# owl-project/owlExaBrick

Hardware: AMD Instinct MI355X
Metric: frames/sec at 2048^2 DVR, exajet-like, MI355X (higher is better)
Workload: dtype f32; 1 GPU; c4_exajet (seed 0xe7a0003 procedural AMR, scale 1.0): 640512000 cells / 1251000 bricks / 13349488 regions, 2048x2048 DVR, dt 0.5, alpha ramp, gradient shading on, space skipping on, frameID 0; tiling=16x16 tiles interleaved over 1 GPU(s)

## Files before the change

include/exa_hip.h:

```cpp
#ifndef EXA_HIP_H
#define EXA_HIP_H

#include <stddef.h>
#include <stdint.h>

#ifdef __cplusplus
extern "C" {
#endif

#define EXA_NUM_XF_VALUES      128
#define EXA_MAX_CHANNELS       10
#define EXA_MAX_ISO_SURFACES   2
#define EXA_MAX_CONTOUR_PLANES 3


typedef struct ExaBrick {
  int32_t  lower[3];
  int32_t  size[3];
  int32_t  level;
  uint32_t begin;
} ExaBrick;

typedef struct ExaBrickRegion {
  float   domain_lo[3], domain_hi[3];
// ... 44 lines not shown
  int32_t               numFields;
  float                 voxelBounds_lo[3], voxelBounds_hi[3];
  const ExaKdNode      *kdNodes;
  uint64_t              numKdNodes;
  int32_t               kdRoot;
  int32_t               allowEmptyCells;
} ExaHipScene;

#define EXA_EMPTY_CELL_POISON_VALUE (-1e20f)
#define EXA_PREP_ALLOW_EMPTY_CELLS 1

typedef struct ExaHipStats {
  uint64_t segments;
  uint64_t sample_evals;
  uint64_t samples;
  uint64_t brick_visits;
  uint64_t corner_loads;
  uint64_t iso_segments;
  uint64_t iso_evals;
  uint64_t nodes_visited;
  uint64_t node_bytes;
  uint64_t pixels;
  uint64_t diag[9];
  uint64_t phase_cycles[5];
  float    kernel_ms;
  float    rebuild_ms;
  uint64_t walk_restarts;
  uint64_t walk_union_nodes;
  uint64_t walk_probe_overflow;
  uint64_t wave_iters;
  uint64_t tile_iters;
  uint64_t walk_leaf_visits;
} ExaHipStats;

typedef struct ExaHipRenderer ExaHipRenderer;
typedef struct ExaPrep ExaPrep;


int exa_prep_create(const int32_t *bricks7, uint64_t numBricks,
                    const int32_t *cellIDs, uint64_t numCellIDs,
                    const float *const *fields, const uint64_t *fieldLen,
                    int32_t numFields, int32_t numRegionFields, int32_t numThreads,
                    ExaPrep **out);
int exa_prep_create_ex(const int32_t *bricks7, uint64_t numBricks,
                       const int32_t *cellIDs, uint64_t numCellIDs,
                       const float *const *fields, const uint64_t *fieldLen,
                       int32_t numFields, int32_t numRegionFields, int32_t numThreads, int32_t flags,
                       ExaPrep **out);
void exa_prep_destroy(ExaPrep *);
int  exa_prep_scene(const ExaPrep *, ExaHipScene *out);
const char *exa_prep_last_error(void);
int exa_prep_ropes(const ExaPrep *, uint64_t *numLeaves, uint64_t *numNodes, float *leafBoxes, int32_t *leafLinks,
                   int32_t *leafRegion, ExaKdNode *nodes, int32_t *flags);
int exa_prep_set_kd_tree(ExaPrep *, const ExaKdNode *nodes, uint64_t numNodes, int32_t root);


int exa_hip_create(const ExaHipScene *scene, int32_t device, ExaHipRenderer **out);
int exa_hip_create_multi(const ExaHipScene *scene, const int32_t *devices, int32_t numDevices, ExaHipRenderer **out);
int exa_hip_destroy(ExaHipRenderer *);

int exa_hip_resize(ExaHipRenderer *, int32_t width, int32_t height);

int exa_hip_set_frame_state(ExaHipRenderer *, const ExaHipFrameState *);

int exa_hip_set_xf(ExaHipRenderer *, int32_t chan, const float *rgba128);

int exa_hip_set_triangles(ExaHipRenderer *, const float *vertices, uint64_t numVertices,
                          const int32_t *triangles, uint64_t numTris);

typedef struct ExaHipTracer {
  int32_t enabled;
  int32_t channels[3];
  int32_t numTraces, numTimesteps;
  float   steplen;
} ExaHipTracer;
int exa_hip_reset_tracer(ExaHipRenderer *, const ExaHipTracer *, const float *seeds);
int exa_hip_set_tracer_enabled(ExaHipRenderer *, int32_t enabled);
int exa_hip_advance_tracer(ExaHipRenderer *, int32_t *rebuild);
int exa_hip_read_traces(ExaHipRenderer *, float *dst);

int exa_hip_set_params(ExaHipRenderer *, const ExaHipParams *);

int exa_hip_set_shard(ExaHipRenderer *, int32_t rank, int32_t worldSize);
uint64_t exa_hip_output_pixels(const ExaHipRenderer *);
int exa_hip_untile(ExaHipRenderer *, const uint32_t *gathered, uint64_t shardStridePixels,
                   int32_t worldSize, uint32_t *rgba8_out, void *hipStream);

int exa_hip_render(ExaHipRenderer *, uint32_t *rgba8, int32_t dstIsDevice,
                   void *hipStream, int32_t async);

int exa_hip_render_stats(ExaHipRenderer *, uint32_t *rgba8, int32_t dstIsDevice, ExaHipStats *out);
int exa_hip_get_stats(ExaHipRenderer *, ExaHipStats *out);

int exa_hip_read_accum(ExaHipRenderer *, float *dst4);
int exa_hip_write_accum(ExaHipRenderer *, const float *src4);

int exa_hip_read_activity(ExaHipRenderer *, int32_t which , uint8_t *dst);

#define EXA_SAMPLE_WORLD_SPACE          1
#define EXA_SAMPLE_GRADIENT             2
#define EXA_SAMPLE_GRADIENT_NORMALIZED  4
int exa_hip_sample_points(ExaHipRenderer *, const float *points , uint64_t n,
                          const int32_t *channels, int32_t numChannels, int32_t flags, float fill,
                          float *values, float *gradients, int32_t *status,
                          int32_t pointersAreDevice, void *hipStream, int32_t async);
int exa_hip_resample(ExaHipRenderer *, const float lo[3], const float hi[3], const int32_t dims[3],
                     int32_t channel, int32_t flags, float fill,
                     float *out , int32_t dstIsDevice, void *hipStream, int32_t async);

int exa_hip_isosurface(ExaHipRenderer *, const float lo[3], const float hi[3], const int32_t dims[3], int32_t channel,
                       float iso, int32_t flags, uint64_t *numVertices, uint64_t *numTriangles, void *hipStream);
int exa_hip_isosurface_read(ExaHipRenderer *, float *vertices, float *gradients, int32_t *triangles,
                            int32_t pointersAreDevice, void *hipStream);
int exa_hip_isosurface_release(ExaHipRenderer *);
int exa_hip_isosurface_stage_ms(ExaHipRenderer *, float ms[6]);

#define EXA_HIST_MAX_BINS   4096
#define EXA_HIST_MAX_LEVELS 32
typedef struct ExaHipFieldStats {
  uint64_t slots;
  uint64_t empty, nan, under, over, binned;
  uint64_t levelCells[EXA_HIST_MAX_LEVELS];
  float    min, max;
} ExaHipFieldStats;
int exa_hip_histogram(ExaHipRenderer *, int32_t channel, float lo, float hi, int32_t numBins,
                      const int32_t box[6] ,
                      uint64_t *cells , uint64_t *volume ,
                      ExaHipFieldStats *stats , void *hipStream);
int exa_hip_histogram_ms(ExaHipRenderer *, float *ms);

#define EXA_STREAM_FORWARD     1
#define EXA_STREAM_BACKWARD    2
#define EXA_STREAM_NORMALIZE   4
#define EXA_STREAM_VELOCITIES  8
#define EXA_STREAM_MAX_STEPS   1048576
#define EXA_STREAM_END_NONE     0
#define EXA_STREAM_END_MAXSTEPS 1
#define EXA_STREAM_END_LEFT     2
#define EXA_STREAM_END_NOVALUE  3
#define EXA_STREAM_END_STAGNANT 4
int exa_hip_streamlines(ExaHipRenderer *, const float *seeds , uint64_t n,
                        const int32_t channels[3], float step, int32_t maxSteps, int32_t flags,
                        uint64_t *numVertices, void *hipStream);
int exa_hip_streamlines_read(ExaHipRenderer *, float *vertices , float *velocities ,
                             uint64_t *offsets , uint32_t *seedVertex , int32_t *reasons ,
                             int32_t pointersAreDevice, void *hipStream);
int exa_hip_streamlines_release(ExaHipRenderer *);
int exa_hip_streamlines_ms(ExaHipRenderer *, float *ms);

int exa_hip_set_option(ExaHipRenderer *, const char *key, int32_t value);

const char *exa_hip_last_error(const ExaHipRenderer * );

#ifdef __cplusplus
}
#endif
#endif
```

owlexabrick_amd/binding.py:

```python
import ctypes as C
import os

import numpy as np

_HERE = os.path.dirname(os.path.abspath(__file__))
LIB_PATH = os.environ.get("EXA_HIP_LIB") or os.path.join(_HERE, "libexa_hip.so")

NUM_XF_VALUES, MAX_CHANNELS, MAX_ISO, MAX_CONTOUR = 128, 10, 2, 3
DEFAULT_BASIS_FORM = 1


class _Iso(C.Structure):
    _fields_ = [("enabled", C.c_int32), ("value", C.c_float), ("channel", C.c_int32)]


class _Contour(C.Structure):
    _fields_ = [("enabled", C.c_int32), ("normal", C.c_float * 3), ("channel", C.c_int32), ("offset", C.c_float)]


class _Clip(C.Structure):
    _fields_ = [("lo", C.c_float * 3), ("hi", C.c_float * 3), ("enabled", C.c_int32)]


class _AO(C.Structure):
    _fields_ = [("length", C.c_float), ("enabled", C.c_int32)]


class ExaHipFrameState(C.Structure):
    _fields_ = [("cam_pos", C.c_float * 3), ("cam_dir00", C.c_float * 3),
                ("cam_dirDu", C.c_float * 3), ("cam_dirDv", C.c_float * 3),
                ("iso", _Iso * MAX_ISO), ("contour", _Contour * MAX_CONTOUR),
                ("clipBox", _Clip), ("ao", _AO), ("clockScale", C.c_float),
                ("xfm_vx", C.c_float * 3), ("xfm_vy", C.c_float * 3),
                ("xfm_vz", C.c_float * 3), ("xfm_p", C.c_float * 3),
                ("frameID", C.c_int32), ("xfDomain", (C.c_float * 2) * MAX_CHANNELS),
                ("xfOpacityScale", C.c_float)]


class ExaHipParams(C.Structure):
    _fields_ = [("dt", C.c_float), ("numPrimaryChannels", C.c_int32), ("colormapChannel", C.c_int32),
                ("gradientShadingDVR", C.c_int32), ("gradientShadingISO", C.c_int32),
                ("numChannels", C.c_int32), ("spaceSkippingEnabled", C.c_int32)]


class ExaHipTracer(C.Structure):
    _fields_ = [("enabled", C.c_int32), ("channels", C.c_int32 * 3), ("numTraces", C.c_int32),
                ("numTimesteps", C.c_int32), ("steplen", C.c_float)]


class ExaHipScene(C.Structure):
    _fields_ = [("bricks", C.c_void_p), ("numBricks", C.c_uint64),
                ("regions", C.c_void_p), ("numRegions", C.c_uint64),
                ("leafList", C.c_void_p), ("leafListSize", C.c_uint64),
                ("scalars", C.c_void_p), ("channelOffset", C.c_void_p),
                ("totalCells", C.c_uint64), ("numFields", C.c_int32),
                ("voxelBounds_lo", C.c_float * 3), ("voxelBounds_hi", C.c_float * 3),
                ("kdNodes", C.c_void_p), ("numKdNodes", C.c_uint64), ("kdRoot", C.c_int32), ("allowEmptyCells", C.c_int32)]


class ExaHipStats(C.Structure):
    _fields_ = [(n, C.c_uint64) for n in ("segments", "sample_evals", "samples", "brick_visits", "corner_loads",
                                          "iso_segments", "iso_evals", "nodes_visited", "node_bytes", "pixels")] + \
               [("diag", C.c_uint64 * 9), ("phase_cycles", C.c_uint64 * 5), ("kernel_ms", C.c_float), ("rebuild_ms", C.c_float),
                ("walk_restarts", C.c_uint64), ("walk_union_nodes", C.c_uint64), ("walk_probe_overflow", C.c_uint64),
                ("wave_iters", C.c_uint64), ("tile_iters", C.c_uint64), ("walk_leaf_visits", C.c_uint64)]

    def asdict(self):
        d = {}
        for n, t in self._fields_:
            v = getattr(self, n)
            d[n] = int(v) if t is C.c_uint64 else (float(v) if t is C.c_float else [int(x) for x in v])
        return d


HIST_MAX_BINS = 4096
HIST_MAX_LEVELS = 32


class ExaHipFieldStats(C.Structure):
    _fields_ = [("slots", C.c_uint64), ("empty", C.c_uint64), ("nan", C.c_uint64), ("under", C.c_uint64), ("over", C.c_uint64),
                ("binned", C.c_uint64), ("levelCells", C.c_uint64 * HIST_MAX_LEVELS), ("min", C.c_float), ("max", C.c_float)]

    def asdict(self):
        d = {k: int(getattr(self, k)) for k in ("slots", "empty", "nan", "under", "over", "binned")}
        d["levelCells"] = np.array(self.levelCells, dtype=np.uint64)
        d["min"], d["max"] = np.float32(self.min), np.float32(self.max)
        return d


BRICK_DTYPE = np.dtype([("lower", "<i4", 3), ("size", "<i4", 3), ("level", "<i4"), ("begin", "<u4")])
REGION_DTYPE = np.dtype([("dom_lo", "<f4", 3), ("dom_hi", "<f4", 3), ("vr_lo", "<f4"), ("vr_hi", "<f4"),
                         ("leafListBegin", "<i4"), ("leafListSize", "<i4"), ("finestLevelCellWidth", "<f4")])
KDNODE_DTYPE = np.dtype([("split", "<f4"), ("axis", "<i4"), ("left", "<i4"), ("right", "<i4")])
KD_EMPTY = -2 ** 31

ABI_SYMBOLS = ["exa_prep_create", "exa_prep_create_ex", "exa_prep_destroy", "exa_prep_scene", "exa_prep_last_error", "exa_prep_ropes", "exa_prep_set_kd_tree",
               "exa_hip_create", "exa_hip_create_multi", "exa_hip_destroy", "exa_hip_resize", "exa_hip_set_frame_state",
               "exa_hip_set_xf", "exa_hip_set_triangles", "exa_hip_reset_tracer", "exa_hip_set_tracer_enabled",
               "exa_hip_advance_tracer", "exa_hip_read_traces", "exa_hip_set_params", "exa_hip_set_shard", "exa_hip_output_pixels",
               "exa_hip_untile", "exa_hip_render", "exa_hip_render_stats", "exa_hip_get_stats",
               "exa_hip_read_accum", "exa_hip_write_accum", "exa_hip_read_activity",
               "exa_hip_set_option", "exa_hip_last_error", "exa_hip_sample_points", "exa_hip_resample",
               "exa_hip_isosurface", "exa_hip_isosurface_read", "exa_hip_isosurface_release", "exa_hip_isosurface_stage_ms",
               "exa_hip_histogram", "exa_hip_histogram_ms",
               "exa_hip_streamlines", "exa_hip_streamlines_read", "exa_hip_streamlines_release", "exa_hip_streamlines_ms"]

SAMPLE_WORLD_SPACE = 1
SAMPLE_GRADIENT = 2
SAMPLE_GRADIENT_NORMALIZED = 4

STREAM_FORWARD = 1
STREAM_BACKWARD = 2
STREAM_NORMALIZE = 4
STREAM_VELOCITIES = 8
STREAM_MAX_STEPS = 1 << 20
STREAM_END_NONE, STREAM_END_MAXSTEPS, STREAM_END_LEFT, STREAM_END_NOVALUE, STREAM_END_STAGNANT = range(5)

_lib = None


def lib():
    global _lib
    if _lib is None:
        if not os.path.exists(LIB_PATH):
            import subprocess
            try:
                subprocess.check_call(["make", "-C", os.path.join(_HERE, "csrc"), "-s", "-j6"])
            except Exception as e:
                raise RuntimeError(f"{LIB_PATH} not found and building it failed ({e}); run "
                                   "__graft_entry__.build(); there is no CPU fallback") from e
        L = C.CDLL(LIB_PATH)
        vp = C.c_void_p
        L.exa_prep_create.restype = C.c_int
        L.exa_prep_create.argtypes = [vp, C.c_uint64, vp, C.c_uint64, C.POINTER(vp), C.POINTER(C.c_uint64),
                                      C.c_int32, C.c_int32, C.c_int32, C.POINTER(vp)]
        L.exa_prep_create_ex.restype = C.c_int
        L.exa_prep_create_ex.argtypes = [vp, C.c_uint64, vp, C.c_uint64, C.POINTER(vp), C.POINTER(C.c_uint64),
                                         C.c_int32, C.c_int32, C.c_int32, C.c_int32, C.POINTER(vp)]
        L.exa_prep_destroy.argtypes = [vp]
        L.exa_prep_ropes.argtypes = [vp, C.POINTER(C.c_uint64), C.POINTER(C.c_uint64), vp, vp, vp, vp, C.POINTER(C.c_int32)]
        L.exa_prep_scene.argtypes = [vp, C.POINTER(ExaHipScene)]
        L.exa_prep_set_kd_tree.argtypes = [vp, vp, C.c_uint64, C.c_int32]
        L.exa_prep_last_error.restype = C.c_char_p
        L.exa_hip_create.argtypes = [C.POINTER(ExaHipScene), C.c_int32, C.POINTER(vp)]
        L.exa_hip_create_multi.argtypes = [C.POINTER(ExaHipScene), C.POINTER(C.c_int32), C.c_int32, C.POINTER(vp)]
        L.exa_hip_destroy.argtypes = [vp]
        L.exa_hip_resize.argtypes = [vp, C.c_int32, C.c_int32]
        L.exa_hip_set_frame_state.argtypes = [vp, C.POINTER(ExaHipFrameState)]
        L.exa_hip_set_xf.argtypes = [vp, C.c_int32, vp]
        L.exa_hip_set_params.argtypes = [vp, C.POINTER(ExaHipParams)]
        L.exa_hip_set_triangles.argtypes = [vp, vp, C.c_uint64, vp, C.c_uint64]
        L.exa_hip_reset_tracer.argtypes = [vp, C.POINTER(ExaHipTracer), vp]
        L.exa_hip_set_tracer_enabled.argtypes = [vp, C.c_int32]
        L.exa_hip_advance_tracer.argtypes = [vp, C.POINTER(C.c_int32)]
        L.exa_hip_read_traces.argtypes = [vp, vp]
        L.exa_hip_set_shard.argtypes = [vp, C.c_int32, C.c_int32]
        L.exa_hip_output_pixels.restype = C.c_uint64
        L.exa_hip_output_pixels.argtypes = [vp]
        L.exa_hip_untile.argtypes = [vp, vp, C.c_uint64, C.c_int32, vp, vp]
        L.exa_hip_render.argtypes = [vp, vp, C.c_int32, vp, C.c_int32]
        L.exa_hip_render_stats.argtypes = [vp, vp, C.c_int32, C.POINTER(ExaHipStats)]
        L.exa_hip_get_stats.argtypes = [vp, C.POINTER(ExaHipStats)]
        L.exa_hip_read_accum.argtypes = [vp, vp]
        L.exa_hip_write_accum.argtypes = [vp, vp]
        L.exa_hip_read_activity.argtypes = [vp, C.c_int32, vp]
        L.exa_hip_set_option.argtypes = [vp, C.c_char_p, C.c_int32]
        L.exa_hip_last_error.restype = C.c_char_p
        L.exa_hip_last_error.argtypes = [vp]
        L.exa_hip_sample_points.argtypes = [vp, vp, C.c_uint64, vp, C.c_int32, C.c_int32, C.c_float, vp, vp, vp,
                                            C.c_int32, vp, C.c_int32]
        L.exa_hip_resample.argtypes = [vp, vp, vp, vp, C.c_int32, C.c_int32, C.c_float, vp, C.c_int32, vp, C.c_int32]
        L.exa_hip_isosurface.argtypes = [vp, vp, vp, vp, C.c_int32, C.c_float, C.c_int32, C.POINTER(C.c_uint64),
                                         C.POINTER(C.c_uint64), vp]
        L.exa_hip_isosurface_read.argtypes = [vp, vp, vp, vp, C.c_int32, vp]
        L.exa_hip_isosurface_release.argtypes = [vp]
        L.exa_hip_isosurface_stage_ms.argtypes = [vp, vp]
        L.exa_hip_histogram_ms.argtypes = [vp, C.POINTER(C.c_float)]
        L.exa_hip_histogram.argtypes = [vp, C.c_int32, C.c_float, C.c_float, C.c_int32, vp, vp, vp, C.POINTER(ExaHipFieldStats), vp]
        L.exa_hip_streamlines.argtypes = [vp, vp, C.c_uint64, vp, C.c_float, C.c_int32, C.c_int32, C.POINTER(C.c_uint64), vp]
        L.exa_hip_streamlines_read.argtypes = [vp, vp, vp, vp, vp, vp, C.c_int32, vp]
        L.exa_hip_streamlines_release.argtypes = [vp]
        L.exa_hip_streamlines_ms.argtypes = [vp, C.POINTER(C.c_float)]
        _lib = L
    return _lib


class Prep:

    def __init__(self, scene, num_region_fields=None, num_threads=0, allow_empty_cells=False):
        L = lib()
        self.bricks7 = np.ascontiguousarray(scene.bricks7, dtype=np.int32).reshape(-1, 7)
        self.cellIDs = np.ascontiguousarray(scene.cellIDs, dtype=np.int32)
        self.fields = [np.ascontiguousarray(f, dtype=np.float32) for f in scene.fields]
        nf = len(self.fields)
        ptrs = (C.c_void_p * max(nf, 1))(*[f.ctypes.data for f in self.fields])
        lens = (C.c_uint64 * max(nf, 1))(*[f.size for f in self.fields])
        self.h = C.c_void_p()
        rc = L.exa_prep_create_ex(self.bricks7.ctypes.data, self.bricks7.shape[0], self.cellIDs.ctypes.data,
                                  self.cellIDs.size, ptrs, lens, nf,
                                  nf if num_region_fields is None else num_region_fields, num_threads,
                                  1 if allow_empty_cells else 0, C.byref(self.h))
        if rc:
            raise RuntimeError(L.exa_prep_last_error().decode())
        self.scene = ExaHipScene()
        L.exa_prep_scene(self.h, C.byref(self.scene))
        self.num_fields = nf

    def _arr(self, ptr, count, dtype):
        if count == 0:
            return np.zeros(0, dtype=dtype)
        buf = (C.c_char * (count * np.dtype(dtype).itemsize)).from_address(ptr)
        return np.frombuffer(buf, dtype=dtype)

    def bricks(self):
        return self._arr(self.scene.bricks, self.scene.numBricks, BRICK_DTYPE)

    def regions(self):
        return self._arr(self.scene.regions, self.scene.numRegions, REGION_DTYPE)

    def leaflist(self):
        return self._arr(self.scene.leafList, self.scene.leafListSize, np.int32)

    def scalars(self):
        return self._arr(self.scene.scalars, self.scene.numFields * self.scene.totalCells, np.float32)

    def kd_nodes(self):
        return self._arr(self.scene.kdNodes, self.scene.numKdNodes, KDNODE_DTYPE)

    def ropes(self):
        nl, nn, flags = C.c_uint64(0), C.c_uint64(0), C.c_int32(0)
        if lib().exa_prep_ropes(self.h, C.byref(nl), C.byref(nn), None, None, None, None, None):
            raise RuntimeError(lib().exa_prep_last_error().decode())
        boxes = np.zeros((nl.value, 6), dtype=np.float32)
        links = np.zeros((nl.value, 6), dtype=np.int32)
        region = np.zeros(nl.value, dtype=np.int32)
        nodes = np.zeros(max(1, nn.value), dtype=KDNODE_DTYPE)
        if lib().exa_prep_ropes(self.h, C.byref(nl), C.byref(nn), boxes.ctypes.data, links.ctypes.data, region.ctypes.data,
                                nodes.ctypes.data, C.byref(flags)):
            raise RuntimeError(lib().exa_prep_last_error().decode())
        return dict(boxes=boxes, links=links, region=region, nodes=nodes[:nn.value], flags=int(flags.value))

    def set_kd_tree(self, nodes, root):
        nodes = np.ascontiguousarray(nodes, dtype=KDNODE_DTYPE)
        if lib().exa_prep_set_kd_tree(self.h, nodes.ctypes.data if len(nodes) else None, len(nodes), int(root)):
            raise RuntimeError(lib().exa_prep_last_error().decode())
        lib().exa_prep_scene(self.h, C.byref(self.scene))

    def voxel_bounds(self):
        return (np.array(self.scene.voxelBounds_lo, dtype=np.float32),
                np.array(self.scene.voxelBounds_hi, dtype=np.float32))

    def close(self):
        if getattr(self, "h", None):
            lib().exa_prep_destroy(self.h)
            self.h = None

    __del__ = close


class Renderer:

    def __init__(self, prep, device=0, multiFieldDvr=True, devices=None):
        L = lib()
        self.prep = prep
        self.h = C.c_void_p()
        if devices is not None:
            arr = (C.c_int32 * len(devices))(*devices)
            rc = L.exa_hip_create_multi(C.byref(prep.scene), arr, len(devices), C.byref(self.h))
        else:
            rc = L.exa_hip_create(C.byref(prep.scene), device, C.byref(self.h))
        if rc:
            raise RuntimeError(L.exa_hip_last_error(None).decode())
        self.numFields = prep.num_fields
        self.frameState = ExaHipFrameState()
        self.frameState.xfm_vx[0] = self.frameState.xfm_vy[1] = self.frameState.xfm_vz[2] = 1.0
        self.frameState.ao.length, self.frameState.ao.enabled = 1e20, 1
        self.frameState.xfOpacityScale = 1.0
        for i in range(MAX_CONTOUR):
            self.frameState.contour[i].normal[0] = 1.0
            self.frameState.contour[i].offset = 0.5
        nprim = self.numFields if multiFieldDvr else 1
        self.params = ExaHipParams(0.5, nprim, 0 if (multiFieldDvr or self.numFields < 2) else 1, 1, 1, nprim, 1)
        self.doSpaceSkipping = True
        self.fbSize = (0, 0)
        self.voxelSpaceBounds = prep.voxel_bounds()

    def _check(self, rc):
        if rc:
            raise RuntimeError(lib().exa_hip_last_error(self.h).decode())

    def close(self):
        if getattr(self, "h", None):
            lib().exa_hip_destroy(self.h)
            self.h = None

    __del__ = close

    def setVoxelSpaceTransform(self, vx, vy, vz, p):
        for i in range(3):
            self.frameState.xfm_vx[i], self.frameState.xfm_vy[i] = float(vx[i]), float(vy[i])
            self.frameState.xfm_vz[i], self.frameState.xfm_p[i] = float(vz[i]), float(p[i])

    def resizeFrameBuffer(self, fbSize):
        self.fbSize = (int(fbSize[0]), int(fbSize[1]))
        self._check(lib().exa_hip_resize(self.h, *self.fbSize))

    def updateIsoValues(self, isoValues, channels, enabled):
        for i in range(MAX_ISO):
            self.frameState.iso[i].value = float(isoValues[i])
            self.frameState.iso[i].channel = int(channels[i])
            self.frameState.iso[i].enabled = int(enabled[i])

    def resetTracer(self, seeds, channels=(0, 1, 2), numTimesteps=100, steplen=1e-6, enabled=True):
        sd = np.ascontiguousarray(seeds, dtype=np.float32).reshape(-1, 3)
        self._tracer = ExaHipTracer(int(enabled), (C.c_int32 * 3)(*channels), sd.shape[0], int(numTimesteps), float(steplen))
        self._check(lib().exa_hip_reset_tracer(self.h, C.byref(self._tracer), sd.ctypes.data))

    def setTracerEnabled(self, enable):
        self._check(lib().exa_hip_set_tracer_enabled(self.h, int(bool(enable))))

    def advanceTracer(self):
        r = C.c_int32(0)
        self._check(lib().exa_hip_advance_tracer(self.h, C.byref(r)))
        return bool(r.value)

    def readTraces(self):
        out = np.zeros((self._tracer.numTraces, self._tracer.numTimesteps, 3), dtype=np.float32)
        self._check(lib().exa_hip_read_traces(self.h, out.ctypes.data))
        return out

    def setTriangles(self, verts, tris):
        v = np.ascontiguousarray(verts, dtype=np.float32).reshape(-1, 3)
        t = np.ascontiguousarray(tris, dtype=np.int32).reshape(-1, 3)
        self._check(lib().exa_hip_set_triangles(self.h, v.ctypes.data, v.shape[0], t.ctypes.data, t.shape[0]))

    def updateContourPlanes(self, normals, offsets, channels, enabled):
        for i in range(MAX_CONTOUR):
            n = np.asarray(normals[i], dtype=np.float32)
            n = (n * (np.float32(1.0) / np.sqrt(np.dot(n, n), dtype=np.float32))).astype(np.float32)
            for k in range(3):
                self.frameState.contour[i].normal[k] = float(n[k])
            self.frameState.contour[i].offset = float(offsets[i])
            self.frameState.contour[i].channel = int(channels[i])
            self.frameState.contour[i].enabled = int(enabled[i])

    def updateCamera(self, pos, dir00, dirDu, dirDv):
        for i in range(3):
            self.frameState.cam_pos[i], self.frameState.cam_dir00[i] = float(pos[i]), float(dir00[i])
            self.frameState.cam_dirDu[i], self.frameState.cam_dirDv[i] = float(dirDu[i]), float(dirDv[i])

    def updateXF(self, chan, opacities, colorMap, xfDomain, xfOpacityScale=0.1):
        colorMap = np.asarray(colorMap, dtype=np.float32)
        if colorMap.shape[0] != NUM_XF_VALUES:
            raise RuntimeError("mismatching xf size!?")
        lut = np.concatenate([colorMap[:, :3], np.asarray(opacities, dtype=np.float32).reshape(-1, 1)], axis=1)
        lut = np.ascontiguousarray(lut, dtype=np.float32)
        self.frameState.xfDomain[chan][0], self.frameState.xfDomain[chan][1] = float(xfDomain[0]), float(xfDomain[1])
        self.frameState.xfOpacityScale = float(xfOpacityScale)
        self._check(lib().exa_hip_set_xf(self.h, chan, lut.ctypes.data))

    def updateFrameID(self, frameID):
        self.frameState.frameID = int(frameID)

    def updateDt(self, dt):
        self.params.dt = float(dt)

    def setSpaceSkipping(self, enable):
        self.doSpaceSkipping = bool(enable)

    def setGradientShadingDVR(self, enable):
        self.params.gradientShadingDVR = int(bool(enable))

    def setGradientShadingISO(self, enable):
        self.params.gradientShadingISO = int(bool(enable))

    def setShard(self, rank, world):
        self._check(lib().exa_hip_set_shard(self.h, rank, world))

    def setOption(self, key, value):
        self._check(lib().exa_hip_set_option(self.h, key.encode(), int(value)))

    def _push_state(self):
        contour = any(self.frameState.contour[i].enabled for i in range(MAX_CONTOUR))
        self.params.spaceSkippingEnabled = int((not contour) and self.doSpaceSkipping)
        self._check(lib().exa_hip_set_frame_state(self.h, C.byref(self.frameState)))
        self._check(lib().exa_hip_set_params(self.h, C.byref(self.params)))

    def outputPixels(self):
        return int(lib().exa_hip_output_pixels(self.h))

    def render(self, device_ptr=None, stream=None, async_=False):
        self._push_state()
        if device_ptr is not None:
            self._check(lib().exa_hip_render(self.h, C.c_void_p(device_ptr), 1, C.c_void_p(stream or 0), int(async_)))
            return None
        n = self.outputPixels()
        out = np.zeros(n, dtype=np.uint32)
        self._check(lib().exa_hip_render(self.h, out.ctypes.data, 0, None, 0))
        W, H = self.fbSize
        return out.reshape(H, W) if n == W * H else out

    def renderStats(self):
        self._push_state()
        n = self.outputPixels()
        out = np.zeros(n, dtype=np.uint32)
        st = ExaHipStats()
        self._check(lib().exa_hip_render_stats(self.h, out.ctypes.data, 0, C.byref(st)))
        W, H = self.fbSize
        return (out.reshape(H, W) if n == W * H else out), st.asdict()

    def stats(self):
        st = ExaHipStats()
        self._check(lib().exa_hip_get_stats(self.h, C.byref(st)))
        return st.asdict()

    def readAccum(self):
        n = self.outputPixels()
        out = np.zeros((n, 4), dtype=np.float32)
        self._check(lib().exa_hip_read_accum(self.h, out.ctypes.data))
        W, H = self.fbSize
        return out.reshape(H, W, 4) if n == W * H else out

    def writeAccum(self, accum):
        a = np.ascontiguousarray(accum, dtype=np.float32)
        self._check(lib().exa_hip_write_accum(self.h, a.ctypes.data))

    def readActivity(self, which=0):
        self._push_state()
        out = np.zeros(self.prep.scene.numRegions, dtype=np.uint8)
        self._check(lib().exa_hip_read_activity(self.h, which, out.ctypes.data))
        return out

    def untile(self, gathered_ptr, shard_stride, world, out_ptr, stream=None):
        self._check(lib().exa_hip_untile(self.h, C.c_void_p(gathered_ptr), shard_stride, world,
                                         C.c_void_p(out_ptr), C.c_void_p(stream or 0)))

    def _probe_world(self, world):
        if world:
            self._push_state()
        return SAMPLE_WORLD_SPACE if world else 0

    def samplePoints(self, points, channels=(0,), gradient=False, normalized=False, world=False, fill=float("nan"),
                     stream=None, async_=False):
        chans = np.ascontiguousarray(channels, dtype=np.int32).reshape(-1)
        flags = self._probe_world(world) | (SAMPLE_GRADIENT if gradient or normalized else 0)
        flags |= SAMPLE_GRADIENT_NORMALIZED if normalized else 0
        k = chans.size
        if getattr(points, "is_cuda", False):
            import torch
            if points.dtype != torch.float32 or not points.is_contiguous() or points.numel() % 3:
                raise TypeError("points: a contiguous float32 tensor [n, 3]")
            n = points.numel() // 3
            values = torch.empty((n, k), dtype=torch.float32, device=points.device)
            grads = torch.empty((n, k, 3), dtype=torch.float32, device=points.device) if flags & SAMPLE_GRADIENT else None
            status = torch.empty((n, k), dtype=torch.int32, device=points.device)
            self._check(lib().exa_hip_sample_points(self.h, _dev_ptr(points), n, chans.ctypes.data, k, flags, float(fill),
                                                    _dev_ptr(values), _dev_ptr(grads), _dev_ptr(status), 1,
                                                    C.c_void_p(stream or 0), int(async_)))
            return values, grads, status
        pts = np.ascontiguousarray(points, dtype=np.float32).reshape(-1, 3)
        n = pts.shape[0]
        values = np.empty((n, k), dtype=np.float32)
        grads = np.empty((n, k, 3), dtype=np.float32) if flags & SAMPLE_GRADIENT else None
        status = np.empty((n, k), dtype=np.int32)
        self._check(lib().exa_hip_sample_points(self.h, pts.ctypes.data, n, chans.ctypes.data, k, flags, float(fill),
                                                values.ctypes.data, grads.ctypes.data if grads is not None else None,
                                                status.ctypes.data, 0, None, 0))
        return values, grads, status

    def resample(self, lo, hi, dims, channel=0, world=False, fill=float("nan"), out_ptr=None, stream=None, async_=False):
        flags = self._probe_world(world)
        lo3 = (C.c_float * 3)(*[float(v) for v in lo])
        hi3 = (C.c_float * 3)(*[float(v) for v in hi])
        d3 = (C.c_int32 * 3)(*[int(v) for v in dims])
        if out_ptr is not None:
            self._check(lib().exa_hip_resample(self.h, lo3, hi3, d3, int(channel), flags, float(fill), _dev_ptr(out_ptr), 1,
                                               C.c_void_p(stream or 0), int(async_)))
            return None
        out = np.empty(tuple(max(int(d), 0) for d in dims[::-1]), dtype=np.float32)
        self._check(lib().exa_hip_resample(self.h, lo3, hi3, d3, int(channel), flags, float(fill), out.ctypes.data, 0, None, 0))
        return out

    def extractIsoSurface(self, lo, hi, dims, iso, channel=0, world=False, gradients=False, stream=None):
        flags = self._probe_world(world) | (SAMPLE_GRADIENT if gradients else 0)
        lo3 = (C.c_float * 3)(*[float(v) for v in lo])
        hi3 = (C.c_float * 3)(*[float(v) for v in hi])
        d3 = (C.c_int32 * 3)(*[int(v) for v in dims])
        nv, nt = C.c_uint64(0), C.c_uint64(0)
        self._check(lib().exa_hip_isosurface(self.h, lo3, hi3, d3, int(channel), float(iso), flags, C.byref(nv), C.byref(nt),
                                             C.c_void_p(stream or 0)))
        self._iso_counts = (int(nv.value), int(nt.value), bool(gradients))
        return self._iso_counts[:2]

    def readIsoSurface(self):
        nv, nt, grad = getattr(self, "_iso_counts", (0, 0, False))
        verts = np.empty((nv, 3), dtype=np.float32)
        tris = np.empty((nt, 3), dtype=np.int32)
        grads = np.empty((nv, 3), dtype=np.float32) if grad else None
        self._check(lib().exa_hip_isosurface_read(self.h, verts.ctypes.data, grads.ctypes.data if grad else None,
                                                  tris.ctypes.data, 0, None))
        return verts, tris, grads

    def releaseIsoSurface(self):
        self._check(lib().exa_hip_isosurface_release(self.h))
        self._iso_counts = (0, 0, False)

    def isoSurfaceStageMs(self):
        ms = (C.c_float * 6)()
        self._check(lib().exa_hip_isosurface_stage_ms(self.h, ms))
        return [float(v) for v in ms]

    def isosurface(self, lo, hi, dims, iso, channel=0, world=False, gradients=False):
        self.extractIsoSurface(lo, hi, dims, iso, channel=channel, world=world, gradients=gradients)
        try:
            return self.readIsoSurface()
        finally:
            self.releaseIsoSurface()

    def histogram(self, channel, lo, hi, bins, box=None, volume=True, stream=None):
        bins = int(bins)
        n = min(max(bins, 0), HIST_MAX_BINS)
        cells = np.zeros(n, dtype=np.uint64)
        vol = np.zeros(n, dtype=np.uint64) if volume else None
        b6 = (C.c_int32 * 6)(*[int(v) for v in box]) if box is not None else None
        st = ExaHipFieldStats()
        self._check(lib().exa_hip_histogram(self.h, int(channel), float(lo), float(hi), bins, b6, cells.ctypes.data,
                                            vol.ctypes.data if volume else None, C.byref(st), C.c_void_p(stream or 0)))
        return cells, vol, st.asdict()

    def histogramMs(self):
        ms = C.c_float(0)
        self._check(lib().exa_hip_histogram_ms(self.h, C.byref(ms)))
        return float(ms.value)
# ... 56 lines not shown
```

owlexabrick_amd/csrc/exa_create.cpp:

```cpp
#include "exa_renderer.h"
#include "exa_hostbvh.h"

#include <cmath>
#include <cstdlib>
#include <cstring>

thread_local std::string g_createError;

namespace {

struct EventSlot { hipEvent_t ExaHipRenderer::*ev; bool timing; };
const EventSlot kEvents[] = {
  { &ExaHipRenderer::ev0, true },      { &ExaHipRenderer::ev1, true },      { &ExaHipRenderer::ev2, true },
  { &ExaHipRenderer::evFork, false },  { &ExaHipRenderer::evJoin4, false }, { &ExaHipRenderer::evJoin2, false },
  { &ExaHipRenderer::evJoinN, false }, { &ExaHipRenderer::evPre, false },   { &ExaHipRenderer::evPre2, false },
  { &ExaHipRenderer::evAo, false },    { &ExaHipRenderer::evAo2, false },
};
hipStream_t ExaHipRenderer::*const kSideStreams[] = { &ExaHipRenderer::side4, &ExaHipRenderer::side2, &ExaHipRenderer::sideN };

uint64_t volumeOf(const ExaBrick &B) { return uint64_t(B.size[0]) * uint64_t(B.size[1]) * uint64_t(B.size[2]); }

void buildBrickOrders(ExaHipRenderer *h, const ExaHipScene *scene)
{
  const uint64_t nb = scene->numBricks;
  h->beginUploaded.resize(nb);
  std::vector<std::pair<uint64_t, uint32_t>> keyed(nb);
  for (uint64_t b = 0; b < nb; b++) {
    const ExaBrick &B = scene->bricks[b];
    h->beginUploaded[b] = B.begin;
    double c[3];
    for (int k = 0; k < 3; k++) {
      const double cw = double(1u << B.level);
      c[k] = double(B.lower[k]) + 0.5 * cw * double(B.size[k]);
    }
    keyed[b] = { mortonKey(c, scene->voxelBounds_lo, scene->voxelBounds_hi), uint32_t(b) };
  }
  std::sort(keyed.begin(), keyed.end());
  h->beginMorton.resize(nb);
  uint64_t at = 0;
  for (uint64_t i = 0; i < nb; i++) {
    h->beginMorton[keyed[i].second] = uint32_t(at);
    at += volumeOf(scene->bricks[keyed[i].second]);
  }
  bool partition = at == scene->totalCells;
  for (int f = 0; f < scene->numFields && partition; f++) partition = scene->channelOffset[f] == uint64_t(f) * scene->totalCells;
  if (partition) {
    std::vector<std::pair<uint32_t, uint64_t>> spans(nb);
    for (uint64_t b = 0; b < nb; b++) spans[b] = { scene->bricks[b].begin, volumeOf(scene->bricks[b]) };
    std::sort(spans.begin(), spans.end());
    uint64_t run = 0;
    for (uint64_t b = 0; b < nb && partition; b++) { partition = spans[b].first == run; run += spans[b].second; }
  }
  h->brickOrderPossible = partition;
  if (!partition) h->beginMorton = h->beginUploaded;
  if (const char *e = std::getenv("EXA_BRICK_ORDER")) h->brickOrderWanted = std::atoi(e) != 0 && h->brickOrderPossible;
}

std::vector<ExaBrick> buildMarchHeaders(const ExaHipScene *scene)
{
  std::vector<ExaBrick> hdr(scene->leafListSize);
  for (uint64_t i = 0; i < scene->leafListSize; i++) {
    const ExaBrick &B = scene->bricks[scene->leafList[i]];
    const float lowerF[3] = { float(B.lower[0]), float(B.lower[1]), float(B.lower[2]) };
    const float invCw = std::ldexp(1.f, -B.level);
    ExaBrick &o = hdr[i];
    std::memcpy(&o.lower[0], lowerF, sizeof(lowerF));
    std::memcpy(&o.size[0], &invCw, sizeof(float));
    o.size[1] = B.size[0]; o.size[2] = B.size[1]; o.level = B.size[2]; o.begin = B.begin;
  }
  return hdr;
}

void chooseAddressForms(ExaHipRenderer *h, const ExaHipScene *scene)
{
  h->mul24 = 1;
  for (uint64_t b = 0; b < scene->numBricks; b++) {
    const ExaBrick &B = scene->bricks[b];
    if (uint64_t(B.size[0]) * uint64_t(B.size[1]) >= (1ull << 24) || B.size[0] >= (1 << 24) || B.size[1] >= (1 << 24) || B.size[2] >= (1 << 24))
      h->mul24 = 0;
  }
  if (scene->totalCells >= (1ull << 32)) h->mul24 = 0;
  h->addr32 = ((scene->totalCells + 2) * sizeof(float) <= (1ull << 32)
               && scene->leafListSize * 32ull < (1ull << 32)
               && scene->numKdNodes * sizeof(KdNodeDev) < (1ull << 32)) ? 1 : 0;
}

bool kdTreeWellFormed(const ExaHipScene *scene)
{
  const uint64_t nk = scene->numKdNodes;
  auto refOk = [&](int32_t ref) {
    if (ref == EXA_KD_EMPTY) return true;
    return ref >= 0 ? uint64_t(ref) < nk : uint64_t(~ref) < scene->numRegions;
  };
  bool ok = refOk(scene->kdRoot) && scene->kdRoot != EXA_KD_EMPTY && nk < 0x7fffffffull;
  for (uint64_t i = 0; ok && i < nk; i++) {
    const ExaKdNode &n = scene->kdNodes[i];
    ok = n.axis >= 0 && n.axis <= 2 && refOk(n.left) && refOk(n.right)
         && (n.left < 0 || uint64_t(n.left) > i) && (n.right < 0 || uint64_t(n.right) > i);
  }
  return ok;
}

void buildKdLevelOrder(const ExaHipScene *scene, std::vector<int32_t> &ids, std::vector<int> &levelBegin)
{
  const uint64_t nk = scene->numKdNodes;
  std::vector<int32_t> kh(nk, 1);
  for (uint64_t ii = nk; ii-- > 0;) {
    const ExaKdNode &n = scene->kdNodes[ii];
    int hh = 0;
    if (n.left >= 0) hh = std::max(hh, kh[n.left]);
    if (n.right >= 0) hh = std::max(hh, kh[n.right]);
    kh[ii] = hh + 1;
  }
  orderByHeight(kh, ids, levelBegin);
}

bool buildMarchTree(const ExaHipScene *scene, const std::vector<KdNodeDev> &kd, std::vector<KdNodeDev> &mk, int32_t &root,
                    uint32_t &bb, uint32_t &sb)
{
  auto bitsFor = [](uint64_t maxValue) { uint32_t b = 0; while (b < 63 && (1ull << b) <= maxValue) b++; return b; };
  uint64_t maxSize = 1; int maxLevel = 0; bool pow2 = true;
  for (uint64_t r = 0; r < scene->numRegions; r++) {
    const ExaBrickRegion &R = scene->regions[r];
    maxSize = std::max<uint64_t>(maxSize, (uint64_t)R.leafListSize);
    const int lv = levelOfWidth(R.finestLevelCellWidth);
    if (float(1 << lv) != R.finestLevelCellWidth) pow2 = false;
    maxLevel = std::max(maxLevel, lv);
  }
  bb = std::max(1u, bitsFor(scene->leafListSize ? scene->leafListSize - 1 : 0));
  sb = bitsFor(maxSize - 1);
  const uint32_t lb = bitsFor((uint64_t)maxLevel);
  if (!pow2 || bb + sb + lb > 31) return false;
  auto pack = [&](int32_t ref) -> int32_t {
    if (ref >= 0 || ref == EXA_KD_EMPTY) return ref;
    const ExaBrickRegion &R = scene->regions[~ref];
    return ~int32_t(packLeafRec(R.leafListBegin, R.leafListSize, R.finestLevelCellWidth, bb, sb));
  };
  mk = kd;
  bool clash = false;
  for (auto &n : mk) {
    n.left = pack(n.left); n.right = pack(n.right);
    clash = clash || (n.left < 0 && n.left != EXA_KD_EMPTY && n.left <= INT32_MIN + 1) || (n.right < 0 && n.right != EXA_KD_EMPTY && n.right <= INT32_MIN + 1);
  }
  root = pack(scene->kdRoot);
  clash = clash || (root < 0 && root <= INT32_MIN + 1);
  if (clash) return false;
  if (mk.empty()) mk.resize(1);
  return true;
}

}

extern "C" {

int exa_hip_create(const ExaHipScene *scene, int32_t device, ExaHipRenderer **out)
{
  if (!out || !scene) { g_createError = "exa_hip_create: null argument"; return 1; }
  *out = nullptr;
  if (scene->allowEmptyCells != 0 && scene->allowEmptyCells != 1) {
    g_createError = "exa_hip_create: ExaHipScene.allowEmptyCells is 0 or 1 (was the struct zero-initialised before it was filled?)";
    return 1;
  }
  int ndev = 0;
  hipError_t e = hipGetDeviceCount(&ndev);
  if (e != hipSuccess || ndev <= 0) {
    g_createError = std::string("exa_hip_create: no HIP device available (") + hipGetErrorString(e)
                  + "); this module has no CPU fallback";
    return 2;
  }
  if (device < 0 || device >= ndev) { g_createError = "exa_hip_create: bad device index"; return 1; }
  if (scene->numFields < 1 || scene->numFields > EXA_MAX_CHANNELS) { g_createError = "exa_hip_create: 1..10 scalar fields required"; return 1; }
  if (scene->numRegions == 0 || scene->numBricks == 0) { g_createError = "exa_hip_create: empty scene"; return 1; }
  if (scene->numRegions > 0x7fffffffull) { g_createError = "exa_hip_create: too many regions"; return 1; }
  ExaHipRenderer *h = new ExaHipRenderer;
  h->device = device;
  auto bail = [&]() { g_createError = h->err; delete h; return 1; };
#define CREATE_TRY(call) do { hipError_t e_ = (call); if (e_ != hipSuccess) { h->fail(std::string(#call) + ": " + hipGetErrorString(e_)); return bail(); } } while (0)
  DeviceGuard guard_(device);
  CREATE_TRY(guard_.err);

  for (uint64_t i = 0; i < scene->leafListSize; i++)
    if (scene->leafList[i] < 0 || uint64_t(scene->leafList[i]) >= scene->numBricks) { h->fail("exa_hip_create: leaf list entry out of range"); return bail(); }
  for (uint64_t b = 0; b < scene->numBricks; b++) {
    const ExaBrick &B = scene->bricks[b];
    if (B.size[0] <= 0 || B.size[1] <= 0 || B.size[2] <= 0 || B.level < 0 || B.level > 30
        || uint64_t(B.begin) + volumeOf(B) > scene->totalCells) { h->fail("exa_hip_create: brick record out of range"); return bail(); }
  }
  for (int f = 0; f < scene->numFields; f++)
    if (scene->channelOffset[f] + scene->totalCells > uint64_t(scene->numFields) * scene->totalCells) { h->fail("exa_hip_create: channel offset out of range"); return bail(); }

  h->numFields = scene->numFields;
  h->emptyCells = scene->allowEmptyCells != 0;
  if (h->emptyCells) h->basisForm = 0;
  h->totalCells = scene->totalCells;
  h->numBricks = scene->numBricks; h->leafListSize = scene->leafListSize;
  buildBrickOrders(h, scene);
  if (const char *e = std::getenv("EXA_BASIS_FORM")) h->basisForm = std::atoi(e) != 0 && !h->emptyCells;
  for (int k = 0; k < 3; k++) { h->voxLo[k] = scene->voxelBounds_lo[k]; h->voxHi[k] = scene->voxelBounds_hi[k]; }
  static_assert(sizeof(ExaBrick) == 2 * sizeof(int4), "brick = two int4");
  CREATE_TRY(h->bricks.upload(reinterpret_cast<const int4 *>(scene->bricks), scene->numBricks * 2));
  CREATE_TRY(h->leafList.upload(scene->leafList, scene->leafListSize));
  {
    const std::vector<ExaBrick> hdr = buildMarchHeaders(scene);
    CREATE_TRY(h->leafHdr.upload(reinterpret_cast<const int4 *>(hdr.data()), hdr.size() * 2));
  }
  chooseAddressForms(h, scene);
  CREATE_TRY(h->scalars.upload(scene->scalars, size_t(scene->numFields) * scene->totalCells));
  std::vector<RegionInfo> ri(scene->numRegions);
  std::vector<float2> vr(scene->numRegions);
  std::vector<float> dom(scene->numRegions * 6);
  for (uint64_t r = 0; r < scene->numRegions; r++) {
    const ExaBrickRegion &R = scene->regions[r];
    if (R.leafListSize < 1 || R.leafListBegin < 0 || uint64_t(R.leafListBegin) + uint64_t(R.leafListSize) > scene->leafListSize) {
      h->fail("exa_hip_create: region leaf list out of range"); return bail();
    }
    {
      int ex = 0;
      const float mant = std::frexp(R.finestLevelCellWidth, &ex);
      if (!(R.finestLevelCellWidth >= 1.f && R.finestLevelCellWidth <= 1073741824.f) || mant != 0.5f) {
        h->fail("exa_hip_create: region finestLevelCellWidth is not a power of two >= 1"); return bail();
      }
    }
    ri[r].listBegin = R.leafListBegin;
    ri[r].listSize = R.leafListSize;
    ri[r].finestLevelCellWidth = R.finestLevelCellWidth;
    ri[r].firstBrick = scene->leafList[R.leafListBegin];
    vr[r] = make_float2(R.valueRange_lo, R.valueRange_hi);
    for (int k = 0; k < 3; k++) { dom[6 * r + k] = R.domain_lo[k]; dom[6 * r + 3 + k] = R.domain_hi[k]; }
  }
  CREATE_TRY(h->regionInfo.upload(ri.data(), ri.size()));
  CREATE_TRY(h->valueRange.upload(vr.data(), vr.size()));
  CREATE_TRY(h->domain.upload(dom.data(), dom.size()));

  for (int k = 0; k < 3; k++) { h->kdLo[k] = INFINITY; h->kdHi[k] = -INFINITY; }
  for (uint64_t r = 0; r < scene->numRegions; r++)
    for (int k = 0; k < 3; k++) {
      h->kdLo[k] = std::fmin(h->kdLo[k], scene->regions[r].domain_lo[k]);
      h->kdHi[k] = std::fmax(h->kdHi[k], scene->regions[r].domain_hi[k]);
    }
  if (scene->kdNodes != nullptr || (scene->numKdNodes == 0 && scene->numRegions == 1 && scene->kdRoot == ~int32_t(0))) {
    const uint64_t nk = scene->numKdNodes;
    if (!kdTreeWellFormed(scene)) { h->fail("exa_hip_create: malformed kd-tree"); return bail(); }
    std::vector<int32_t> kids;
    buildKdLevelOrder(scene, kids, h->kdLevelBegin);
    std::vector<KdNodeDev> kd(nk);
    for (uint64_t i = 0; i < nk; i++) {
      kd[i].split = scene->kdNodes[i].split;
      kd[i].word = (uint32_t)scene->kdNodes[i].axis;
      kd[i].left = scene->kdNodes[i].left;
      kd[i].right = scene->kdNodes[i].right;
    }
    std::vector<RegionRec> rec(scene->numRegions);
    for (uint64_t r = 0; r < scene->numRegions; r++) {
      const ExaBrickRegion &R = scene->regions[r];
      RegionRec &q = rec[r];
      q.lo[0] = R.domain_lo[0]; q.lo[1] = R.domain_lo[1]; q.lo[2] = R.domain_lo[2];
      q.hi0 = R.domain_hi[0]; q.hi1 = R.domain_hi[1]; q.hi2 = R.domain_hi[2];
      q.finestLevelCellWidth = R.finestLevelCellWidth;
      q.firstBrick = scene->leafList[R.leafListBegin];
      q.listBegin = R.leafListBegin; q.listSize = R.leafListSize; q.pad0 = q.pad1 = 0;
    }
    CREATE_TRY(h->kdNodes.upload(kd.data(), kd.size()));
    {
      std::vector<KdNodeDev> mk;
      int32_t root = 0;
      uint32_t bb = 0, sb = 0;
      if (buildMarchTree(scene, kd, mk, root, bb, sb)) {
        CREATE_TRY(h->kdMarchNodes.upload(mk.data(), mk.size()));
        h->kdMarchRoot = root;
        h->leafBeginBits = bb; h->leafSizeBits = sb;
      }
    }
    CREATE_TRY(h->kdLevelIds.upload(kids.data(), kids.size()));
    CREATE_TRY(h->regionRec.upload(rec.data(), rec.size()));
    h->kdRoot = scene->kdRoot;
    h->haveKd = true;
  }
  CREATE_TRY(h->volActive.alloc(scene->numRegions));
  CREATE_TRY(h->isoActive.alloc(scene->numRegions));
  CREATE_TRY(h->xf.alloc(size_t(EXA_MAX_CHANNELS) * EXA_NUM_XF_VALUES));
  std::memset(h->xfHost, 0, sizeof(h->xfHost));
  CREATE_TRY(h->statsBuf.alloc(ST_COUNT));
  CREATE_TRY(h->errorFlag.alloc(1));
  CREATE_TRY(hipMemset(h->errorFlag.p, 0, sizeof(int32_t)));
  for (const EventSlot &slot : kEvents)
    CREATE_TRY(hipEventCreateWithFlags(&(h->*slot.ev), slot.timing ? hipEventDefault : hipEventDisableTiming));
  for (auto stream : kSideStreams) CREATE_TRY(hipStreamCreateWithFlags(&(h->*stream), hipStreamNonBlocking));
  {
    hipDeviceProp_t prop;
    if (hipGetDeviceProperties(&prop, device) == hipSuccess && prop.multiProcessorCount > 0)
      h->numSimdWaves = prop.multiProcessorCount * 4 * 6;
  }

  h->sc.bricks = h->bricks.p;
  h->sc.leafList = h->leafList.p;
  h->sc.leafHdr = h->leafHdr.p;
  h->sc.scalars = h->scalars.p;
  h->sc.regionInfo = h->regionInfo.p;
  h->sc.valueRange = h->valueRange.p;
  h->sc.domain = h->domain.p;
  for (int f = 0; f < EXA_MAX_CHANNELS; f++) h->sc.channelOffset[f] = f < scene->numFields ? scene->channelOffset[f] : 0;
  h->sc.numRegions = (uint32_t)scene->numRegions;
  h->sc.numInternal = 0;
#undef CREATE_TRY
  *out = h;
  return 0;
}

int exa_hip_create_multi(const ExaHipScene *scene, const int32_t *devices, int32_t numDevices, ExaHipRenderer **out)
{
  if (!out || !scene || !devices || numDevices < 1 || numDevices > 64) { g_createError = "exa_hip_create_multi: bad arguments"; return 1; }
  *out = nullptr;
  ExaHipRenderer *h = new ExaHipRenderer;
  h->device = devices[0];
  auto bail = [&](const std::string &msg) { g_createError = msg; exa_hip_destroy(h); return 1; };
  for (int i = 0; i < numDevices; i++) {
    ExaHipRenderer *c = nullptr;
    if (int rc = exa_hip_create(scene, devices[i], &c)) { exa_hip_destroy(h); return rc; }
    h->children.push_back(c);
    c->colorRowMajor = true;
    c->rank = i; c->world = numDevices; c->layoutDirty = true;
    DeviceGuard g(devices[i]);
    if (g.err != hipSuccess || hipStreamCreateWithFlags(&c->ownStream, hipStreamNonBlocking) != hipSuccess)
      return bail("exa_hip_create_multi: cannot create a stream on device " + std::to_string(devices[i]));
    if (devices[i] != devices[0]) {
      int can = 0;
      if (hipDeviceCanAccessPeer(&can, devices[i], devices[0]) != hipSuccess || !can)
        return bail("exa_hip_create_multi: device " + std::to_string(devices[i]) + " cannot access device " + std::to_string(devices[0]));
      const hipError_t e = hipDeviceEnablePeerAccess(devices[0], 0);
      if (e != hipSuccess && e != hipErrorPeerAccessAlreadyEnabled) return bail(std::string("hipDeviceEnablePeerAccess: ") + hipGetErrorString(e));
      (void)hipGetLastError();
    }
  }
  {
    DeviceGuard g(devices[0]);
    if (g.err != hipSuccess || hipEventCreateWithFlags(&h->evCall, hipEventDisableTiming) != hipSuccess) return bail("exa_hip_create_multi: hipEventCreate failed");
  }
  h->numFields = h->children[0]->numFields;
  *out = h;
  return 0;
}

int exa_hip_destroy(ExaHipRenderer *h)
{
  if (!h) return 0;
  for (ExaHipRenderer *c : h->children) exa_hip_destroy(c);
  h->children.clear();
  DeviceGuard guard_(h->device);
  if (h->ownStream) (void)hipStreamDestroy(h->ownStream);
  if (h->evCall) (void)hipEventDestroy(h->evCall);
  (void)hipDeviceSynchronize();
  for (const EventSlot &slot : kEvents) if (h->*slot.ev) (void)hipEventDestroy(h->*slot.ev);
  for (auto stream : kSideStreams) if (h->*stream) (void)hipStreamDestroy(h->*stream);
  delete h;
  return 0;
}

}
```

owlexabrick_amd/csrc/exa_device.h:

```cpp
#pragma once
#include "../../include/exa_hip.h"
#include <hip/hip_runtime.h>

#include <vector>

#ifndef EXA_MARCH_WAVES
#define EXA_MARCH_WAVES 6
#endif
#ifndef EXA_ROPE_WAVES
#define EXA_ROPE_WAVES 7
#endif
#ifndef EXA_MULTI_WAVES
#define EXA_MULTI_WAVES 6
#endif
#ifndef EXA_PREPASS_WAVES
#define EXA_PREPASS_WAVES 4
#endif
#ifndef EXA_IL2_WAVES
#define EXA_IL2_WAVES 5
#endif
#ifndef EXA_IL34_WAVES
#define EXA_IL34_WAVES 4
#endif
#ifndef EXA_PREPASS_ISO_WAVES
#define EXA_PREPASS_ISO_WAVES 4
#endif
#ifndef EXA_AO_ISO_WAVES
#define EXA_AO_ISO_WAVES 6
#endif
#ifndef EXA_EMPTY_CELLS
#define EXA_EMPTY_CELLS 0
#endif
#ifndef EXA_BASIS_FORM
#define EXA_BASIS_FORM 0
#endif
namespace exa {

struct alignas(64) BvhNode {
  float4 q0, q1, q2;
  int32_t child0, child1, pad0, pad1;
};
static_assert(sizeof(BvhNode) == 64, "node must be one 64-byte line");

struct alignas(16) RegionInfo {
  int32_t listBegin;
  int32_t listSize;
  float   finestLevelCellWidth;
  int32_t firstBrick;
};

struct alignas(16) KdNodeDev {
  float    split;
  uint32_t word;
  int32_t  left, right;
};
static_assert(sizeof(KdNodeDev) == 16, "kd node = one 16-byte load");

struct alignas(16) RopeLeaf {
  float    lo[3], hi0;
  float    hi1, hi2;
  uint32_t rec;
  uint32_t flags;
  int32_t  rope[6];
  int32_t  region;
  int32_t  pad;
};
static_assert(sizeof(RopeLeaf) == 64, "rope leaf = four 16-byte loads");

struct alignas(16) RegionRec {
  float   lo[3], hi0;
  float   hi1, hi2, finestLevelCellWidth; int32_t firstBrick;
  int32_t listBegin, listSize, pad0, pad1;
};
static_assert(sizeof(RegionRec) == 48, "region record = three 16-byte loads");

struct DeviceScene {
  const int4       *bricks;
  const int32_t    *leafList;
  const int4       *leafHdr;
  const float      *scalars;
  const RegionInfo *regionInfo;
  const float2     *valueRange;
  const float      *domain;
  unsigned long long channelOffset[EXA_MAX_CHANNELS];
  uint32_t numRegions;
  uint32_t numInternal;
};

#ifndef EXA_KD_STACK
#define EXA_KD_STACK 4
#endif
#ifndef EXA_KD_STACK_MULTI
#define EXA_KD_STACK_MULTI 3
#endif
#ifndef EXA_ROPE_QUEUE
#define EXA_ROPE_QUEUE 5
#endif
#ifndef EXA_ROPE_QUEUE_MULTI
#define EXA_ROPE_QUEUE_MULTI 5
#endif
#ifndef EXA_SEG_QUEUE
#define EXA_SEG_QUEUE 4
#endif
enum { kKdStackEntries = EXA_KD_STACK, kKdStackMultiEntries = EXA_KD_STACK_MULTI };
enum { kTile = 16, kTilePixels = 256, kStackDepth = 32, kKdStack = EXA_KD_STACK, kKdStackMulti = EXA_KD_STACK_MULTI, kSegQueue = EXA_SEG_QUEUE,
       kRopeQueue = EXA_ROPE_QUEUE, kRopeQueueMulti = EXA_ROPE_QUEUE_MULTI,
       kKdBlock = 256,
       kWideSegCap = 256,
       kWalkProbeBits = 15, kWalkProbeSize = 1 << kWalkProbeBits };

enum StatSlot { ST_SEGMENTS, ST_SAMPLE_EVALS, ST_SAMPLES, ST_BRICK_VISITS, ST_CORNER_LOADS,
                ST_ISO_SEGMENTS, ST_ISO_EVALS, ST_NODES,
                ST_W_BRICK, ST_L_BRICK, ST_W_FINAL, ST_L_FINAL, ST_W_NODE, ST_L_NODE, ST_W_LEAF, ST_L_LEAF,
                ST_KD_MISMATCH,
                ST_T_BRICK, ST_T_FINAL, ST_T_WALK, ST_T_SEG, ST_T_OTHER,
                ST_RESTARTS, ST_UNION, ST_PROBE_OVERFLOW, ST_WAVE_ITERS, ST_TILE_ITERS,
                ST_ROPE_LEAVES,
                ST_COUNT };

struct alignas(16) AoRecord { float4 posFd, ngAmb, baseRnd; uint32_t slot, pad0, pad1, pad2; };
static_assert(sizeof(AoRecord) == 64, "AO record = four 16-byte stores");

struct RenderArgs {
  DeviceScene        sc;
  const BvhNode     *volNodes;
  const BvhNode     *isoNodes;
  const KdNodeDev   *kdNodes;
  const KdNodeDev   *kdMarchNodes;
  int32_t            kdMarchRoot;
  uint32_t           leafBeginBits, leafSizeBits;
  const RegionRec   *regionRec;
  const RopeLeaf    *ropeLeaves;
  const KdNodeDev   *ropeNodes;
  int32_t            ropeRoot;
  int32_t            ropeFastDiv;
  int32_t            ropeAddr32;
  int32_t            kdRoot;
  int32_t            kdIsoRoot;
  float              kdLo[3], kdHi[3];
  const BvhNode     *meshNodes;
  const float       *meshVerts;
  const int32_t     *meshTris;
  int32_t            numTris;
  const BvhNode     *streamNodes;
  const float       *traces;
  int32_t            numStreamPrims;
  int32_t            tracerChannels[3], numTraces, numTimesteps, timestep;
  float              steplen;
  float              worldLo[3], worldHi[3];
  ExaHipFrameState   fs;
  ExaHipParams       p;
  const float4      *xf;
  const float       *cellsIl;
  int32_t            il32;
  int32_t            mul24;
  int32_t            addr32;
  float              invDtPow2;
  int32_t            fastSampler;
  float              tfFracMagic;
  int32_t            numXfChannels;
  int32_t            W, H, tilesX, tilesY;
  int32_t            rank, world;
  const int32_t     *tileMap;
  uint32_t          *color;
  int32_t            colorRowMajor;
  float4            *accum;
  float4            *surf;
  float4            *pixOut;
  uint32_t          *surfRnd;
  unsigned long long *stats;
  int32_t           *errorFlag;
  int32_t            debugPixel;
  const int32_t     *wideTileMap;
  float4            *wideSegs;
  uint32_t          *walkProbe;
  AoRecord          *aoRecs;
  uint32_t          *aoCount;
  uint32_t          *aoKeys;
  uint32_t          *aoHist;
  uint32_t          *aoOrder;
  uint8_t           *aoHit;
  uint32_t           aoBins;
  uint32_t          *tileCostPre;
  uint32_t          *tileCost;
};

struct SampleArgs {
  const int4        *leafHdr;
  const float       *scalars;
  const KdNodeDev   *kdNodes;
  const RegionRec   *regionRec;
  int32_t            kdRoot;
  int32_t            maxSteps;
  float              kdLo[3], kdHi[3];
  int32_t           *errorFlag;
  int32_t            world;
  int32_t            normalized;
  float              fill;
  ExaHipFrameState   fs;
  int32_t            numChannels;
  unsigned long long fieldOffset[EXA_MAX_CHANNELS];
  const float       *points;
  unsigned long long count;
  float             *values, *gradients;
  int32_t           *status;
  float              lo[3], step[3];
  int32_t            box0[3], box1[3];
  unsigned long long patchesX, patchesY, numPatches;
  unsigned long long strideY, strideZ;
  float             *out;
};
enum { kSamplePatchShapes = 4 };

struct StreamArgs {
  SampleArgs         s;
  const float       *seeds;
  unsigned long long numSeeds;
  unsigned long long laneBase;
  unsigned long long numLanes;
  float              step;
  int32_t            maxSteps;
  int32_t            flags;
  uint32_t          *counts;
  int32_t           *reasons;
  const unsigned long long *offsets;
  const uint32_t    *seedVertex;
  float             *vertices;
  float             *velocities;
};

hipError_t buildLbvhTopologyDevice(const float *boxes, uint32_t numPrims, BvhNode *nodes, int32_t *levelIds,
                                   std::vector<uint32_t> &internalNodesPerDepth, hipStream_t s);

#define EXA_FORM_LAUNCHERS                                                                                              \
  hipError_t launchRender(const RenderArgs &a, int numBlocks, bool grad, bool iso, bool stats, hipStream_t s);          \
  hipError_t launchSurfacePrepassKd(const RenderArgs &a, int numBlocks, bool stats, hipStream_t s);                     \
   \
  hipError_t launchAoRaysKd(const RenderArgs &a, int numBlocks, hipStream_t s);                                         \
  hipError_t launchCompositeKd(const RenderArgs &a, int numBlocks, hipStream_t s);                                      \
  hipError_t launchRenderKd(const RenderArgs &a, int numBlocks, bool grad, bool fast, bool surf,                        \
                            int stats , hipStream_t s);                                 \
                                                                    \
  hipError_t launchRenderKdRope(const RenderArgs &a, int numBlocks, bool grad, bool fast, bool surf,                    \
                                int stats, hipStream_t s);                                                              \
  hipError_t launchRenderKdWide(const RenderArgs &a, int numTiles, int lanesPerRay, bool grad, bool fast, bool surf,    \
                                hipStream_t s);                                                                         \
                          \
  hipError_t launchComputeTraces(const RenderArgs &a, float *traces, int count, hipStream_t s);                        \
    \
  hipError_t launchSamplePoints(const SampleArgs &a, bool grad, hipStream_t s);                                      \
  hipError_t launchSampleGrid(const SampleArgs &a, int shape, bool uniform, hipStream_t s);                          \
                                                                          \
  hipError_t launchStreamlines(const StreamArgs &a, bool emit, hipStream_t s);
namespace form0 { EXA_FORM_LAUNCHERS }
namespace form1 { EXA_FORM_LAUNCHERS }
namespace form0e { EXA_FORM_LAUNCHERS }
#undef EXA_FORM_LAUNCHERS

hipError_t launchVolumeActivity(const DeviceScene &sc, const ExaHipFrameState &fs, const ExaHipParams &p,
                                const float4 *xf, uint8_t *active, float tfFracMagic, hipStream_t s);
hipError_t launchIsoActivity(const DeviceScene &sc, const ExaHipFrameState &fs, uint8_t *active, hipStream_t s);
hipError_t launchRefit(BvhNode *nodes, const int32_t *nodeIds, int count, const float *domain,
                       const uint8_t *active, hipStream_t s);
hipError_t launchKdRefit(KdNodeDev *nodes, KdNodeDev *marchNodes, const int32_t *nodeIds, int count, const uint8_t *active, int which, hipStream_t s);
hipError_t launchRopeActivity(RopeLeaf *leaves, uint32_t numRegions, const uint8_t *active, int which, uint32_t *activeCount, hipStream_t s);
hipError_t launchPermuteBricks(const float *src, float *dst, const uint32_t *srcBegin, const uint32_t *dstBegin, int4 *bricks,
                               unsigned long long numBricks, int4 *leafHdr, const int32_t *leafList, unsigned long long leafListSize,
                               unsigned long long totalCells, int numFields, hipStream_t s);
hipError_t launchInterleave(const DeviceScene &sc, unsigned long long totalCells, int nch, float *out, hipStream_t s);
hipError_t launchUntile(const uint32_t *gathered, unsigned long long shardStride, int world,
                        int W, int H, uint32_t *out, hipStream_t s);
hipError_t launchProfileMarker(int tag, hipStream_t s);

}
```

owlexabrick_amd/csrc/exa_frame.cpp:

```cpp
#include "exa_renderer.h"
#include "exa_hostbvh.h"

#include <chrono>
#include <cmath>
#include <cstdio>
#include <cstdlib>
#include <thread>

#ifndef EXA_WIDE_SPEED2
#define EXA_WIDE_SPEED2 1.63
#endif
#ifndef EXA_WIDE_WORK2
#define EXA_WIDE_WORK2 1.49
#endif
#ifndef EXA_WIDE_WORK4
#define EXA_WIDE_WORK4 1.88
#endif

int ExaHipRenderer::applyBrickOrder(hipStream_t s)
{
  if (brickOrderWanted == brickOrder) return 0;
  const std::vector<uint32_t> &from = brickOrder ? beginMorton : beginUploaded, &to = brickOrderWanted ? beginMorton : beginUploaded;
  HIP_TRY(this, hipStreamSynchronize(s));
  HIP_TRY(this, hipDeviceSynchronize());
  DevBuf<uint32_t> dFrom, dTo;
  DevBuf<float> moved;
  HIP_TRY(this, dFrom.upload(from.data(), from.size()));
  HIP_TRY(this, dTo.upload(to.data(), to.size()));
  HIP_TRY(this, moved.alloc(scalars.n));
  HIP_TRY(this, launchPermuteBricks(scalars.p, moved.p, dFrom.p, dTo.p, bricks.p, numBricks, leafHdr.p, leafList.p, leafListSize,
                                    totalCells, numFields, s));
  HIP_TRY(this, hipStreamSynchronize(s));
  std::swap(scalars.p, moved.p);
  sc.scalars = scalars.p;
  brickOrder = brickOrderWanted;
  ilChannels = 0; cellsIl.release();
  return 0;
}

void ExaHipRenderer::worldBounds(float lo[3], float hi[3]) const
{
  auto cross = [](const float *a, const float *b, float *o) { o[0] = a[1] * b[2] - a[2] * b[1]; o[1] = a[2] * b[0] - a[0] * b[2]; o[2] = a[0] * b[1] - a[1] * b[0]; };
  float c0[3], c1[3], c2[3];
  cross(fs.xfm_vy, fs.xfm_vz, c0); cross(fs.xfm_vz, fs.xfm_vx, c1); cross(fs.xfm_vx, fs.xfm_vy, c2);
  const float det = fs.xfm_vx[0] * c0[0] + fs.xfm_vx[1] * c0[1] + fs.xfm_vx[2] * c0[2];
  const float ix[3] = { c0[0] / det, c1[0] / det, c2[0] / det }, iy[3] = { c0[1] / det, c1[1] / det, c2[1] / det },
              iz[3] = { c0[2] / det, c1[2] / det, c2[2] / det };
  float ip[3];
  for (int k = 0; k < 3; k++) ip[k] = -(fs.xfm_p[0] * ix[k] + (fs.xfm_p[1] * iy[k] + fs.xfm_p[2] * iz[k]));
  for (int k = 0; k < 3; k++) {
    lo[k] = voxLo[0] * ix[k] + (voxLo[1] * iy[k] + (voxLo[2] * iz[k] + ip[k]));
    hi[k] = voxHi[0] * ix[k] + (voxHi[1] * iy[k] + (voxHi[2] * iz[k] + ip[k]));
  }
}

int ExaHipRenderer::rebuildLayout()
{
  tilesX = (W + kTile - 1) / kTile;
  tilesY = (H + kTile - 1) / kTile;
  numBlocks = numBlocksFor();
  const size_t px = world <= 1 ? size_t(W) * H : size_t(numBlocks) * kTilePixels;
  HIP_TRY(this, accum.alloc(px));
  if (px) HIP_TRY(this, hipMemset(accum.p, 0, px * sizeof(float4)));
  HIP_TRY(this, color.alloc(px));
  surf.release(); surfRnd.release();
  std::vector<int32_t> map;
  map.reserve(numBlocks);
  for (int t = rank; t < tilesX * tilesY; t += world) map.push_back(t);
  if (tileOrder == 1 && world == 1 && tilesX % 8 == 0 && tilesY % 8 == 0 && ((tilesX / 8) * (tilesY / 8)) % 8 == 0) {
    const int stx = tilesX / 8;
    for (int b = 0; b < numBlocks; b++) {
      const int xcd = b % 8, j = b / 8;
      const int super = (j / 64) * 8 + xcd, in = j % 64;
      const int sx = super % stx, sy = super / stx;
      map[b] = (sy * 8 + in / 8) * tilesX + sx * 8 + in % 8;
    }
  }
  if (tileOrder == 2) {
    uint64_t st = 0x9E3779B97F4A7C15ull;
    for (size_t i = map.size(); i > 1; i--) {
      st = st * 6364136223846793005ull + 1442695040888963407ull;
      std::swap(map[i - 1], map[size_t((st >> 33) % i)]);
    }
  } else if (tileOrder == 3) {
    const float cx = 0.5f * tilesX, cy = 0.5f * tilesY;
    std::stable_sort(map.begin(), map.end(), [&](int32_t a, int32_t b) {
      const float ax = a % tilesX + 0.5f - cx, ay = a / tilesX + 0.5f - cy, bx = b % tilesX + 0.5f - cx, by = b / tilesX + 0.5f - cy;
      return ax * ax + ay * ay < bx * bx + by * by;
    });
  }
  if (tileOrder >= 4) {
    auto part = [](uint32_t v) { v &= 0xffff; v = (v | v << 8) & 0x00ff00ff; v = (v | v << 4) & 0x0f0f0f0f; v = (v | v << 2) & 0x33333333; v = (v | v << 1) & 0x55555555; return v; };
    std::stable_sort(map.begin(), map.end(), [&](int32_t a, int32_t b) {
      return (part(a % tilesX) | part(a / tilesX) << 1) < (part(b % tilesX) | part(b / tilesX) << 1);
    });
    const int chunk = tileOrder == 5 ? 16 : (tileOrder == 6 ? 64 : (tileOrder == 7 ? 256 : 0));
    if (chunk && map.size() % size_t(8 * chunk) == 0) {
      std::vector<int32_t> z(map);
      for (size_t b = 0; b < map.size(); b++) {
        const size_t xcd = b % 8, j = b / 8;
        map[b] = z[((j / chunk) * 8 + xcd) * chunk + j % chunk];
      }
    }
  }
  HIP_TRY(this, tileMap.upload(map.data(), map.size()));
  HIP_TRY(this, tileCost.alloc(size_t(tilesX) * tilesY));
  HIP_TRY(this, tileCostPre.alloc(size_t(tilesX) * tilesY));
  nPreCheap = nPreHeavy = 0;
  baseMap = map; curMap = map;
  costPhase = 1;
  nNormal = nWide4 = nWide2 = 0;
  if (assignWide(nullptr)) return 1;
  layoutDirty = false;
  return 0;
}

int ExaHipRenderer::reorderFromCosts()
{
  costPhase = 0;
  const size_t n = curMap.size();
  if (n < 2) return 0;
  std::vector<uint32_t> costOfTile(size_t(tilesX) * tilesY, 0);
  HIP_TRY(this, hipMemcpy(costOfTile.data(), tileCost.p, costOfTile.size() * sizeof(uint32_t), hipMemcpyDeviceToHost));
  uint32_t maxC = 0;
  for (size_t b = 0; b < n; b++) maxC = std::max(maxC, costOfTile[curMap[b]]);
  int kClasses = 256;
  if (const char *e = std::getenv("EXA_COST_CLASSES")) kClasses = std::max(1, std::min(4096, std::atoi(e)));
  std::vector<std::vector<int32_t>> cls(kClasses);
  for (size_t b = 0; b < n; b++) {
    const int32_t t = baseMap[b];
    const int c = kClasses - 1 - int(uint64_t(costOfTile[t]) * kClasses / (uint64_t(maxC) + 1));
    cls[c].push_back(t);
  }
  if (std::getenv("EXA_HIP_VERBOSE")) {
    uint64_t sum = 0;
    for (size_t b = 0; b < n; b++) sum += costOfTile[curMap[b]];
    std::fprintf(stderr, "[exa_hip] tile costs: %zu tiles, max %u iterations, sum %llu, per class (heaviest first):", n, maxC,
                 (unsigned long long)sum);
    for (int c = 0; c < kClasses; c++) std::fprintf(stderr, " %zu", cls[c].size());
    std::fprintf(stderr, "\n");
  }
  std::vector<int32_t> order;
  order.reserve(n);
  for (int c = 0; c < kClasses; c++) order.insert(order.end(), cls[c].begin(), cls[c].end());
  if (order != curMap) {
    HIP_TRY(this, hipMemcpy(tileMap.p, order.data(), n * sizeof(int32_t), hipMemcpyHostToDevice));
    curMap.swap(order);
  }
  nPreCheap = nPreHeavy = 0;
  if (preMeasured && prepassSplit) {
    std::vector<uint32_t> pre(size_t(tilesX) * tilesY, 0);
    HIP_TRY(this, hipMemcpy(pre.data(), tileCostPre.p, pre.size() * sizeof(uint32_t), hipMemcpyDeviceToHost));
    uint32_t maxP = 0;
    for (size_t b = 0; b < n; b++) maxP = std::max(maxP, pre[curMap[b]]);
    uint32_t div = 32, minSteps = 16;
    if (const char *e = std::getenv("EXA_PREPASS_SPLIT_DIV")) div = (uint32_t)std::max(1, std::atoi(e));
    if (const char *e = std::getenv("EXA_PREPASS_SPLIT_MIN")) minSteps = (uint32_t)std::max(0, std::atoi(e));
    const uint32_t thr = std::max<uint32_t>(minSteps, maxP / div);
    std::vector<int32_t> cheap, heavy;
    for (size_t b = 0; b < n; b++) (pre[curMap[b]] > thr ? heavy : cheap).push_back(curMap[b]);
    if (!heavy.empty() && !cheap.empty()) {
      std::stable_sort(heavy.begin(), heavy.end(), [&](int32_t x, int32_t y) { return pre[x] > pre[y]; });
      std::vector<int32_t> both(cheap);
      both.insert(both.end(), heavy.begin(), heavy.end());
      HIP_TRY(this, splitMap.refill(both.data(), both.size()));
      nPreCheap = (int)cheap.size(); nPreHeavy = (int)heavy.size();
    }
    if (std::getenv("EXA_HIP_VERBOSE"))
      std::fprintf(stderr, "[exa_hip] pre-pass costs: longest iso march %u steps; %d tiles in the heavy pipeline, %d in the other\n", maxP, nPreHeavy, nPreCheap);
  }
  return assignWide(&costOfTile);
}

int ExaHipRenderer::assignWide(const std::vector<uint32_t> *costOfTile)
{
  const size_t n = curMap.size();
  std::vector<int32_t> normal, w4, w2;
  const int lanesTop = 4;
  if (wideMode == 2 || wideMode == 4) {
    (wideMode >= 4 ? w4 : w2) = curMap;
  } else if (wideMode == 1 && costOfTile) {
    double kSpeed2 = EXA_WIDE_SPEED2;
    const double kWork2 = EXA_WIDE_WORK2, kLoaded = 1.3;
// ... 141 lines not shown
          std::fprintf(stderr, "[exa_hip] no memory for the channel-interleaved copy of %d fields: field-by-field march\n", want);
        ilNoMemory = want;
        want = 0;
      }
      if (want) {
        HIP_TRY(this, hipMemsetAsync(cellsIl.p + size_t(totalCells) * want, 0, 2 * size_t(want) * sizeof(float), s));
        HIP_TRY(this, launchInterleave(sc, totalCells, want, cellsIl.p, s));
        ilChannels = want;
      }
    }
  }
  const bool needIso = isoEnabled();
  if (volDirty || (needIso && isoDirty)) {
    HIP_TRY(this, hipEventRecord(ev2, s));
    const bool volChanged = volDirty;
    if (volDirty) {
      HIP_TRY(this, launchVolumeActivity(sc, fs, p, xf.p, volActive.p, tfFracMagic(), s));
      if (lbvhBuilt && refit(volNodes, volActive.p, s)) return 1;
      if (haveKd && kdRefit(volActive.p, 0, s)) return 1;
      volDirty = false;
    }
    if (needIso && isoDirty) {
      if (lbvhBuilt && !isoNodes.p && topoNodes.n) {
        HIP_TRY(this, isoNodes.alloc(topoNodes.n));
        HIP_TRY(this, hipMemcpyAsync(isoNodes.p, topoNodes.p, topoNodes.n * sizeof(BvhNode), hipMemcpyDeviceToDevice, s));
      }
      HIP_TRY(this, launchIsoActivity(sc, fs, isoActive.p, s));
      if (lbvhBuilt && refit(isoNodes, isoActive.p, s)) return 1;
      if (haveKd && kdRefit(isoActive.p, 1, s)) return 1;
      isoDirty = false;
    }
    if (haveKd && volChanged) {
      if (!activeCountBuf.p) HIP_TRY(this, activeCountBuf.alloc(1));
      HIP_TRY(this, hipMemsetAsync(activeCountBuf.p, 0, sizeof(uint32_t), s));
      HIP_TRY(this, launchRopeActivity(ropeBuilt ? ropeLeaves.p : nullptr, sc.numRegions, volActive.p, 0, activeCountBuf.p, s));
      ropeFlagsStale = !ropeBuilt;
    }
    HIP_TRY(this, hipEventRecord(ev1, s));
    HIP_TRY(this, hipEventSynchronize(ev1));
    HIP_TRY(this, hipEventElapsedTime(&last.rebuild_ms, ev2, ev1));
    if (haveKd && volChanged) HIP_TRY(this, hipMemcpy(&activeRegions, activeCountBuf.p, sizeof(uint32_t), hipMemcpyDeviceToHost));
    if (haveKd && kdRoot < 0 && kdRoot != EXA_KD_EMPTY) {
      uint8_t f[2] = {1, 1};
      HIP_TRY(this, hipMemcpy(&f[0], volActive.p + ~kdRoot, 1, hipMemcpyDeviceToHost));
      if (needIso) HIP_TRY(this, hipMemcpy(&f[1], isoActive.p + ~kdRoot, 1, hipMemcpyDeviceToHost));
      rootLeafVolActive = f[0] != 0;
      rootLeafIsoActive = f[1] != 0;
    }
  }
  const bool ropeBefore = ropeThisFrame;
  ropeThisFrame = ropeWanted();
  if (ropeThisFrame != ropeBefore && std::getenv("EXA_HIP_VERBOSE"))
    std::fprintf(stderr, "[exa_hip] %u of %u regions active for the volume march: %s walk (option walk = %d)\n", activeRegions, sc.numRegions,
                 ropeThisFrame ? "rope" : "stack", walkMode);
  if (ropeThisFrame && !ropeBuilt) {
    HIP_TRY(this, hipStreamSynchronize(s));
    if (buildRopes()) return 1;
    ropeThisFrame = ropeBuilt;
  }
  if (ropeThisFrame && ropeFlagsStale) {
    HIP_TRY(this, launchRopeActivity(ropeLeaves.p, sc.numRegions, volActive.p, 0, nullptr, s));
    ropeFlagsStale = false;
  }
  return 0;
}

int ExaHipRenderer::rebuildStreamlines(hipStream_t s)
{
  streamDirty = false;
  numStreamPrims = 0;
  if (!haveTracer) return 0;
  const int NT = tracer.numTimesteps;
  const long long nprims = (long long)tracer.numTraces * (NT - 1);
  const int timestep = std::min(this->timestep, NT);
  if (timestep < 2 || nprims <= 0) return 0;
  HIP_TRY(this, hipStreamSynchronize(s));
  std::vector<float> host(traces.n);
  HIP_TRY(this, hipMemcpy(host.data(), traces.p, traces.n * sizeof(float), hipMemcpyDeviceToHost));
  std::vector<float> boxes;
  std::vector<int32_t> prim;
  for (long long p = 0; p < nprims; p++) {
    if (int(p % NT) >= timestep - 1) continue;
    const float *pa = &host[3 * p], *pb = &host[3 * (p + 1)];
    if (!(pa[0] < 2e10f && pb[0] < 2e10f)) continue;
    for (int k = 0; k < 3; k++) boxes.push_back(std::fmin(pa[k] - 2.f, pb[k] - 2.f));
    for (int k = 0; k < 3; k++) boxes.push_back(std::fmax(pa[k] + 2.f, pb[k] + 2.f));
    prim.push_back((int32_t)p);
  }
  if (prim.empty()) return 0;
  LbvhTopology topo;
  topo.build(boxes.data(), prim.size());
  const std::vector<BvhNode> nodes = fillBoxes(topo, boxes, [&](size_t i) { return prim[i]; });
  HIP_TRY(this, streamNodes.upload(nodes.data(), nodes.size()));
  numStreamPrims = (int)prim.size();
  return 0;
}

int ExaHipRenderer::fillRenderArgs(RenderArgs &a, uint32_t *dstDevice, bool stats, hipStream_t s)
{
  a.sc = sc;
  a.volNodes = volNodes.p;
  a.isoNodes = isoNodes.p;
  a.fs = fs;
  a.p = p;
  a.xf = xf.p;
  a.tfFracMagic = tfFracMagic();
  a.fastSampler = fastSampler;
  a.mul24 = mul24; a.addr32 = addr64 ? 0 : addr32;
  a.cellsIl = ilChannels == p.numPrimaryChannels ? cellsIl.p : nullptr;
  a.il32 = (uint64_t(totalCells) + 2) * uint64_t(ilChannels > 0 ? ilChannels : 1) * sizeof(float) <= (1ull << 32) && !addr64 ? 1 : 0;
  {
    int e = 0;
    const float mant = std::frexp(p.dt, &e);
    a.invDtPow2 = (mant == 0.5f && e > -100 && e < 100) ? 1.f / p.dt : 0.f;
  }
  a.numXfChannels = numFields;
  a.W = W; a.H = H; a.tilesX = tilesX; a.tilesY = tilesY;
  a.rank = rank; a.world = world;
  a.tileMap = tileMap.p;
  a.color = dstDevice;
  a.colorRowMajor = colorRowMajor ? 1 : 0;
  a.accum = accum.p;
  a.surf = surf.p;
  a.surfRnd = surfRnd.p;
  a.stats = statsBuf.p;
  a.errorFlag = errorFlag.p;
  a.debugPixel = debugPixel;
  a.walkProbe = nullptr;
  if (stats && statsMode == 1 && walkProbeOn && useKd()) {
    const size_t need = size_t(numBlocks) * (256 / 64) * kWalkProbeSize;
    if (walkProbe.n != need) HIP_TRY(this, walkProbe.alloc(need));
    HIP_TRY(this, hipMemsetAsync(walkProbe.p, 0, need * sizeof(uint32_t), s));
    a.walkProbe = walkProbe.p;
  }
  a.tileCost = nullptr;
  a.tileCostPre = nullptr;
  if (feedback && costPhase == 1 && useKd() && measureCosts) {
    HIP_TRY(this, hipMemsetAsync(tileCost.p, 0, tileCost.n * sizeof(uint32_t), s));
    a.tileCost = tileCost.p;
    preMeasured = surfacesEnabled();
    if (preMeasured) {
      HIP_TRY(this, hipMemsetAsync(tileCostPre.p, 0, tileCostPre.n * sizeof(uint32_t), s));
      a.tileCostPre = tileCostPre.p;
    }
  }
  a.kdNodes = kdNodes.p;
  const bool packed = packRecords && kdMarchNodes.p != nullptr && !(stats && statsMode == 1);
  a.kdMarchNodes = packed ? kdMarchNodes.p : kdNodes.p;
  a.kdMarchRoot = packed ? kdMarchRoot : kdRoot;
  if (!rootLeafVolActive) a.kdMarchRoot = EXA_KD_EMPTY + 1;
  a.leafBeginBits = packed ? leafBeginBits : 0;
  a.leafSizeBits = packed ? leafSizeBits : 0;
  a.regionRec = regionRec.p;
  a.ropeLeaves = (ropeThisFrame && ropeBuilt) ? ropeLeaves.p : nullptr;
  a.ropeNodes = ropeNodes.p;
  a.ropeRoot = ropeRoot;
  a.ropeFastDiv = ropeFastDiv;
  a.ropeAddr32 = addr64 ? 0 : ropeAddr32;
  a.kdRoot = kdRoot;
  a.kdIsoRoot = rootLeafIsoActive ? kdRoot : EXA_KD_EMPTY + 1;
  for (int k = 0; k < 3; k++) { a.kdLo[k] = kdLo[k]; a.kdHi[k] = kdHi[k]; }
  worldBounds(a.worldLo, a.worldHi);
  a.meshNodes = meshNodes.p; a.meshVerts = meshVerts.p; a.meshTris = meshTris.p; a.numTris = numTris;
  a.streamNodes = streamNodes.p; a.traces = traces.p; a.numStreamPrims = numStreamPrims;
  for (int k = 0; k < 3; k++) a.tracerChannels[k] = tracer.channels[k];
  a.numTraces = tracer.numTraces; a.numTimesteps = tracer.numTimesteps; a.timestep = std::min(timestep, tracer.numTimesteps); a.steplen = tracer.steplen;
  return 0;
}

int ExaHipRenderer::prepareSurfaceLists(RenderArgs &a, bool stats, hipStream_t s)
{
  if (useKd() && surfacesEnabled() && surf.n != accum.n) {
    HIP_TRY(this, surf.alloc(accum.n));
    HIP_TRY(this, surfRnd.alloc(accum.n));
    a.surf = surf.p; a.surfRnd = surfRnd.p;
  }
  a.aoRecs = nullptr; a.aoCount = nullptr; a.aoKeys = nullptr; a.aoHist = nullptr; a.aoOrder = nullptr; a.aoHit = nullptr; a.aoBins = 0;
  if (!(useKd() && surfacesEnabled() && fs.ao.enabled && aoDefer && !stats)) return 0;
  const size_t recs = size_t(numBlocks) * kTilePixels;
  if (aoRecs.n != recs && aoRecs.alloc(recs) != hipSuccess) {
    (void)hipGetLastError();
    aoRecs.release();
    if (std::getenv("EXA_HIP_VERBOSE")) std::fprintf(stderr, "[exa_hip] no memory for the list of deferred AO rays (%zu records): traced inline\n", recs);
    return 0;
  }
  if (!aoCount.p) HIP_TRY(this, aoCount.alloc(8));
  HIP_TRY(this, hipMemsetAsync(aoCount.p, 0, 8 * sizeof(uint32_t), s));
  a.aoRecs = aoRecs.p; a.aoCount = aoCount.p;
  if (aoDefer == 2) {
    const uint32_t cells = world <= 1 ? uint32_t((W + 31) / 32) * uint32_t((H + 31) / 32) : uint32_t((numBlocks + 3) / 4);
    const uint32_t bins = std::max(1u, cells) * 24u;
    if (aoKeys.n != 2 * recs) { HIP_TRY(this, aoKeys.alloc(2 * recs)); HIP_TRY(this, aoOrder.alloc(2 * recs)); HIP_TRY(this, aoHit.alloc(2 * recs)); }
    if (aoBins != bins) { HIP_TRY(this, aoHist.alloc(2 * size_t(bins))); aoBins = bins; }
    a.aoKeys = aoKeys.p; a.aoOrder = aoOrder.p; a.aoHit = aoHit.p; a.aoHist = aoHist.p; a.aoBins = bins;
  }
  return 0;
}

hipError_t ExaHipRenderer::march(const RenderArgs &a, int n, bool surfArg, int statsArg, hipStream_t s)
{
  return (ropeThisFrame && ropeBuilt) ? EXA_FORM(this, launchRenderKdRope)(a, n, p.gradientShadingDVR != 0, fastMath != 0, surfArg, statsArg, s)
                                      : EXA_FORM(this, launchRenderKd)(a, n, p.gradientShadingDVR != 0, fastMath != 0, surfArg, statsArg, s);
}

int ExaHipRenderer::launchSurfaces(const RenderArgs &a, bool surfOn, bool stats, hipStream_t s)
{
  if (surfOn) HIP_TRY(this, EXA_FORM(this, launchSurfacePrepassKd)(a, numBlocks, stats, s));
  if (surfOn && !stats) HIP_TRY(this, EXA_FORM(this, launchAoRaysKd)(a, numBlocks, s));
  return 0;
}

int ExaHipRenderer::launchPlain(const RenderArgs &a, bool surfOn, bool stats, hipStream_t s)
{
  if (launchSurfaces(a, surfOn, stats, s)) return 1;
  HIP_TRY(this, march(a, numBlocks, surfOn, stats ? statsMode : 0, s));
  return 0;
}

int ExaHipRenderer::launchSplit(const RenderArgs &a, bool overlap, hipStream_t s)
{
  HIP_TRY(this, hipEventRecord(evFork, s));
  RenderArgs ah = a, ac = a;
  ac.tileMap = splitMap.p;
  ah.tileMap = splitMap.p + nPreCheap;
  if (a.aoRecs) {
    ah.aoRecs = a.aoRecs + size_t(nPreCheap) * kTilePixels;
    ah.aoCount = a.aoCount + 4;
    if (a.aoKeys) {
      const size_t off = 2 * size_t(nPreCheap) * kTilePixels;
      ah.aoKeys = a.aoKeys + off; ah.aoOrder = a.aoOrder + off; ah.aoHit = a.aoHit + off; ah.aoHist = a.aoHist + a.aoBins;
    }
  }
  HIP_TRY(this, hipStreamWaitEvent(side2, evFork, 0));
  HIP_TRY(this, EXA_FORM(this, launchSurfacePrepassKd)(ah, nPreHeavy, false, side2));
  HIP_TRY(this, hipStreamWaitEvent(sideN, evFork, 0));
  HIP_TRY(this, EXA_FORM(this, launchSurfacePrepassKd)(ac, nPreCheap, false, sideN));
  if (overlap) {
    HIP_TRY(this, hipEventRecord(evPre2, side2));
    HIP_TRY(this, hipEventRecord(evPre, sideN));
    HIP_TRY(this, hipStreamWaitEvent(side4, evPre2, 0));
    HIP_TRY(this, EXA_FORM(this, launchAoRaysKd)(ah, nPreHeavy, side4));
    HIP_TRY(this, hipEventRecord(evAo2, side4));
    HIP_TRY(this, hipStreamWaitEvent(side4, evPre, 0));
    HIP_TRY(this, EXA_FORM(this, launchAoRaysKd)(ac, nPreCheap, side4));
    HIP_TRY(this, hipEventRecord(evAo, side4));
  } else {
    HIP_TRY(this, EXA_FORM(this, launchAoRaysKd)(ah, nPreHeavy, side2));
    HIP_TRY(this, EXA_FORM(this, launchAoRaysKd)(ac, nPreCheap, sideN));
  }
  HIP_TRY(this, march(ac, nPreCheap, true, 0, sideN));
  if (overlap) {
    HIP_TRY(this, hipStreamWaitEvent(sideN, evAo, 0));
    HIP_TRY(this, EXA_FORM(this, launchCompositeKd)(ac, nPreCheap, sideN));
  }
  HIP_TRY(this, hipEventRecord(evJoinN, sideN));
  HIP_TRY(this, march(ah, nPreHeavy, true, 0, side2));
  if (overlap) {
    HIP_TRY(this, hipStreamWaitEvent(side2, evAo2, 0));
    HIP_TRY(this, EXA_FORM(this, launchCompositeKd)(ah, nPreHeavy, side2));
  }
  HIP_TRY(this, hipEventRecord(evJoin2, side2));
  HIP_TRY(this, hipStreamWaitEvent(s, evJoin2, 0));
  HIP_TRY(this, hipStreamWaitEvent(s, evJoinN, 0));
  return 0;
}

int ExaHipRenderer::launchOverlap(const RenderArgs &a, hipStream_t s)
{
  HIP_TRY(this, EXA_FORM(this, launchSurfacePrepassKd)(a, numBlocks, false, s));
  HIP_TRY(this, hipEventRecord(evPre, s));
  HIP_TRY(this, hipStreamWaitEvent(side4, evPre, 0));
  HIP_TRY(this, EXA_FORM(this, launchAoRaysKd)(a, numBlocks, side4));
  HIP_TRY(this, hipEventRecord(evAo, side4));
  HIP_TRY(this, march(a, numBlocks, true, 0, s));
  HIP_TRY(this, hipStreamWaitEvent(s, evAo, 0));
  HIP_TRY(this, EXA_FORM(this, launchCompositeKd)(a, numBlocks, s));
  return 0;
}

int ExaHipRenderer::launchWide(const RenderArgs &a, bool surfOn, hipStream_t s)
{
  if (launchSurfaces(a, surfOn, false, s)) return 1;
  HIP_TRY(this, hipEventRecord(evFork, s));
  RenderArgs aw = a;
  if (nWide4) {
    HIP_TRY(this, hipStreamWaitEvent(side4, evFork, 0));
    aw.wideTileMap = wideMap.p;
    aw.wideSegs = wideSegs.p;
    HIP_TRY(this, EXA_FORM(this, launchRenderKdWide)(aw, nWide4, lanesTopInUse, p.gradientShadingDVR != 0, fastMath != 0, surfOn, side4));
    HIP_TRY(this, hipEventRecord(evJoin4, side4));
  }
  if (nWide2) {
    HIP_TRY(this, hipStreamWaitEvent(side2, evFork, 0));
    aw.wideTileMap = wideMap.p + nWide4;
    aw.wideSegs = wideSegs.p + size_t(nWide4) * segsPerRay(lanesTopInUse) * kTilePixels;
    HIP_TRY(this, EXA_FORM(this, launchRenderKdWide)(aw, nWide2, 2, p.gradientShadingDVR != 0, fastMath != 0, surfOn, side2));
    HIP_TRY(this, hipEventRecord(evJoin2, side2));
  }
  RenderArgs an = a;
  an.tileMap = normalMap.p;
  HIP_TRY(this, hipStreamWaitEvent(sideN, evFork, 0));
  HIP_TRY(this, march(an, nNormal, surfOn, 0, sideN));
  HIP_TRY(this, hipEventRecord(evJoinN, sideN));
  if (nWide4) HIP_TRY(this, hipStreamWaitEvent(s, evJoin4, 0));
  if (nWide2) HIP_TRY(this, hipStreamWaitEvent(s, evJoin2, 0));
  HIP_TRY(this, hipStreamWaitEvent(s, evJoinN, 0));
  return 0;
}

int ExaHipRenderer::launch(uint32_t *dstDevice, bool stats, hipStream_t s)
{
  if (streamDirty && rebuildStreamlines(s)) return 1;
  RenderArgs a{};
  if (fillRenderArgs(a, dstDevice, stats, s)) return 1;
  if (haveTracer && tracer.enabled && timestep < tracer.numTimesteps && timestep >= 1) {
    const long long px = (long long)W * H;
    HIP_TRY(this, EXA_FORM(this, launchComputeTraces)(a, traces.p, (int)std::min<long long>(tracer.numTraces, px), s));
  }
  if (prepareSurfaceLists(a, stats, s)) return 1;
  HIP_TRY(this, hipEventRecord(ev0, s));
  if (useKd()) {
    const bool surfOn = surfacesEnabled();
    const bool wide = !stats && !emptyCells && nWide4 + nWide2 > 0 && p.numPrimaryChannels == 1 && a.debugPixel < 0;
    const bool split = surfOn && !stats && !wide && costPhase == 0 && !a.tileCost && nPreHeavy > 0 && nPreCheap > 0
                       && nPreHeavy + nPreCheap == numBlocks && a.debugPixel < 0;
    const bool overlap = aoOverlap && a.aoRecs && fs.ao.enabled && !wide && !(fs.clockScale > 0.f);
    if (overlap) {
      if (pixBuf.n != accum.n) HIP_TRY(this, pixBuf.alloc(accum.n));
      a.pixOut = pixBuf.p;
    }
    if (split) { if (launchSplit(a, overlap, s)) return 1; }
    else if (overlap) { if (launchOverlap(a, s)) return 1; }
    else if (wide) { if (launchWide(a, surfOn, s)) return 1; }
    else if (launchPlain(a, surfOn, stats, s)) return 1;
  } else {
    HIP_TRY(this, EXA_FORM(this, launchRender)(a, numBlocks, p.gradientShadingDVR != 0, surfacesEnabled(), stats, s));
  }
  last.node_bytes = useKd() ? sizeof(KdNodeDev) : sizeof(BvhNode);
  HIP_TRY(this, hipEventRecord(ev1, s));
  return 0;
}

int ExaHipRenderer::buildRopes()
{
  const auto tBuild0 = std::chrono::steady_clock::now();
  const size_t nk = kdNodes.n, nr = sc.numRegions;
  static_assert(sizeof(KdNodeDev) == sizeof(ExaKdNode), "the device's kd node is the ABI's with activity bits in the axis word");
  std::vector<ExaKdNode> kd(nk);
  std::vector<float> dom(6 * nr);
  std::vector<RegionInfo> ri(nr);
  if (nk) HIP_TRY(this, hipMemcpy(kd.data(), kdNodes.p, nk * sizeof(KdNodeDev), hipMemcpyDeviceToHost));
  HIP_TRY(this, hipMemcpy(dom.data(), domain.p, dom.size() * sizeof(float), hipMemcpyDeviceToHost));
  HIP_TRY(this, hipMemcpy(ri.data(), regionInfo.p, nr * sizeof(RegionInfo), hipMemcpyDeviceToHost));
  const unsigned nthreads = std::min(16u, std::max(1u, std::thread::hardware_concurrency()));
// ... 228 lines not shown
```

owlexabrick_amd/csrc/exa_kernels.hip:

```cpp
#include "exa_device.h"
#include <cfloat>

#if EXA_BASIS_FORM == 0 && EXA_EMPTY_CELLS
#define EXA_FORM_NS form0e
#elif EXA_BASIS_FORM == 0
#define EXA_FORM_NS form0
#elif EXA_BASIS_FORM == 1 && EXA_EMPTY_CELLS
#error "empty cells are a per-corner property: the per-axis association (EXA_BASIS_FORM 1) does not apply"
#elif EXA_BASIS_FORM == 1
#define EXA_FORM_NS form1
#else
#error "EXA_BASIS_FORM is 0 (source order) or 1 (per-axis association with fused multiply-adds)"
#endif
#define EXA_F1 (EXA_BASIS_FORM == 1)
#ifndef EXA_TU_ROPE
#define EXA_TU_ROPE 0
#endif
#ifndef EXA_TU_SAMPLE
#define EXA_TU_SAMPLE 0
#endif
#ifndef EXA_TU_STREAM
#define EXA_TU_STREAM 0
#endif
namespace exa {
// ... 1747 lines not shown
  }
}

__device__ __forceinline__ Ray aoRayOf(const ExaHipFrameState &fs, const float4 posFd, const float4 ngAmb, const float4 baseRnd, unsigned j)
{
  Lcg rnd;
  rnd.state = __float_as_uint(baseRnd.w);
  if (j & 1u) { rnd.next(); rnd.next(); }
  const V3 wN = mk(ngAmb.x, ngAmb.y, ngAmb.z);
  const V3 vN = fabsf(wN.x) > fabsf(wN.y) ? normalize(mk(-wN.z, 0.f, wN.x)) : normalize(mk(0.f, wN.z, -wN.y));
  const V3 uN = cross(vN, wN);
  const float u1 = rnd.next(), u2 = rnd.next();
  const float rr = sqrtf(u1);
  const float theta = 2.f * 3.14159265358979323846f * u2;
  const V3 sp = mk(rr * cosf(theta), rr * sinf(theta), sqrtf(1.f - u1));
  Ray ao_ray;
  ao_ray.org = mk(posFd.x, posFd.y, posFd.z);
  ao_ray.dir = normalize((sp.x * uN + sp.y * vN) + sp.z * wN);
  ao_ray.tmin = 1e-4f; ao_ray.tmax = fs.ao.length;
  return ao_ray;
}

enum { kAoDirClasses = 24, kAoCellShift = 5 };
__device__ __forceinline__ uint32_t aoRayKey(const RenderArgs &a, uint32_t slot, V3 d)
{
  const float ax = fabsf(d.x), ay = fabsf(d.y), az = fabsf(d.z);
  const uint32_t dom = (ax >= ay && ax >= az) ? 0u : (ay >= az ? 1u : 2u);
  const uint32_t oct = (d.x < 0.f ? 1u : 0u) | (d.y < 0.f ? 2u : 0u) | (d.z < 0.f ? 4u : 0u);
  uint32_t cell;
  if (a.world == 1) {
    const uint32_t px = slot % (uint32_t)a.W, py = slot / (uint32_t)a.W;
    cell = (py >> kAoCellShift) * (((uint32_t)a.W + 31u) >> kAoCellShift) + (px >> kAoCellShift);
  } else {
    cell = slot >> 10;
  }
  return cell * kAoDirClasses + oct * 3u + dom;
}
#if !EXA_TU_ROPE
__global__ __launch_bounds__(256) void aoKeyKernel(const RenderArgs a)
{
  const unsigned numRays = 2u * a.aoCount[0];
  for (unsigned j = blockIdx.x * 256u + threadIdx.x; j < numRays; j += gridDim.x * 256u) {
    const AoRecord *r = a.aoRecs + (j >> 1);
    const Ray ray = aoRayOf(a.fs, r->posFd, r->ngAmb, r->baseRnd, j);
    const uint32_t key = min(aoRayKey(a, r->slot, ray.dir), a.aoBins - 1u);
    a.aoKeys[j] = key;
    atomicAdd(&a.aoHist[key], 1u);
  }
}
__global__ __launch_bounds__(1024) void aoScanKernel(uint32_t *hist, uint32_t numBins)
{
  __shared__ uint32_t part[1024];
  const uint32_t per = (numBins + 1023u) / 1024u;
  const uint32_t b0 = min(threadIdx.x * per, numBins), b1 = min(b0 + per, numBins);
  uint32_t sum = 0;
  for (uint32_t b = b0; b < b1; b++) sum += hist[b];
  part[threadIdx.x] = sum;
  __syncthreads();
  for (uint32_t off = 1; off < 1024u; off <<= 1) {
    const uint32_t v = threadIdx.x >= off ? part[threadIdx.x - off] : 0u;
    __syncthreads();
    part[threadIdx.x] += v;
    __syncthreads();
  }
  uint32_t run = part[threadIdx.x] - sum;
  for (uint32_t b = b0; b < b1; b++) { const uint32_t c = hist[b]; hist[b] = run; run += c; }
}
__global__ __launch_bounds__(256) void aoScatterKernel(const RenderArgs a)
{
  const unsigned numRays = 2u * a.aoCount[0];
  for (unsigned j = blockIdx.x * 256u + threadIdx.x; j < numRays; j += gridDim.x * 256u)
    a.aoOrder[atomicAdd(&a.aoHist[a.aoKeys[j]], 1u)] = j;
}
__global__ __launch_bounds__(256) void aoFinalizeKernel(const RenderArgs a)
{
  const unsigned numHits = a.aoCount[0];
  for (unsigned h = blockIdx.x * 256u + threadIdx.x; h < numHits; h += gridDim.x * 256u) {
    const AoRecord *r = a.aoRecs + h;
    const float4 posFd = r->posFd, ngAmb = r->ngAmb, baseRnd = r->baseRnd;
    const uint32_t slot = r->slot;
    const int hitCnt = (int)a.aoHit[2u * h] + (int)a.aoHit[2u * h + 1u];
    const float shadow = (float)hitCnt / 2;
    const float fd = posFd.w;
    const float ns = 1.f - shadow;
    const float t_hit = a.surf[slot].w;
    a.surf[slot] = make_float4(ngAmb.w + baseRnd.x * fd * ns, ngAmb.w + baseRnd.y * fd * ns, ngAmb.w + baseRnd.z * fd * ns, t_hit);
  }
}

#endif

template <bool ISO_ONLY, bool SORTED>
__global__ __launch_bounds__(kKdBlock, (ISO_ONLY ? EXA_AO_ISO_WAVES : EXA_PREPASS_WAVES)) void aoRaysKdKernel(const RenderArgs a)
{
  extern __shared__ __attribute__((aligned(16))) unsigned char smem[];
  float4 *xfLds = reinterpret_cast<float4 *>(smem);
  unsigned char *sp0 = smem + size_t(a.numXfChannels) * EXA_NUM_XF_VALUES * sizeof(float4);
  int *stackRef = reinterpret_cast<int *>(sp0);
  float *stackF = reinterpret_cast<float *>(sp0 + size_t(kKdStackEntries) * kKdBlock * 4) + threadIdx.x;
  int *qRegion = reinterpret_cast<int *>(sp0 + size_t(kKdStack) * kKdBlock * 12) + threadIdx.x;
  float *qT = reinterpret_cast<float *>(sp0 + size_t(kKdStack) * kKdBlock * 12 + size_t(kSegQueue) * kKdBlock * 4) + threadIdx.x;
  for (int i = threadIdx.x; i < a.numXfChannels * EXA_NUM_XF_VALUES; i += kKdBlock) xfLds[i] = a.xf[i];
  __syncthreads();
  Ctx<0> C;
  C.a = &a;
  C.xfLds = xfLds;
  C.stack = stackRef + threadIdx.x;
  C.guardTripped = false;
  C.fastSampler = a.fastSampler != 0;
  const ExaHipFrameState &fs = a.fs;
  const unsigned numRays = 2u * a.aoCount[0];
  for (;;) {
    unsigned base = 0;
    if ((threadIdx.x & 63) == 0) base = atomicAdd(&a.aoCount[2], 64u);
    base = (unsigned)__shfl((int)base, 0, 64);
    if (base >= numRays) break;
    const unsigned k = base + (threadIdx.x & 63);
    const bool live = k < numRays;
    const unsigned j = (SORTED && live) ? a.aoOrder[k] : k;
    int hitFlag = 0;
    float4 posFd = make_float4(0.f, 0.f, 0.f, 0.f), ngAmb = posFd, baseRnd = posFd;
    uint32_t slot = 0;
    if (live) {
      const AoRecord *r = a.aoRecs + (j >> 1);
      posFd = r->posFd; ngAmb = r->ngAmb; baseRnd = r->baseRnd; slot = r->slot;
      const Ray ao_ray = aoRayOf(fs, posFd, ngAmb, baseRnd, j);
      SurfaceHit ao;
      traceSurfacesKd<0, ISO_ONLY>(C, ao_ray, ao, false, stackF, qRegion, qT);
      if (ao.primID >= 0 || ao.primID == EXA_PRIMID_ISOSURFACE || ao.primID == EXA_PRIMID_PLANE
          || ao.primID == EXA_PRIMID_STREAMLINE) hitFlag = 1;
      if (SORTED) a.aoHit[j] = (uint8_t)hitFlag;
    }
    if (SORTED) continue;
    const int other = __shfl_xor(hitFlag, 1, 64);
    if (live && !(j & 1u)) {
      const int hitCnt = hitFlag + other;
      const float shadow = (float)hitCnt / 2;
      const float fd = posFd.w;
      const float ns = 1.f - shadow;
      const float t_hit = a.surf[slot].w;
      a.surf[slot] = make_float4(ngAmb.w + baseRnd.x * fd * ns, ngAmb.w + baseRnd.y * fd * ns, ngAmb.w + baseRnd.z * fd * ns, t_hit);
    }
  }
  if (C.guardTripped) atomicExch(a.errorFlag, 1);
}

constexpr int marchWaves(int MULTI, int STATS, bool SMALL, int NCH, bool ROPE)
{
  return NCH ? (NCH == 2 ? EXA_IL2_WAVES : EXA_IL34_WAVES)
             : (MULTI == 1 ? EXA_MULTI_WAVES
                           : (MULTI ? 5 : ((ROPE && !STATS && SMALL && EXA_BASIS_FORM == 1) ? EXA_ROPE_WAVES : EXA_MARCH_WAVES)));
}

template <bool GRAD, bool FAST, int MULTI, bool SURF, int STATS, bool SMALL, int NCH = 0, bool ROPE = false>
__global__ __launch_bounds__(kKdBlock, marchWaves(MULTI, STATS, SMALL, NCH, ROPE)) void renderFrameKdKernel(const RenderArgs a)
{
  constexpr bool LEAN = marchWaves(MULTI, STATS, SMALL, NCH, ROPE) >= 7;
  constexpr int PACKED_CT = !ROPE ? -1 : (STATS == 1 ? 0 : (SMALL ? 1 : -1));
  const bool packedRec = PACKED_CT < 0 ? a.leafBeginBits != 0 : PACKED_CT != 0;
  static_assert(NCH == 0 || (MULTI == 2 && STATS == 0), "the interleaved march is a multi-channel variant of the shipped kernel");
  constexpr int KSB = MULTI == 1 ? kKdStackMulti : kKdStack;
  constexpr int KS = MULTI == 1 ? kKdStackMultiEntries : kKdStackEntries;
  constexpr int QN = ROPE ? (MULTI == 1 ? kRopeQueueMulti : kRopeQueue) : kSegQueue;
  static_assert(MULTI != 0 || (size_t(EXA_NUM_XF_VALUES) * sizeof(float4) + size_t(kKdBlock) * (ROPE ? QN * 16 : (KSB + QN) * 12))
                                  * marchWaves(MULTI, STATS, SMALL, NCH, ROPE) <= 160 * 1024,
                "LDS per workgroup x waves per SIMD exceeds the CU's 160 KB: shorten the queue or lower the occupancy");
  extern __shared__ __attribute__((aligned(16))) unsigned char smem[];
  float4 *xfLds = reinterpret_cast<float4 *>(smem);
  unsigned char *sp0 = smem + size_t(a.numXfChannels) * EXA_NUM_XF_VALUES * sizeof(float4);
  int *stackRef = reinterpret_cast<int *>(sp0);
  float *stackF = reinterpret_cast<float *>(sp0 + size_t(KS) * kKdBlock * 4) + threadIdx.x;
  unsigned char *q0 = ROPE ? sp0 : sp0 + size_t(KSB) * kKdBlock * 12;
  int *qRegion = reinterpret_cast<int *>(q0) + threadIdx.x;
  float *qT = reinterpret_cast<float *>(q0 + size_t(QN) * kKdBlock * 4) + threadIdx.x;
  float4 *queue4 = reinterpret_cast<float4 *>(sp0) + threadIdx.x;
  for (int i = threadIdx.x; i < a.numXfChannels * EXA_NUM_XF_VALUES; i += kKdBlock) xfLds[i] = a.xf[i];
  __syncthreads();

  Ctx<STATS> C;
  C.a = &a;
  C.xfLds = xfLds;
  C.stack = stackRef + threadIdx.x;
  C.guardTripped = false;
  const unsigned long long clockBegin = clock64();
  if (STATS) for (int i = 0; i < ST_COUNT; i++) C.st[i] = 0;
  __shared__ unsigned long long lapMarks[STATS == 2 ? 8 * (kKdBlock / 64) : 1];
  if (STATS == 2) {
    C.lapMark = lapMarks + 8 * (threadIdx.x >> 6);
    if ((threadIdx.x & 63) == 0) {
      C.lapMark[0] = clock64(); C.lapMark[1] = ST_T_OTHER - ST_T_BRICK;
      for (int i = 2; i < 7; i++) C.lapMark[i] = 0;
    }
  }

  const int wavesPerBlock = kKdBlock / 64;
  const int gwave = blockIdx.x * wavesPerBlock + (threadIdx.x >> 6);
  const int tile = a.tileMap[gwave >> 2];
  const int tx = tile % a.tilesX, ty = tile / a.tilesX;
  const int wave = gwave & 3, lane = threadIdx.x & 63;
  const int inX = ((wave & 1) << 3) + laneX(lane), inY = ((wave >> 1) << 3) + laneY(lane);
  const int px = tx * kTile + inX, py = ty * kTile + inY;
  const bool inside = px < a.W && py < a.H && (a.debugPixel < 0 || a.debugPixel == px + a.W * py);

  if (STATS == 1 && a.walkProbe) C.probe = a.walkProbe + size_t(gwave) * kWalkProbeSize;
  unsigned marchIters = 0;
  if (inside) {
    const ExaHipFrameState &fs = a.fs;
    const int frameID = fs.frameID;
    Lcg rnd;
    rnd.init((uint32_t)(frameID * a.W * a.H) + (uint32_t)px, (uint32_t)py);
    const float sx = float(px) + rnd.next();
    const float sy = float(py) + rnd.next();
    Ray ray;
    ray.org = mk(fs.cam_pos);
    ray.dir = normalize((mk(fs.cam_dir00) + sx * mk(fs.cam_dirDu)) + sy * mk(fs.cam_dirDv));
    ray.tmin = 1e-6f; ray.tmax = 1e8f;
    float surface_t_hit = ray.tmax;
    if (SURF) {
      const size_t slot0 = (a.world == 1) ? size_t(px) + size_t(a.W) * py
                                          : size_t(tile / a.world) * kTilePixels + (inY * kTile + inX);
      surface_t_hit = a.surf[slot0].w;
      rnd.state = a.surfRnd[slot0];
    }
    const float interleavedSamplingOffset = rnd.next();
    ray.tmax = surface_t_hit;
    if (fs.clipBox.enabled) {
      float c0, c1;
      boxTest(ray, mk(fs.clipBox.lo), mk(fs.clipBox.hi), c0, c1);
      ray.tmin = c0; ray.tmax = c1;
    }
    surface_t_hit = ray.tmax;
    ray.org = xfmPoint(fs, ray.org);
    ray.org.x = __int_as_float(__builtin_amdgcn_readfirstlane(__float_as_int(ray.org.x)));
    ray.org.y = __int_as_float(__builtin_amdgcn_readfirstlane(__float_as_int(ray.org.y)));
    ray.org.z = __int_as_float(__builtin_amdgcn_readfirstlane(__float_as_int(ray.org.z)));
    ray.dir = xfmVector(fs, ray.dir);
    const float dt_scale = length(ray.dir);
    ray.dir = normalize(ray.dir);
    ray.tmin = dt_scale * ray.tmin;
    ray.tmax = surface_t_hit * dt_scale;

    Color4 pixelColor; pixelColor.x = pixelColor.y = pixelColor.z = pixelColor.w = 0.f;
    const int numChannels = a.p.numPrimaryChannels;

    KdWalk w;
    w.pk.v = 0;
    {
      Ray whole = ray; whole.tmin = -INFINITY; whole.tmax = INFINITY;
      float r0, r1;
      const bool hit = boxTest(whole, mk(a.kdLo), mk(a.kdHi), r0, r1);
      w.tn = fmaxf(r0, ray.tmin);
      w.tf = fminf(r1, ray.tmax);
      w.tEnd = w.tf;
      w.ref = (hit && w.tn < w.tf) ? (ROPE ? a.ropeRoot : a.kdMarchRoot) : EXA_KD_DONE;
    }
    bool ropeFast = false;
    if (ROPE) ropeFast = a.ropeFastDiv != 0 && !anyLane(!ropeRayInRange(ray));

    float walkTmin = ray.tmin;

    bool haveSeg = false;
    int listBegin = 0, listSize = 0;
    float flcw = 1.f;
    float t1 = 0.f, t_i = 0.f, t_sample = 0.f, actual_dt = 0.f;
    int child = 0, chan = 0;
    int4 hb0 = make_int4(0, 0, 0, 1), hb1 = make_int4(1, 1, 1, 0);
    Basis B;
    B.sumWV = 0.f; B.sumW = 0.f; B.sumD = mk(0.f, 0.f, 0.f); B.sumDC = mk(0.f, 0.f, 0.f);
    float xWV[NCH > 1 ? NCH - 1 : 1];
    V3 xD[NCH > 1 ? NCH - 1 : 1];
#pragma unroll
    for (int c = 0; c < (NCH > 1 ? NCH - 1 : 1); c++) { xWV[c] = 0.f; xD[c] = mk(0.f, 0.f, 0.f); }
    const float *field0 = a.sc.scalars + a.sc.channelOffset[0];
    const float *field = field0;
    float xfRcpRange0 = 0.f, xfRange0 = 0.f;
    if (FAST && !MULTI) {
      xfRange0 = __int_as_float(__builtin_amdgcn_readfirstlane(__float_as_int((fs.xfDomain[0][1] - fs.xfDomain[0][0]) + 1e-20f)));
      xfRcpRange0 = __int_as_float(__builtin_amdgcn_readfirstlane(__float_as_int(__builtin_amdgcn_rcpf(xfRange0))));
    }
    float xfRcpRangeN[NCH ? NCH : 1], xfRangeN[NCH ? NCH : 1];
#pragma unroll
    for (int c = 0; c < (NCH ? NCH : 1); c++) {
      xfRangeN[c] = (FAST && NCH) ? __int_as_float(__builtin_amdgcn_readfirstlane(__float_as_int((fs.xfDomain[c][1] - fs.xfDomain[c][0]) + 1e-20f))) : 0.f;
      xfRcpRangeN[c] = (FAST && NCH) ? __int_as_float(__builtin_amdgcn_readfirstlane(__float_as_int(__builtin_amdgcn_rcpf(xfRangeN[c])))) : 0.f;
    }

    unsigned iter = 0;
    for (;; iter++) {
      if (iter == 0xfffffff0u) { C.guardTripped = true; break; }
      if (anyLane(!haveSeg && w.pk.get(PK_QCOUNT) == 0 && w.ref != EXA_KD_DONE)) {
        C.lap(ST_T_WALK);
        do {
          const bool want = w.pk.get(PK_QCOUNT) < QN && w.ref != EXA_KD_DONE;
          if (want) {
            if (ROPE) ropeStep<STATS, SMALL, QN, LEAN, PACKED_CT>(C, w, walkTmin, a, queue4, ray, ropeFast, interleavedSamplingOffset);
            else kdStep<false, STATS, SMALL, KS>(C, w, walkTmin, a, stackF, qRegion, qT, ray, 0, walkTmin, 1.f, a.kdMarchNodes, a.kdMarchRoot);
          }
        } while (anyLane(!haveSeg && w.pk.get(PK_QCOUNT) == 0 && w.ref != EXA_KD_DONE));
      }
      if (!haveSeg) {
        C.lap(ST_T_SEG);
        const int qc = w.pk.get(PK_QCOUNT);
        if (qc == 0) break;
        const int qh = w.pk.get(PK_QHEAD);
        int region;
        float t0, tiQueued = 0.f;
        if (ROPE) {
          const float4 e = queue4[qh * kKdBlock];
          region = __float_as_int(e.x); t1 = e.y; tiQueued = e.z; t0 = e.w;
        } else {
          region = qRegion[qh * kKdBlock];
          t0 = qT[(2 * qh) * kKdBlock];
          t1 = qT[(2 * qh + 1) * kKdBlock];
        }
        w.pk.template incWrap<QN>(PK_QHEAD);
        w.pk.dec(PK_QCOUNT);
        if (packedRec) {
          const unsigned d = (unsigned)region;
          listBegin = (int)(d & ((1u << a.leafBeginBits) - 1u));
          listSize = (int)((d >> a.leafBeginBits) & ((1u << a.leafSizeBits) - 1u)) + 1;
          flcw = __int_as_float((127 + (int)(d >> (a.leafBeginBits + a.leafSizeBits))) << 23);
        } else {
          const RegionInfo ri = a.sc.regionInfo[region];
          listBegin = ri.listBegin; listSize = ri.listSize;
          flcw = ri.finestLevelCellWidth;
        }
        C.count(ST_SEGMENTS);
        haveSeg = true;
        w.pk.setBit(PK_NEEDHDR);
        if (ROPE && packedRec)
          t_i = tiQueued;
        else if (a.invDtPow2 != 0.f)
          t_i = firstSampleTPow2(t0, a.p.dt * flcw, a.invDtPow2 * __int_as_float(0x7f000000 - __float_as_int(flcw)), interleavedSamplingOffset);
        else
          t_i = firstSampleT(t0, a.p.dt * flcw, interleavedSamplingOffset);
        {
          const float t_next = fminf(t_i, t1);
          t_sample = 0.5f * (fminf(t1, t_next) + t0);
          actual_dt = t_next - t0;
        }
        C.count(ST_SAMPLE_EVALS);
      }

      C.lap(ST_T_BRICK);
      C.phase(ST_W_BRICK);
      if (listSize > 1 || w.pk.get(PK_NEEDHDR)) {
        if (SMALL) {
          const char *hp = reinterpret_cast<const char *>(a.sc.leafHdr) + ((uint32_t)(listBegin + child) << 5);
          hb0 = *reinterpret_cast<const int4 *>(hp); hb1 = *reinterpret_cast<const int4 *>(hp + 16);
        } else {
          const unsigned at = 2u * (unsigned)(listBegin + child);
          hb0 = a.sc.leafHdr[at]; hb1 = a.sc.leafHdr[at + 1u];
        }
        w.pk.clearField(PK_NEEDHDR);
      }
      if (NCH) addBasisFastIl<GRAD, SMALL, (NCH ? NCH : 2)>(B, xWV, xD, hb0, hb1, a.cellsIl, rayAt(ray.org, t_sample, ray.dir));
      else addBasisFast<GRAD, STATS, SMALL>(C, B, hb0, hb1, MULTI ? field : field0, rayAt(ray.org, t_sample, ray.dir));
      child++;
      if (child < listSize) continue;

      C.lap(ST_T_FINAL);
      C.phase(ST_W_FINAL);
      if (NCH) {
        if (B.sumW > 1e-20f) {
#pragma unroll
          for (int c = 0; c < NCH; c++) {
            const float wv = c == 0 ? B.sumWV : xWV[c == 0 ? 0 : c - 1];
            const V3 sd = c == 0 ? B.sumD : xD[c == 0 ? 0 : c - 1];
            const float cellValue = fdivExact<FAST>(wv, B.sumW);
            V3 grad = mk(0.f, 0.f, 0.f);
            if (GRAD) grad = gradOf(B.sumW, wv, sd, B.sumDC);
            integrateVolume<FAST, STATS, FAST>(C, ray, pixelColor, actual_dt, cellValue, grad, flcw, c, xfRcpRangeN[c], xfRangeN[c]);
          }
        }
#pragma unroll
        for (int c = 0; c < (NCH > 1 ? NCH - 1 : 1); c++) { xWV[c] = 0.f; xD[c] = mk(0.f, 0.f, 0.f); }
      } else if (B.sumW > 1e-20f) {
        C.count(ST_SAMPLES);
        const float cellValue = fdivExact<FAST>(B.sumWV, B.sumW);
        V3 grad = mk(0.f, 0.f, 0.f);
        if (GRAD) grad = gradOf(B.sumW, B.sumWV, B.sumD, B.sumDC);
        integrateVolume<FAST, STATS, (FAST && !MULTI), LEAN>(C, ray, pixelColor, actual_dt, cellValue, grad, flcw, MULTI ? chan : 0, xfRcpRange0, xfRange0);
      }
      B.sumWV = 0.f; B.sumW = 0.f; B.sumD = mk(0.f, 0.f, 0.f); B.sumDC = mk(0.f, 0.f, 0.f);
      child = 0;
      if (MULTI && !NCH) {
        chan++;
        if (chan < numChannels) {
          field = a.sc.scalars + a.sc.channelOffset[chan];
          C.count(ST_SAMPLE_EVALS);
          continue;
        }
        chan = 0; field = field0;
      }
      if (pixelColor.w >= EXA_TERMINATION_THRESHOLD) {
        pixelColor.x = pixelColor.x * pixelColor.w;
        pixelColor.y = pixelColor.y * pixelColor.w;
        pixelColor.z = pixelColor.z * pixelColor.w;
        pixelColor.w = 1.f;
        break;
      }
      const float t_last = fminf(t_i, t1);
      if (t_last >= t1) {
        haveSeg = false;
        continue;
      }
      t_i += a.p.dt * flcw;
      {
        const float t_next = fminf(t_i, t1);
        t_sample = 0.5f * (fminf(t1, t_next) + t_last);
        actual_dt = t_next - t_last;
      }
      C.count(ST_SAMPLE_EVALS);
    }

    C.lap(ST_T_OTHER);
    marchIters = iter;
    size_t slot, colorSlot;
    {
      unsigned tid = threadIdx.x, bid = blockIdx.x;
      asm volatile("" : "+v"(tid));
      asm volatile("" : "+s"(bid));
      const int lane2 = tid & 63, wave2 = (tid >> 6) & 3;
      const int inX2 = ((wave2 & 1) << 3) + laneX(lane2), inY2 = ((wave2 >> 1) << 3) + laneY(lane2);
      slot = (a.world == 1) ? size_t(tx * kTile + inX2) + size_t(a.W) * (ty * kTile + inY2)
                            : size_t(a.tileMap[(bid * wavesPerBlock + (tid >> 6)) >> 2] / a.world) * kTilePixels + (inY2 * kTile + inX2);
      colorSlot = a.colorRowMajor ? size_t(tx * kTile + inX2) + size_t(a.W) * (ty * kTile + inY2) : slot;
    }
    if (SURF && a.pixOut) {
      a.pixOut[slot] = make_float4(pixelColor.x, pixelColor.y, pixelColor.z, pixelColor.w);
    } else {
    float4 bgColor = make_float4(0.f, 0.f, 0.f, 0.f);
    if (SURF) bgColor = a.surf[slot];
    float cr = pixelColor.w * pixelColor.x + (1.f - pixelColor.w) * bgColor.x;
    float cg = pixelColor.w * pixelColor.y + (1.f - pixelColor.w) * bgColor.y;
    float cb = pixelColor.w * pixelColor.z + (1.f - pixelColor.w) * bgColor.z;
    if (fs.clockScale > 0.f) cr = clockHeat(fs.clockScale, clockBegin);
    if (frameID > 0) {
      const float4 acc = a.accum[slot];
      cr += acc.x; cg += acc.y; cb += acc.z;
    }
    a.accum[slot] = make_float4(cr, cg, cb, 1.f);
    const float div = frameID + 1.f;
    cr = cr / div; cg = cg / div; cb = cb / div;
    a.color[colorSlot] = make_rgba8(linear_to_srgb(cr), linear_to_srgb(cg), linear_to_srgb(cb));
    }
  }

  if (a.tileCost) {
    unsigned v = marchIters;
    for (int off = 32; off > 0; off >>= 1) v = max(v, (unsigned)__shfl_down((int)v, off, 64));
    unsigned bid = blockIdx.x, tid = threadIdx.x;
    asm volatile("" : "+s"(bid));
    asm volatile("" : "+v"(tid));
    if (lane == 0) atomicMax(&a.tileCost[a.tileMap[(bid * wavesPerBlock + (tid >> 6)) >> 2]], v);
  }
  if (C.guardTripped) atomicExch(a.errorFlag, 1);
  if (STATS == 2) {
    if (lane < 5 && C.lapMark[2 + lane]) atomicAdd(&a.stats[ST_T_BRICK + lane], C.lapMark[2 + lane]);
  }
  if (STATS == 1) {
    for (int i = 0; i < ST_COUNT; i++) {
      unsigned long long v = inside ? C.st[i] : 0ull;
      for (int off = 32; off > 0; off >>= 1) v += __shfl_down(v, off, 64);
      if ((threadIdx.x & 63) == 0 && v) atomicAdd(&a.stats[i], v);
    }
    __shared__ unsigned wgMaxIters;
    if (threadIdx.x == 0) wgMaxIters = 0;
    __syncthreads();
    unsigned v = marchIters;
    for (int off = 32; off > 0; off >>= 1) v = max(v, (unsigned)__shfl_down((int)v, off, 64));
    if (lane == 0) atomicMax(&wgMaxIters, v);
    __syncthreads();
    if (lane == 0) atomicAdd(&a.stats[ST_WAVE_ITERS], (unsigned long long)v);
    if (threadIdx.x == 0) atomicAdd(&a.stats[ST_TILE_ITERS], 4ull * wgMaxIters);
  }
}

__device__ __forceinline__ void kdCollectStep(Ctx<0> &C, KdWalk &w, const float winLo, const float winHi, const RenderArgs &a,
                                              float *stackF, const Ray &ray, const KdNodeDev *nodes, const int root,
                                              float4 *out, unsigned &count)
{
  if (w.ref != EXA_KD_EMPTY && !(w.tn < winHi)) { w.ref = EXA_KD_DONE; return; }
  if (w.ref < 0 && w.ref > EXA_KD_DONE) {
    if (w.tn >= winLo && w.tn < w.tf) out[count++] = make_float4(__int_as_float(~w.ref), w.tn, w.tf, 0.f);
    w.ref = EXA_KD_EMPTY;
  }
  if (w.ref == EXA_KD_EMPTY || (w.ref != EXA_KD_DONE && !(w.tf > winLo))) kdPop(C, w, root, stackF, nodes, ray);
#define EXA_KD_POP_LATER() (w.ref = EXA_KD_EMPTY)
  if (w.ref < 0 || !(w.tf > winLo) || !(w.tn < winHi)) return;
  const int4 n = *reinterpret_cast<const int4 *>(nodes + w.ref);
  const float split = __int_as_float(n.x);
  const int axis = n.y & 3;
  const int bits = (n.y >> 2) & 3;
  const float ox = ray.org.x, oy = ray.org.y, oz = ray.org.z, dx = ray.dir.x, dy = ray.dir.y, dz = ray.dir.z;
  float o = axis == 0 ? ox : oy, d = axis == 0 ? dx : dy;
  o = axis == 2 ? oz : o;
  d = axis == 2 ? dz : d;
  if (d == 0.f) {
    if (o < split && (bits & 1)) w.ref = n.z;
    else if (o > split && (bits & 2)) w.ref = n.w;
    else EXA_KD_POP_LATER();
    return;
  }
  const float ts = (split - o) / d;
  const bool nearIsLeft = d > 0.f;
  const int nearRef = nearIsLeft ? n.z : n.w, farRef = nearIsLeft ? n.w : n.z;
  const bool nearAct = (bits & (nearIsLeft ? 1 : 2)) != 0, farAct = (bits & (nearIsLeft ? 2 : 1)) != 0;
  if (ts >= w.tf) {
    if (nearAct) w.ref = nearRef; else EXA_KD_POP_LATER();
  } else if (ts <= w.tn) {
    if (farAct) w.ref = farRef; else EXA_KD_POP_LATER();
  } else if (nearAct) {
    if (farAct) {
      const int head = w.pk.get(PK_SHEAD), count_ = w.pk.get(PK_SCOUNT);
      C.stack[head * kKdBlock] = farRef;
      stackF[(2 * head) * kKdBlock] = ts;
      stackF[(2 * head + 1) * kKdBlock] = w.tf;
      w.pk.template incWrap<kKdStackEntries>(PK_SHEAD);
      if (count_ == kKdStackEntries) w.pk.setBit(PK_DROPPED); else w.pk.inc(PK_SCOUNT);
    }
    w.ref = nearRef;
    w.tf = ts;
  } else if (farAct) {
    w.ref = farRef;
    w.tn = ts;
  } else {
    EXA_KD_POP_LATER();
  }
}
#undef EXA_KD_POP_LATER

template <bool GRAD, bool FAST, bool SURF, int L, bool SMALL>
__global__ __launch_bounds__(kKdBlock, 4) void renderFrameKdWideKernel(const RenderArgs a)
{
  extern __shared__ __attribute__((aligned(16))) unsigned char smem[];
  float4 *xfLds = reinterpret_cast<float4 *>(smem);
  unsigned char *sp0 = smem + size_t(a.numXfChannels) * EXA_NUM_XF_VALUES * sizeof(float4);
  int *stackRef = reinterpret_cast<int *>(sp0);
  float *stackF = reinterpret_cast<float *>(sp0 + size_t(kKdStackEntries) * kKdBlock * 4) + threadIdx.x;
  for (int i = threadIdx.x; i < a.numXfChannels * EXA_NUM_XF_VALUES; i += kKdBlock) xfLds[i] = a.xf[i];
  __syncthreads();

  Ctx<false> C;
  C.a = &a;
  C.xfLds = xfLds;
  C.stack = stackRef + threadIdx.x;
  C.guardTripped = false;
  const unsigned long long clockBegin = clock64();

  __builtin_amdgcn_s_setprio(3);
  const int tile = a.wideTileMap[blockIdx.x / L];
  const int part = blockIdx.x % L;
  const int tx = tile % a.tilesX, ty = tile / a.tilesX;
  const int lane = threadIdx.x & 63, sub = lane & (L - 1), lead = lane & ~(L - 1);
  const bool leader = sub == 0;
  const int r = part * (kTilePixels / L) + (threadIdx.x >> 6) * (64 / L) + lane / L;
  const int inX = (((r >> 6) & 1) << 3) + (r & 7), inY = ((r >> 7) << 3) + ((r >> 3) & 7);
  const int px = tx * kTile + inX, py = ty * kTile + inY;
  const bool inside = px < a.W && py < a.H && (a.debugPixel < 0 || a.debugPixel == px + a.W * py);

  unsigned myVisits = 0;
  if (inside) {
    const ExaHipFrameState &fs = a.fs;
    const int frameID = fs.frameID;
    Lcg rnd;
    rnd.init((uint32_t)(frameID * a.W * a.H) + (uint32_t)px, (uint32_t)py);
    const float sx = float(px) + rnd.next();
    const float sy = float(py) + rnd.next();
    Ray ray;
    ray.org = mk(fs.cam_pos);
    ray.dir = normalize((mk(fs.cam_dir00) + sx * mk(fs.cam_dirDu)) + sy * mk(fs.cam_dirDv));
    ray.tmin = 1e-6f; ray.tmax = 1e8f;
    const size_t slot = (a.world == 1) ? size_t(px) + size_t(a.W) * py
                                       : size_t(tile / a.world) * kTilePixels + (inY * kTile + inX);
    float surface_t_hit = ray.tmax;
    if (SURF) {
      surface_t_hit = a.surf[slot].w;
      rnd.state = a.surfRnd[slot];
    }
    const float interleavedSamplingOffset = rnd.next();
    ray.tmax = surface_t_hit;
    if (fs.clipBox.enabled) {
      float c0, c1;
      boxTest(ray, mk(fs.clipBox.lo), mk(fs.clipBox.hi), c0, c1);
      ray.tmin = c0; ray.tmax = c1;
    }
    surface_t_hit = ray.tmax;
    ray.org = xfmPoint(fs, ray.org);
    ray.dir = xfmVector(fs, ray.dir);
    const float dt_scale = length(ray.dir);
    ray.dir = normalize(ray.dir);
    ray.tmin = dt_scale * ray.tmin;
    ray.tmax = surface_t_hit * dt_scale;

    Color4 pixelColor; pixelColor.x = pixelColor.y = pixelColor.z = pixelColor.w = 0.f;

    float4 *const mySegs = a.wideSegs + (size_t(blockIdx.x / L) * kTilePixels * L + size_t(r) * L + sub) * kWideSegCap;
    unsigned myCount = 0;
    KdWalk w;
    w.pk.v = 0;
    float winLo, winHi;
    {
      Ray whole = ray; whole.tmin = -INFINITY; whole.tmax = INFINITY;
      float r0, r1;
      const bool hit = boxTest(whole, mk(a.kdLo), mk(a.kdHi), r0, r1);
      w.tn = fmaxf(r0, ray.tmin);
      w.tf = fminf(r1, ray.tmax);
      w.tEnd = w.tf;
      w.ref = (hit && w.tn < w.tf) ? a.kdMarchRoot : EXA_KD_DONE;
      const float span = w.tf - w.tn;
      winLo = sub == 0 ? -INFINITY : w.tn + span * (float(sub) / float(L));
      winHi = sub == L - 1 ? INFINITY : w.tn + span * (float(sub + 1) / float(L));
      for (unsigned g = 0;; g++) {
        if (g == 0xfffffff0u) { C.guardTripped = true; break; }
        const bool want = w.ref != EXA_KD_DONE && myCount < kWideSegCap;
        if (!anyLane(want)) break;
        if (want) kdCollectStep(C, w, winLo, winHi, a, stackF, ray, a.kdMarchNodes, a.kdMarchRoot, mySegs, myCount);
      }
    }
    __builtin_amdgcn_fence(__ATOMIC_RELEASE, "wavefront");
    __builtin_amdgcn_fence(__ATOMIC_ACQUIRE, "wavefront");
    float walkTmin = ray.tmin;
    int curWin = 0;
    unsigned curIdx = 0, curCount = (unsigned)__shfl((int)myCount, lead, 64);
    const float4 *curSegs = a.wideSegs + (size_t(blockIdx.x / L) * kTilePixels * L + size_t(r) * L) * kWideSegCap;

    bool haveSeg = false, newStep = false, needHdr = false, mine = false;
    int listBegin = 0, listSize = 0;
// ... 108 lines not shown
          Color4 o;
          o.x = __shfl(smp.x, lead + s, 64); o.y = __shfl(smp.y, lead + s, 64);
          o.z = __shfl(smp.z, lead + s, 64); o.w = __shfl(smp.w, lead + s, 64);
          const int oc = __shfl(contributes, lead + s, 64);
          if (!rayDone && !segDone) {
            const float tn = fminf(ti, t1);
            if (oc) compositeSample(pixelColor, o);
            if (pixelColor.w >= EXA_TERMINATION_THRESHOLD) rayDone = true;
            else if (tn >= t1) segDone = true;
            tl = tn;
            ti = ti + dtSeg;
          }
        }
        tiBase = ti; tlBase = tl;
      }
      if (rayDone) {
        pixelColor.x = pixelColor.x * pixelColor.w;
        pixelColor.y = pixelColor.y * pixelColor.w;
        pixelColor.z = pixelColor.z * pixelColor.w;
        pixelColor.w = 1.f;
        break;
      }
      if (segDone) haveSeg = false;
      else newStep = true;
    }

    if (leader) {
      float4 bgColor = make_float4(0.f, 0.f, 0.f, 0.f);
      if (SURF) bgColor = a.surf[slot];
      float cr = pixelColor.w * pixelColor.x + (1.f - pixelColor.w) * bgColor.x;
      float cg = pixelColor.w * pixelColor.y + (1.f - pixelColor.w) * bgColor.y;
      float cb = pixelColor.w * pixelColor.z + (1.f - pixelColor.w) * bgColor.z;
      if (fs.clockScale > 0.f) cr = clockHeat(fs.clockScale, clockBegin);
      if (frameID > 0) {
        const float4 acc = a.accum[slot];
        cr += acc.x; cg += acc.y; cb += acc.z;
      }
      a.accum[slot] = make_float4(cr, cg, cb, 1.f);
      const float div = frameID + 1.f;
      cr = cr / div; cg = cg / div; cb = cb / div;
      a.color[a.colorRowMajor ? size_t(px) + size_t(a.W) * py : slot] = make_rgba8(linear_to_srgb(cr), linear_to_srgb(cg), linear_to_srgb(cb));
    }
  }
  if (a.tileCost) {
    unsigned v = myVisits;
    for (int off = 1; off < L; off <<= 1) v += (unsigned)__shfl_xor((int)v, off, 64);
    for (int off = 32; off > 0; off >>= 1) v = max(v, (unsigned)__shfl_down((int)v, off, 64));
    if (lane == 0) atomicMax(&a.tileCost[tile], v);
  }
  if (C.guardTripped) atomicExch(a.errorFlag, 1);
}

#if !EXA_TU_ROPE
__global__ __launch_bounds__(256) void compositeKdKernel(const RenderArgs a)
{
  const int tile = a.tileMap[blockIdx.x];
  const int tx = tile % a.tilesX, ty = tile / a.tilesX;
  const int inX = threadIdx.x & 15, inY = threadIdx.x >> 4;
  const int px = tx * kTile + inX, py = ty * kTile + inY;
  if (!(px < a.W && py < a.H) || !(a.debugPixel < 0 || a.debugPixel == px + a.W * py)) return;
  const size_t slot = (a.world == 1) ? size_t(px) + size_t(a.W) * py : size_t(tile / a.world) * kTilePixels + (inY * kTile + inX);
  const size_t colorSlot = a.colorRowMajor ? size_t(px) + size_t(a.W) * py : slot;
  const float4 pixelColor = a.pixOut[slot];
  const float4 bgColor = a.surf[slot];
  const int frameID = a.fs.frameID;
  float cr = pixelColor.w * pixelColor.x + (1.f - pixelColor.w) * bgColor.x;
  float cg = pixelColor.w * pixelColor.y + (1.f - pixelColor.w) * bgColor.y;
  float cb = pixelColor.w * pixelColor.z + (1.f - pixelColor.w) * bgColor.z;
  if (frameID > 0) {
    const float4 acc = a.accum[slot];
    cr += acc.x; cg += acc.y; cb += acc.z;
  }
  a.accum[slot] = make_float4(cr, cg, cb, 1.f);
  const float div = frameID + 1.f;
  cr = cr / div; cg = cg / div; cb = cb / div;
  a.color[colorSlot] = make_rgba8(linear_to_srgb(cr), linear_to_srgb(cg), linear_to_srgb(cb));
}
hipError_t launchCompositeKd(const RenderArgs &a, int numBlocks, hipStream_t s)
{
  if (numBlocks <= 0) return hipSuccess;
  hipLaunchKernelGGL(compositeKdKernel, dim3(numBlocks), dim3(256), 0, s, a);
  return hipGetLastError();
}

hipError_t launchRenderKdWide(const RenderArgs &a, int numTiles, int lanesPerRay, bool grad, bool fast, bool surf, hipStream_t s)
{
  if (numTiles <= 0) return hipSuccess;
#if EXA_EMPTY_CELLS
  return hipErrorNotSupported;
#else
  const size_t lds = size_t(a.numXfChannels) * EXA_NUM_XF_VALUES * sizeof(float4) + size_t(kKdStack + kSegQueue) * kKdBlock * 12;
  const dim3 grid(numTiles * lanesPerRay), block(kKdBlock);
  const bool small = a.mul24 && a.addr32;
#define EXA_W4(G, F, S, L) do { if (small) hipLaunchKernelGGL((renderFrameKdWideKernel<G, F, S, L, true>), grid, block, lds, s, a); \
                                else hipLaunchKernelGGL((renderFrameKdWideKernel<G, F, S, L, false>), grid, block, lds, s, a); } while (0)
#define EXA_W3(G, F, S) do { if (lanesPerRay == 2) EXA_W4(G, F, S, 2); else EXA_W4(G, F, S, 4); } while (0)
#define EXA_W2(G, F) do { if (surf) EXA_W3(G, F, true); else EXA_W3(G, F, false); } while (0)
  if (grad) { if (fast) EXA_W2(true, true); else EXA_W2(true, false); }
  else      { if (fast) EXA_W2(false, true); else EXA_W2(false, false); }
#undef EXA_W4
#undef EXA_W2
#undef EXA_W3
  return hipGetLastError();
#endif
}

hipError_t launchSurfacePrepassKd(const RenderArgs &a, int numBlocks, bool stats, hipStream_t s)
{
  if (numBlocks <= 0) return hipSuccess;
  const size_t lds = size_t(a.numXfChannels) * EXA_NUM_XF_VALUES * sizeof(float4) + size_t(kKdStack + kSegQueue) * kKdBlock * 12;
  const dim3 grid(numBlocks * (256 / kKdBlock)), block(kKdBlock);
  bool isoOnly = a.numTris == 0 && a.numStreamPrims == 0;
  for (int i = 0; i < EXA_MAX_CONTOUR_PLANES; i++) isoOnly = isoOnly && !a.fs.contour[i].enabled;
  const bool defer = !stats && a.aoRecs && a.aoCount;
  if (stats)        hipLaunchKernelGGL((surfacePrepassKdKernel<1, false, false>), grid, block, lds, s, a);
  else if (isoOnly) { if (defer) hipLaunchKernelGGL((surfacePrepassKdKernel<0, true, true>), grid, block, lds, s, a);
                      else       hipLaunchKernelGGL((surfacePrepassKdKernel<0, true, false>), grid, block, lds, s, a); }
  else              { if (defer) hipLaunchKernelGGL((surfacePrepassKdKernel<0, false, true>), grid, block, lds, s, a);
                      else       hipLaunchKernelGGL((surfacePrepassKdKernel<0, false, false>), grid, block, lds, s, a); }
  return hipGetLastError();
}

hipError_t launchAoRaysKd(const RenderArgs &a, int numBlocks, hipStream_t s)
{
  if (numBlocks <= 0) return hipSuccess;
  const size_t lds = size_t(a.numXfChannels) * EXA_NUM_XF_VALUES * sizeof(float4) + size_t(kKdStack + kSegQueue) * kKdBlock * 12;
  const dim3 block(kKdBlock);
  bool isoOnly = a.numTris == 0 && a.numStreamPrims == 0;
  for (int i = 0; i < EXA_MAX_CONTOUR_PLANES; i++) isoOnly = isoOnly && !a.fs.contour[i].enabled;
  const bool defer = a.aoRecs && a.aoCount;
  if (defer && a.fs.ao.enabled) {
    const int maxBlocks = 256 * (isoOnly ? EXA_AO_ISO_WAVES : EXA_PREPASS_WAVES);
    const long long upper = ((long long)numBlocks * kTilePixels * 2 + kKdBlock - 1) / kKdBlock;
    const dim3 g2((unsigned)(upper < maxBlocks ? upper : maxBlocks));
    if (a.aoKeys) {
      const dim3 gs((unsigned)(upper < 2048 ? upper : 2048)), b256(256);
      if (hipError_t e = hipMemsetAsync(a.aoHist, 0, size_t(a.aoBins) * sizeof(uint32_t), s)) return e;
      hipLaunchKernelGGL(aoKeyKernel, gs, b256, 0, s, a);
      hipLaunchKernelGGL(aoScanKernel, dim3(1), dim3(1024), 0, s, a.aoHist, a.aoBins);
      hipLaunchKernelGGL(aoScatterKernel, gs, b256, 0, s, a);
      if (isoOnly) hipLaunchKernelGGL((aoRaysKdKernel<true, true>), g2, block, lds, s, a);
      else         hipLaunchKernelGGL((aoRaysKdKernel<false, true>), g2, block, lds, s, a);
      hipLaunchKernelGGL(aoFinalizeKernel, gs, b256, 0, s, a);
    } else {
      if (isoOnly) hipLaunchKernelGGL((aoRaysKdKernel<true, false>), g2, block, lds, s, a);
      else         hipLaunchKernelGGL((aoRaysKdKernel<false, false>), g2, block, lds, s, a);
    }
  }
  return hipGetLastError();
}

#endif

template <bool ROPE>
static hipError_t launchRenderKdT(const RenderArgs &a, int numBlocks, bool grad, bool fast, bool surf, int stats, hipStream_t s)
{
  if (numBlocks <= 0) return hipSuccess;
#ifndef EXA_LDS_PAD
#define EXA_LDS_PAD 0
#endif
  const int mode = a.p.numPrimaryChannels > 1 ? ((a.numXfChannels <= 2 && !stats) ? 1 : 2) : 0;
  const int nch = (!EXA_EMPTY_CELLS && a.cellsIl && !stats && a.p.numPrimaryChannels >= 2 && a.p.numPrimaryChannels <= 4) ? a.p.numPrimaryChannels : 0;
  const size_t perLane = ROPE ? size_t(mode == 1 && !nch ? kRopeQueueMulti : kRopeQueue) * 16
                              : size_t((mode == 1 && !nch ? kKdStackMulti : kKdStack) + kSegQueue) * 12;
  const size_t lds = size_t(a.numXfChannels) * EXA_NUM_XF_VALUES * sizeof(float4) + perLane * kKdBlock + EXA_LDS_PAD;
  const dim3 grid(numBlocks * (256 / kKdBlock)), block(kKdBlock);
  const bool small = a.mul24 && a.addr32 && (!ROPE || (a.ropeAddr32 && a.leafBeginBits));
#define EXA_LAUNCH(G, F, M, I, S, A) hipLaunchKernelGGL((renderFrameKdKernel<G, F, M, I, S, A, 0, ROPE>), grid, block, lds, s, a)
#define EXA_PICK2(G, F, M, I) do { if (stats == 1) EXA_LAUNCH(G, F, (M ? 2 : 0), I, 1, false); else if (stats == 2) EXA_LAUNCH(G, F, (M ? 2 : 0), I, 2, false); \
                                   else if (small) EXA_LAUNCH(G, F, M, I, 0, true); else EXA_LAUNCH(G, F, M, I, 0, false); } while (0)
#define EXA_PICK(G, F, M) do { if (surf) EXA_PICK2(G, F, M, true); else EXA_PICK2(G, F, M, false); } while (0)
#define EXA_PICKM(G, F) do { if (mode == 0) EXA_PICK(G, F, 0); else if (mode == 1) EXA_PICK(G, F, 1); else EXA_PICK(G, F, 2); } while (0)
#if !EXA_EMPTY_CELLS
  if (nch) {
    const bool smallIl = small && a.il32;
#define EXA_IL4(G, F, I, A, N) hipLaunchKernelGGL((renderFrameKdKernel<G, F, 2, I, 0, A, N, ROPE>), grid, block, lds, s, a)
#define EXA_IL3(G, F, I, A) do { if (nch == 2) EXA_IL4(G, F, I, A, 2); else if (nch == 3) EXA_IL4(G, F, I, A, 3); else EXA_IL4(G, F, I, A, 4); } while (0)
#define EXA_IL2(G, F, I) do { if (smallIl) EXA_IL3(G, F, I, true); else EXA_IL3(G, F, I, false); } while (0)
#define EXA_IL1(G, F) do { if (surf) EXA_IL2(G, F, true); else EXA_IL2(G, F, false); } while (0)
    if (grad) { if (fast) EXA_IL1(true, true); else EXA_IL1(true, false); }
    else      { if (fast) EXA_IL1(false, true); else EXA_IL1(false, false); }
#undef EXA_IL1
#undef EXA_IL2
#undef EXA_IL3
#undef EXA_IL4
    return hipGetLastError();
  }
#endif
  if (grad) { if (fast) EXA_PICKM(true, true); else EXA_PICKM(true, false); }
  else      { if (fast) EXA_PICKM(false, true); else EXA_PICKM(false, false); }
#undef EXA_PICKM
#undef EXA_PICK
#undef EXA_PICK2
#undef EXA_LAUNCH
  return hipGetLastError();
}
#if EXA_TU_ROPE
hipError_t launchRenderKdRope(const RenderArgs &a, int numBlocks, bool grad, bool fast, bool surf, int stats, hipStream_t s)
{ return launchRenderKdT<true>(a, numBlocks, grad, fast, surf, stats, s); }
#else
hipError_t launchRenderKd(const RenderArgs &a, int numBlocks, bool grad, bool fast, bool surf, int stats, hipStream_t s)
{ return launchRenderKdT<false>(a, numBlocks, grad, fast, surf, stats, s); }
#endif

}

#if EXA_BASIS_FORM == 0 && !EXA_EMPTY_CELLS && !EXA_TU_ROPE
using namespace form0;
__global__ __launch_bounds__(256) void kdRefitKernel(KdNodeDev *nodes, KdNodeDev *marchNodes, const int32_t *nodeIds, int count,
                                                     const uint8_t *active, int which)
{
  const int i = blockIdx.x * 256 + threadIdx.x;
  if (i >= count) return;
  const int id = nodeIds[i];
  const KdNodeDev n = nodes[id];
  const int sh = 2 + 2 * which;
  auto act = [&](int ref) -> uint32_t {
    if (ref == EXA_KD_EMPTY) return 0u;
    if (ref < 0) return active[~ref] ? 1u : 0u;
    return ((nodes[ref].word >> sh) & 3u) ? 1u : 0u;
  };
  const uint32_t bits = act(n.left) | (act(n.right) << 1);
  const uint32_t word = (n.word & ~(3u << sh)) | (bits << sh);
  nodes[id].word = word;
  if (marchNodes) marchNodes[id].word = word;
}

hipError_t launchKdRefit(KdNodeDev *nodes, KdNodeDev *marchNodes, const int32_t *nodeIds, int count, const uint8_t *active, int which, hipStream_t s)
{
  if (count <= 0) return hipSuccess;
  hipLaunchKernelGGL(kdRefitKernel, dim3((count + 255) / 256), dim3(256), 0, s, nodes, marchNodes, nodeIds, count, active, which);
  return hipGetLastError();
}

__global__ __launch_bounds__(256) void ropeActivityKernel(RopeLeaf *leaves, uint32_t numRegions, const uint8_t *active, int which, uint32_t *activeCount)
{
  const uint32_t r = blockIdx.x * 256u + threadIdx.x;
  const bool act = r < numRegions && active[r] != 0;
  if (leaves && r < numRegions) {
    const uint32_t f = leaves[r].flags;
    leaves[r].flags = (f & ~(1u << which)) | ((act ? 1u : 0u) << which);
  }
  if (activeCount) {
    const unsigned long long m = __ballot(act);
    if ((threadIdx.x & 63) == 0 && m) atomicAdd(activeCount, (uint32_t)__popcll(m));
  }
}
hipError_t launchRopeActivity(RopeLeaf *leaves, uint32_t numRegions, const uint8_t *active, int which, uint32_t *activeCount, hipStream_t s)
{
  if (numRegions == 0) return hipSuccess;
  hipLaunchKernelGGL(ropeActivityKernel, dim3((numRegions + 255) / 256), dim3(256), 0, s, leaves, numRegions, active, which, activeCount);
  return hipGetLastError();
}
#endif

#if !EXA_TU_ROPE
namespace EXA_FORM_NS {

__device__ __forceinline__ bool sampleDirection(Ctx<false> &C, V3 pos, V3 &result)
{
  Ray ray; ray.org = pos; ray.dir = mk(1.f, 1.f, 1.f); ray.tmin = 0.f; ray.tmax = 2e-10f;
  const RegionHit prd = traceRegion(C, C.a->volNodes, ray);
  result = mk(0.f, 0.f, 0.f);
  if (prd.leafID < 0) return false;
  const RegionInfo ri = C.a->sc.regionInfo[prd.leafID];
  V3 unused;
  float r0 = 0.f, r1 = 0.f, r2 = 0.f;
  bool ok = samplePoint<false, false>(C, r0, unused, ri, pos, C.a->tracerChannels[0]);
  if (ok) ok = samplePoint<false, false>(C, r1, unused, ri, pos, C.a->tracerChannels[1]);
  if (ok) ok = samplePoint<false, false>(C, r2, unused, ri, pos, C.a->tracerChannels[2]);
  result = mk(r0, r1, r2);
  return ok;
}

__global__ __launch_bounds__(256) void computeTracesKernel(const RenderArgs a, float *traces, int count)
{
  __shared__ int stackLds[kStackDepth * 256];
  const int i = blockIdx.x * 256 + threadIdx.x;
  Ctx<false> C;
  C.a = &a; C.xfLds = nullptr; C.stack = stackLds + threadIdx.x; C.guardTripped = false;
  if (i >= count) return;
  const int t = a.timestep, NT = a.numTimesteps;
  if (!(t < NT)) return;
  V3 p = mk(traces + 3 * (size_t(i) * NT + (t - 1)));
  const V3 pp = p;
  if (p.x < 2e10f) {
    bool valid = true;
    V3 k1, k2, k3, k4;
    valid &= sampleDirection(C, p, k1);
    k1 = a.steplen * k1;
    const V3 ptry1 = p + .5f * k1;
    valid &= sampleDirection(C, ptry1, k2);
    k2 = a.steplen * k2;
    const V3 ptry2 = p + .5f * k2;
    valid &= sampleDirection(C, ptry2, k3);
    k3 = a.steplen * k3;
    const V3 ptry3 = p + k3;
    valid &= sampleDirection(C, ptry3, k4);
    k4 = a.steplen * k4;
    p = p + (1 / 6.f) * (((k1 + 2.f * k2) + 2.f * k3) + k4);
    const bool inside = p.x >= a.worldLo[0] && p.y >= a.worldLo[1] && p.z >= a.worldLo[2]
                     && p.x <= a.worldHi[0] && p.y <= a.worldHi[1] && p.z <= a.worldHi[2];
    if (!valid || !inside || length(p - pp) < 1e-10f) p = mk(2e10f, 2e10f, 2e10f);
  }
  float *dst = traces + 3 * (size_t(i) * NT + t);
  dst[0] = p.x; dst[1] = p.y; dst[2] = p.z;
}

hipError_t launchComputeTraces(const RenderArgs &a, float *traces, int count, hipStream_t s)
{
  if (count <= 0) return hipSuccess;
  hipLaunchKernelGGL(computeTracesKernel, dim3((count + 255) / 256), dim3(256), 0, s, a, traces, count);
  return hipGetLastError();
}

}
#endif

#if EXA_BASIS_FORM == 0 && !EXA_EMPTY_CELLS && !EXA_TU_ROPE
__global__ __launch_bounds__(256) void volumeActivityKernel(DeviceScene sc, ExaHipFrameState fs, ExaHipParams p,
                                                            const float4 *xf, uint8_t *active, float tfFracMagic)
{
  extern __shared__ __attribute__((aligned(16))) unsigned char smem[];
  float4 *xfLds = reinterpret_cast<float4 *>(smem);
  for (int i = threadIdx.x; i < p.numChannels * EXA_NUM_XF_VALUES; i += 256) xfLds[i] = xf[i];
  __syncthreads();
  const uint32_t r = blockIdx.x * 256u + threadIdx.x;
  if (r >= sc.numRegions) return;
  const float2 vr = sc.valueRange[r];
  bool act = false;
  for (int c = 0; c < p.numChannels && !act; ++c) {
    const float dlo = fs.xfDomain[c][0], dhi = fs.xfDomain[c][1];
    if (vr.x > dhi) continue;
    if (vr.y < dlo) continue;
    const float scaled_lo = (vr.x - dlo) / ((dhi - dlo) + 1e-20f);
    const float scaled_hi = (vr.y - dlo) / ((dhi - dlo) + 1e-20f);
    const int idx_lo = min(EXA_NUM_XF_VALUES - 1, max(0, int(scaled_lo * (EXA_NUM_XF_VALUES - 1))));
    const int idx_hi = min(EXA_NUM_XF_VALUES - 1, max(0, int(scaled_hi * (EXA_NUM_XF_VALUES - 1)) + 1));
    for (int i = idx_lo; i <= idx_hi; i++) {
      float cellValue = float(i) / (EXA_NUM_XF_VALUES - 1);
      cellValue *= dhi - dlo;
      cellValue += dlo;
      const Color4 rgba = lookupXF(xfLds, fs, cellValue, c, tfFracMagic);
      if (rgba.w > 0.f) { act = true; break; }
    }
  }
  active[r] = (uint8_t)(p.spaceSkippingEnabled ? (act ? 1 : 0) : 1);
}

__global__ __launch_bounds__(256) void isoActivityKernel(DeviceScene sc, ExaHipFrameState fs, uint8_t *active)
{
  const uint32_t r = blockIdx.x * 256u + threadIdx.x;
  if (r >= sc.numRegions) return;
  const float2 vr = sc.valueRange[r];
  bool act = false;
  for (int i = 0; i < EXA_MAX_ISO_SURFACES; i++)
    if (fs.iso[i].enabled && fs.iso[i].value >= vr.x && fs.iso[i].value <= vr.y) act = true;
  active[r] = act ? 1 : 0;
}

hipError_t launchVolumeActivity(const DeviceScene &sc, const ExaHipFrameState &fs, const ExaHipParams &p,
                                const float4 *xf, uint8_t *active, float tfFracMagic, hipStream_t s)
{
  if (sc.numRegions == 0) return hipSuccess;
  const size_t lds = size_t(p.numChannels) * EXA_NUM_XF_VALUES * sizeof(float4);
  hipLaunchKernelGGL(volumeActivityKernel, dim3((sc.numRegions + 255) / 256), dim3(256), lds, s, sc, fs, p, xf, active, tfFracMagic);
  return hipGetLastError();
}
hipError_t launchIsoActivity(const DeviceScene &sc, const ExaHipFrameState &fs, uint8_t *active, hipStream_t s)
{
  if (sc.numRegions == 0) return hipSuccess;
  hipLaunchKernelGGL(isoActivityKernel, dim3((sc.numRegions + 255) / 256), dim3(256), 0, s, sc, fs, active);
  return hipGetLastError();
}

__device__ __forceinline__ void childBox(const BvhNode *nodes, int child, const float *domain, const uint8_t *active,
                                         float lo[3], float hi[3])
{
  lo[0] = lo[1] = lo[2] = FLT_MAX;
  hi[0] = hi[1] = hi[2] = -FLT_MAX;
  if (child == INT32_MIN) return;
  if (child < 0) {
    const int r = ~child;
    if (!active[r]) return;
    for (int k = 0; k < 3; k++) { lo[k] = domain[6 * size_t(r) + k]; hi[k] = domain[6 * size_t(r) + 3 + k]; }
    return;
  }
  const BvhNode &n = nodes[child];
  const float l0[3] = { n.q0.x, n.q0.y, n.q0.z }, h0[3] = { n.q0.w, n.q1.x, n.q1.y };
  const float l1[3] = { n.q1.z, n.q1.w, n.q2.x }, h1[3] = { n.q2.y, n.q2.z, n.q2.w };
  const bool e0 = l0[0] > h0[0], e1 = l1[0] > h1[0];
  for (int k = 0; k < 3; k++) {
    if (!e0) { lo[k] = fminf(lo[k], l0[k]); hi[k] = fmaxf(hi[k], h0[k]); }
    if (!e1) { lo[k] = fminf(lo[k], l1[k]); hi[k] = fmaxf(hi[k], h1[k]); }
  }
}

__global__ __launch_bounds__(256) void refitKernel(BvhNode *nodes, const int32_t *nodeIds, int count,
                                                   const float *domain, const uint8_t *active)
{
  const int i = blockIdx.x * 256 + threadIdx.x;
  if (i >= count) return;
  const int id = nodeIds[i];
  BvhNode n = nodes[id];
  float l0[3], h0[3], l1[3], h1[3];
  childBox(nodes, n.child0, domain, active, l0, h0);
  childBox(nodes, n.child1, domain, active, l1, h1);
  n.q0 = make_float4(l0[0], l0[1], l0[2], h0[0]);
  n.q1 = make_float4(h0[1], h0[2], l1[0], l1[1]);
  n.q2 = make_float4(l1[2], h1[0], h1[1], h1[2]);
  nodes[id] = n;
}

hipError_t launchRefit(BvhNode *nodes, const int32_t *nodeIds, int count, const float *domain,
                       const uint8_t *active, hipStream_t s)
{
  if (count <= 0) return hipSuccess;
  hipLaunchKernelGGL(refitKernel, dim3((count + 255) / 256), dim3(256), 0, s, nodes, nodeIds, count, domain, active);
  return hipGetLastError();
}

__global__ __launch_bounds__(256) void permuteBricksKernel(const float *src, float *dst, const uint32_t *srcBegin, const uint32_t *dstBegin,
                                                           const int4 *bricks, unsigned long long totalCells, int numFields)
{
  const size_t b = blockIdx.x;
  const int4 b0 = bricks[2 * b], b1 = bricks[2 * b + 1];
  const unsigned long long vol = (unsigned long long)b0.w * (unsigned long long)b1.x * (unsigned long long)b1.y;
  const unsigned long long sb = srcBegin[b], db = dstBegin[b];
  for (int f = 0; f < numFields; f++)
    for (unsigned long long i = threadIdx.x; i < vol; i += 256) dst[f * totalCells + db + i] = src[f * totalCells + sb + i];
}
__global__ __launch_bounds__(256) void patchBeginKernel(int4 *bricks, unsigned long long numBricks, int4 *leafHdr, const int32_t *leafList,
                                                        unsigned long long leafListSize, const uint32_t *dstBegin)
{
  const unsigned long long i = blockIdx.x * 256ull + threadIdx.x;
  if (i < numBricks) bricks[2 * i + 1].w = (int)dstBegin[i];
  if (i < leafListSize) leafHdr[2 * i + 1].w = (int)dstBegin[leafList[i]];
}
hipError_t launchPermuteBricks(const float *src, float *dst, const uint32_t *srcBegin, const uint32_t *dstBegin, int4 *bricks,
                               unsigned long long numBricks, int4 *leafHdr, const int32_t *leafList, unsigned long long leafListSize,
                               unsigned long long totalCells, int numFields, hipStream_t s)
{
  if (numBricks == 0) return hipSuccess;
  hipLaunchKernelGGL(permuteBricksKernel, dim3((unsigned)numBricks), dim3(256), 0, s, src, dst, srcBegin, dstBegin, bricks, totalCells, numFields);
  const unsigned long long n = numBricks > leafListSize ? numBricks : leafListSize;
  hipLaunchKernelGGL(patchBeginKernel, dim3((unsigned)((n + 255) / 256)), dim3(256), 0, s, bricks, numBricks, leafHdr, leafList, leafListSize, dstBegin);
  return hipGetLastError();
}

__global__ __launch_bounds__(256) void interleaveKernel(DeviceScene sc, unsigned long long totalCells, int nch, float *out)
{
  const unsigned long long n = totalCells * (unsigned long long)nch;
  for (unsigned long long i = blockIdx.x * 256ull + threadIdx.x; i < n; i += (unsigned long long)gridDim.x * 256ull) {
    const unsigned long long cell = i / (unsigned)nch;
    const int c = (int)(i - cell * (unsigned)nch);
    out[i] = sc.scalars[sc.channelOffset[c] + cell];
  }
}

hipError_t launchInterleave(const DeviceScene &sc, unsigned long long totalCells, int nch, float *out, hipStream_t s)
{
  if (totalCells == 0) return hipSuccess;
  hipLaunchKernelGGL(interleaveKernel, dim3(256 * 64), dim3(256), 0, s, sc, totalCells, nch, out);
  return hipGetLastError();
}

__global__ __launch_bounds__(256) void untileKernel(const uint32_t *gathered, unsigned long long shardStride,
                                                    int world, int W, int H, int tilesX, uint32_t *out)
{
  const int tile = blockIdx.x;
  const int tx = tile % tilesX, ty = tile / tilesX;
  const int inX = threadIdx.x & 15, inY = threadIdx.x >> 4;
  const int px = tx * kTile + inX, py = ty * kTile + inY;
  if (px >= W || py >= H) return;
  const int rank = tile % world;
  out[size_t(px) + size_t(W) * py]
      = gathered[size_t(rank) * shardStride + size_t(tile / world) * kTilePixels + (inY * kTile + inX)];
}

hipError_t launchUntile(const uint32_t *gathered, unsigned long long shardStride, int world,
                        int W, int H, uint32_t *out, hipStream_t s)
{
  const int tilesX = (W + kTile - 1) / kTile, tilesY = (H + kTile - 1) / kTile;
  hipLaunchKernelGGL(untileKernel, dim3(tilesX * tilesY), dim3(256), 0, s, gathered, shardStride, world, W, H, tilesX, out);
  return hipGetLastError();
}

__global__ void profileMarkerKernel(int tag) { (void)tag; }
hipError_t launchProfileMarker(int tag, hipStream_t s)
{
  hipLaunchKernelGGL(profileMarkerKernel, dim3(1), dim3(1), 0, s, tag);
  return hipGetLastError();
}
#endif
#endif
}
```

owlexabrick_amd/csrc/exa_module.cpp:

```cpp
#include "exa_renderer.h"
#include "exa_hostbvh.h"

#include <cmath>
#include <cstring>

namespace {

bool isMulti(const ExaHipRenderer *h) { return h && !h->children.empty(); }

template <typename Call>
int onChild(ExaHipRenderer *h, ExaHipRenderer *c, Call call)
{
  const int rc = call(c);
  if (rc) h->fail(c->err);
  return rc;
}

template <typename Call>
int onEveryChild(ExaHipRenderer *h, Call call)
{
  for (ExaHipRenderer *c : h->children)
    if (int rc = onChild(h, c, call)) return rc;
  return 0;
}
// ... 60 lines not shown
  h->numTris = 0;
  h->meshNodes.release(); h->meshVerts.release(); h->meshTris.release();
  if (numTris == 0) return 0;
  if (!vertices || !triangles || numTris > 0x3fffffffull) { h->fail("exa_hip_set_triangles: bad arguments"); return 1; }
  for (uint64_t i = 0; i < 3 * numTris; i++)
    if (triangles[i] < 0 || uint64_t(triangles[i]) >= numVertices) { h->fail("broken triangle model"); return 1; }
  std::vector<float> boxes(6 * numTris);
  for (uint64_t t = 0; t < numTris; t++)
    for (int k = 0; k < 3; k++) {
      const float a = vertices[3 * triangles[3 * t] + k], b = vertices[3 * triangles[3 * t + 1] + k], c = vertices[3 * triangles[3 * t + 2] + k];
      const float lo = std::fmin(a, std::fmin(b, c)), hi = std::fmax(a, std::fmax(b, c));
      const float pad = 1e-5f * std::fmax(std::fmax(std::fabs(lo), std::fabs(hi)), hi - lo) + 1e-30f;
      boxes[6 * t + k] = lo - pad; boxes[6 * t + 3 + k] = hi + pad;
    }
  LbvhTopology topo;
  topo.build(boxes.data(), numTris);
  const std::vector<BvhNode> nodes = fillBoxes(topo, boxes, [](size_t t) { return t; });
  HIP_TRY(h, h->meshNodes.upload(nodes.data(), nodes.size()));
  HIP_TRY(h, h->meshVerts.upload(vertices, 3 * numVertices));
  HIP_TRY(h, h->meshTris.upload(triangles, 3 * numTris));
  h->numTris = (int)numTris;
  return 0;
}

int exa_hip_reset_tracer(ExaHipRenderer *h, const ExaHipTracer *t, const float *seeds)
{
  if (isMulti(h)) return onEveryChild(h, [&](ExaHipRenderer *c) { return exa_hip_reset_tracer(c, t, seeds); });
  if (!h || !t || !seeds) return 1;
  if (t->numTraces < 0 || t->numTimesteps < 2 || (long long)t->numTraces * t->numTimesteps > (1ll << 28)) { h->fail("exa_hip_reset_tracer: bad trace counts"); return 1; }
  for (int k = 0; k < 3; k++)
    if (t->channels[k] < 0 || t->channels[k] >= h->numFields) { h->fail("exa_hip_reset_tracer: tracer channel out of range"); return 1; }
  EXA_ON_DEVICE(h);
  HIP_TRY(h, hipDeviceSynchronize());
  h->tracer = *t;
  h->haveTracer = true;
  std::vector<float> host(size_t(t->numTraces) * t->numTimesteps * 3, 0.f);
  for (int i = 0; i < t->numTraces; i++) std::memcpy(&host[size_t(i) * t->numTimesteps * 3], &seeds[3 * i], 3 * sizeof(float));
  HIP_TRY(h, h->traces.upload(host.data(), host.size()));
  h->timestep = 0;
  h->streamDirty = true;
  return 0;
}

int exa_hip_set_tracer_enabled(ExaHipRenderer *h, int32_t enabled)
{
  if (isMulti(h)) return onEveryChild(h, [&](ExaHipRenderer *c) { return exa_hip_set_tracer_enabled(c, enabled); });
  if (!h) return 1;
  h->tracer.enabled = enabled;
  return 0;
}

int exa_hip_advance_tracer(ExaHipRenderer *h, int32_t *rebuild)
{
  if (isMulti(h))
    return onEveryChild(h, [&](ExaHipRenderer *c) { return exa_hip_advance_tracer(c, c == firstChild(h) ? rebuild : nullptr); });
  if (!h) return 1;
  if (rebuild) *rebuild = 0;
  if (!h->haveTracer || !h->tracer.enabled) return 0;
  h->timestep++;
  if (h->timestep <= h->tracer.numTimesteps) h->streamDirty = true;
  if (rebuild) *rebuild = h->streamDirty;
  return 0;
}

int exa_hip_read_traces(ExaHipRenderer *h, float *dst)
{
  if (isMulti(h))
    return onChild(h, firstChild(h), [&](ExaHipRenderer *c) { return exa_hip_read_traces(c, dst); });
  if (!h || !dst || !h->haveTracer) return 1;
  EXA_ON_DEVICE(h);
  HIP_TRY(h, hipDeviceSynchronize());
  HIP_TRY(h, hipMemcpy(dst, h->traces.p, h->traces.n * sizeof(float), hipMemcpyDeviceToHost));
  return 0;
}

int exa_hip_set_params(ExaHipRenderer *h, const ExaHipParams *p)
{
  if (isMulti(h)) return onEveryChild(h, [&](ExaHipRenderer *c) { return exa_hip_set_params(c, p); });
  if (!h || !p) return 1;
  if (!(p->dt > 0.f)) { h->fail("exa_hip_set_params: dt must be > 0"); return 1; }
  if (!h->haveParams || h->p.numChannels != p->numChannels || h->p.spaceSkippingEnabled != p->spaceSkippingEnabled)
    h->volDirty = true;
  if (!h->haveParams || std::memcmp(&h->p, p, sizeof(*p)) != 0) h->costPhase = 1;
  h->p = *p;
  h->haveParams = true;
  return 0;
}

int exa_hip_set_shard(ExaHipRenderer *h, int32_t rank, int32_t worldSize)
{
  if (isMulti(h)) { h->fail("exa_hip_set_shard: a multi-device handle shards the frame internally"); return 1; }
  if (!h) return 1;
  if (worldSize < 1 || rank < 0 || rank >= worldSize) { h->fail("exa_hip_set_shard: bad rank/world"); return 1; }
  h->rank = rank; h->world = worldSize;
  h->layoutDirty = true;
  if (h->W > 0) { EXA_ON_DEVICE(h); return h->rebuildLayout(); }
  return 0;
}

int exa_hip_set_option(ExaHipRenderer *h, const char *key, int32_t value)
{
  if (isMulti(h)) return onEveryChild(h, [&](ExaHipRenderer *c) { return exa_hip_set_option(c, key, value); });
  if (!h || !key) return 1;
  if (!std::strcmp(key, "tile_order")) { h->tileOrder = value; h->layoutDirty = true; return 0; }
  if (!std::strcmp(key, "tile_feedback")) { h->feedback = value; h->layoutDirty = true; return 0; }
  if (!std::strcmp(key, "wide_march")) {
    if (value != 0 && value != 1 && value != 2 && value != 4) { h->fail("exa_hip_set_option: wide_march is 0, 1, 2 or 4"); return 1; }
    h->wideMode = value; h->layoutDirty = true; return 0;
  }
  if (!std::strcmp(key, "stats_mode")) {
    if (value != 1 && value != 2) { h->fail("exa_hip_set_option: stats_mode is 1 or 2"); return 1; }
    h->statsMode = value; return 0;
  }
  if (!std::strcmp(key, "ao_defer")) {
    if (value < 0 || value > 2) { h->fail("exa_hip_set_option: ao_defer is 0, 1 or 2"); return 1; }
    h->aoDefer = value; return 0;
  }
  if (!std::strcmp(key, "prepass_split")) { h->prepassSplit = value != 0; h->costPhase = 1; return 0; }
  if (!std::strcmp(key, "ao_overlap")) { h->aoOverlap = value != 0; return 0; }
  if (!std::strcmp(key, "walk_probe")) { h->walkProbeOn = value != 0; return 0; }
  if (!std::strcmp(key, "debug_pixel")) { h->debugPixel = value; return 0; }
  if (!std::strcmp(key, "profile_marker")) {
    EXA_ON_DEVICE(h);
    if (launchProfileMarker(value, nullptr) != hipSuccess) { h->fail("exa_hip_set_option: profile_marker launch failed"); return 1; }
    return 0;
  }
  if (!std::strcmp(key, "accel")) { h->accel = value; return 0; }
  if (!std::strcmp(key, "walk")) {
    if (value < 0 || value > 2) { h->fail("exa_hip_set_option: walk is 0 (chosen per frame), 1 (stack walk) or 2 (rope walk)"); return 1; }
    h->walkMode = value; return 0;
  }
  if (!std::strcmp(key, "lbvh_build")) {
    if (h->lbvhBuilt && value != h->lbvhOnHost) { h->fail("exa_hip_set_option: lbvh_build must be set before the LBVH is first used"); return 1; }
    h->lbvhOnHost = value; return 0;
  }
  if (!std::strcmp(key, "fast_math")) { h->fastMath = value; return 0; }
  if (!std::strcmp(key, "fast_sampler")) { h->fastSampler = value; return 0; }
  if (!std::strcmp(key, "basis_form")) {
    if (value != 0 && value != 1) { h->fail("exa_hip_set_option: basis_form is 0 or 1"); return 1; }
    if (value && h->emptyCells) {
      h->fail("exa_hip_set_option: a scene with empty cells keeps basis_form 0 (an empty cell is a per-corner property, the per-axis association needs per-axis ones)");
      return 1;
    }
    h->basisForm = value; return 0;
  }
  if (!std::strcmp(key, "sample_patch")) {
    if (value < 0 || value >= kSamplePatchShapes) { h->fail("exa_hip_set_option: sample_patch is 0 (64x1x1), 1 (16x4x1), 2 (8x8x1) or 3 (4x4x4)"); return 1; }
    h->samplePatch = value; return 0;
  }
  if (!std::strcmp(key, "sample_uniform")) { h->sampleUniform = value != 0; return 0; }
  if (!std::strcmp(key, "interleave")) { h->interleave = value != 0; return 0; }
  if (!std::strcmp(key, "addr64")) { h->addr64 = value != 0; return 0; }
  if (!std::strcmp(key, "pack_records")) { h->packRecords = value != 0; return 0; }
  if (!std::strcmp(key, "brick_order")) {
    if (value && !h->brickOrderPossible) {
      h->fail("exa_hip_set_option: brick_order 1 needs channel offsets f * totalCells and brick begins that partition [0, totalCells)");
      return 1;
    }
    h->brickOrderWanted = value != 0; return 0;
  }
  if (!std::strcmp(key, "tf_filter")) {
    if (value != 0 && value != 1) { h->fail("exa_hip_set_option: tf_filter is 0 or 1"); return 1; }
    if (value != h->tfFilter) { h->tfFilter = value; h->volDirty = true; }
    return 0;
  }
  h->fail(std::string("exa_hip_set_option: unknown key ") + key);
  return 1;
}

int exa_hip_read_activity(ExaHipRenderer *h, int32_t which, uint8_t *dst)
{
  if (isMulti(h)) return onChild(h, firstChild(h), [&](ExaHipRenderer *c) { return exa_hip_read_activity(c, which, dst); });
  if (!h || !dst) return 1;
  EXA_ON_DEVICE(h);
  if (h->prepareFrame(nullptr)) return 1;
  if (which == 1 && !h->isoEnabled()) {
    HIP_TRY(h, launchIsoActivity(h->sc, h->fs, h->isoActive.p, nullptr));
  }
  HIP_TRY(h, hipDeviceSynchronize());
  HIP_TRY(h, hipMemcpy(dst, which ? h->isoActive.p : h->volActive.p, h->sc.numRegions, hipMemcpyDeviceToHost));
  return 0;
}

}
```

owlexabrick_amd/csrc/exa_renderer.h:

```cpp
#pragma once
#include "exa_device.h"
#include "exa_ropes.h"

#include <algorithm>
#include <string>
#include <utility>
#include <vector>

using namespace exa;

#define EXA_FORM(r, fn) ((r)->emptyCells ? form0e::fn : ((r)->basisForm ? form1::fn : form0::fn))

#define HIP_TRY(h, call)                                                                   \
  do {                                                                                     \
    hipError_t e_ = (call);                                                                \
    if (e_ != hipSuccess) {                                                                \
      (h)->fail(std::string(#call) + ": " + hipGetErrorString(e_));                        \
      return 1;                                                                            \
    }                                                                                      \
  } while (0)

extern thread_local std::string g_createError;

struct DeviceGuard {
  int prev = -1;
  hipError_t err;
  explicit DeviceGuard(int device)
  {
    if (hipGetDevice(&prev) != hipSuccess) prev = -1;
    err = hipSetDevice(device);
  }
  ~DeviceGuard() { if (prev >= 0) (void)hipSetDevice(prev); }
  DeviceGuard(const DeviceGuard &) = delete;
  DeviceGuard &operator=(const DeviceGuard &) = delete;
};
#define EXA_ON_DEVICE(h) EXA_ON_DEVICE_OF(h, h)
#define EXA_ON_DEVICE_OF(h, r) DeviceGuard guard_((r)->device); HIP_TRY(h, guard_.err)

template <typename T>
struct DevBuf {
  T *p = nullptr;
  size_t n = 0;
  hipError_t alloc(size_t count)
  {
    release();
    n = count;
    if (count == 0) return hipSuccess;
    return hipMalloc((void **)&p, count * sizeof(T) + 16);
  }
  hipError_t upload(const T *src, size_t count)
  {
    hipError_t e = alloc(count);
    if (e != hipSuccess || count == 0) return e;
    return hipMemcpy(p, src, count * sizeof(T), hipMemcpyHostToDevice);
  }
  hipError_t refill(const T *src, size_t count)
  {
    if (count > cap || !p) {
      hipError_t e = alloc(std::max(count, size_t(1)));
      if (e != hipSuccess) return e;
      cap = std::max(count, size_t(1));
    }
    n = count;
    return count ? hipMemcpy(p, src, count * sizeof(T), hipMemcpyHostToDevice) : hipSuccess;
  }
  size_t cap = 0;
  void release() { if (p) (void)hipFree(p); p = nullptr; n = 0; cap = 0; }
  ~DevBuf() { release(); }
};

struct ExaHipRenderer {
  int device = 0;
  std::string err;
  void fail(const std::string &m) { err = m; }

  std::vector<ExaHipRenderer *> children;
  bool colorRowMajor = false;
  hipStream_t ownStream = nullptr;
  hipEvent_t evCall = nullptr;

  DevBuf<int4> bricks;
  DevBuf<int32_t> leafList;
  DevBuf<int4> leafHdr;
  DevBuf<float> scalars;
  DevBuf<float> cellsIl;
  int ilChannels = 0;
  int ilNoMemory = 0;
  int interleave = 1;
  bool emptyCells = false;
  int basisForm = 1;
  int addr64 = 0;
  int packRecords = 1;
  uint64_t totalCells = 0;
  std::vector<uint32_t> beginUploaded, beginMorton;
  int brickOrder = 0, brickOrderWanted = 0;
  bool brickOrderPossible = true;
  uint64_t numBricks = 0, leafListSize = 0;
  int applyBrickOrder(hipStream_t s);
  DevBuf<RegionInfo> regionInfo;
  DevBuf<float2> valueRange;
  DevBuf<float> domain;
  DeviceScene sc{};
  int numFields = 0;

  DevBuf<KdNodeDev> kdNodes;
  DevBuf<KdNodeDev> kdMarchNodes;
  int32_t kdMarchRoot = 0;
  uint32_t leafBeginBits = 0, leafSizeBits = 0;
  DevBuf<RegionRec> regionRec;
  DevBuf<int32_t> kdLevelIds;
  std::vector<int> kdLevelBegin;
  int32_t kdRoot = EXA_KD_EMPTY;
  bool rootLeafVolActive = true, rootLeafIsoActive = true;
  bool haveKd = false;
  int accel = 1;
  float kdLo[3], kdHi[3];

  DevBuf<RopeLeaf> ropeLeaves;
  DevBuf<KdNodeDev> ropeNodes;
  DevBuf<uint32_t> activeCountBuf;
  int32_t ropeRoot = EXA_KD_EMPTY + 1;
  bool ropeBuilt = false, ropeFailed = false, ropeFlagsStale = true, ropeThisFrame = false;
  int ropeFastDiv = 0, ropeAddr32 = 0;
  int walkMode = 0;
  uint32_t activeRegions = 0;
  static constexpr double kRopeActiveFraction = 0.4;
  bool ropeWanted() const
  {
    if (!useKd() || ropeFailed || walkMode == 1) return false;
    if (walkMode == 2) return true;
    return double(activeRegions) >= kRopeActiveFraction * double(sc.numRegions);
  }
  int buildRopes();

  DevBuf<BvhNode> meshNodes;
  DevBuf<float> meshVerts;
  DevBuf<int32_t> meshTris;
  int numTris = 0;

  ExaHipTracer tracer{};
  bool haveTracer = false;
  DevBuf<float> traces;
  DevBuf<BvhNode> streamNodes;
  int numStreamPrims = 0, timestep = 0;
  bool streamDirty = false;
  int rebuildStreamlines(hipStream_t s);

  DevBuf<BvhNode> volNodes, isoNodes;
  DevBuf<int32_t> levelIds;
  DevBuf<uint8_t> volActive, isoActive;
  bool volDirty = true, isoDirty = true;

  DevBuf<float4> xf;
  float xfHost[EXA_MAX_CHANNELS][EXA_NUM_XF_VALUES][4];
  bool xfDirty = true;
  ExaHipFrameState fs{};
  ExaHipParams p{};
  bool haveFs = false, haveParams = false;

  int W = 0, H = 0, tilesX = 0, tilesY = 0;
  int rank = 0, world = 1;
  int tileOrder = 4;
  int debugPixel = -1;
  int fastMath = 1;
  int mul24 = 0, addr32 = 0;
  int fastSampler = 1;
  int tfFilter = 1;
  float tfFracMagic() const { return tfFilter ? 32768.f : 0.f; }
  DevBuf<float4> accum;
  DevBuf<float4> surf;
  DevBuf<uint32_t> tileCost;
  DevBuf<uint32_t> tileCostPre;
  DevBuf<int32_t> splitMap;
  int nPreCheap = 0, nPreHeavy = 0;
  int prepassSplit = 1;
  bool preMeasured = false;
  std::vector<int32_t> baseMap, curMap;
  int feedback = 1;
  int statsMode = 1;
  int costPhase = 0;
  int wideMode = 1;
  static size_t segsPerRay(int lanes) { return size_t(lanes) * kWideSegCap; }
  int numSimdWaves = 256 * 4 * 6;
  DevBuf<int32_t> normalMap, wideMap;
  DevBuf<float4> wideSegs;
  int nNormal = 0, nWide4 = 0, nWide2 = 0;
  int lanesTopInUse = 4;
  hipStream_t side4 = nullptr, side2 = nullptr, sideN = nullptr;
  hipEvent_t evFork = nullptr, evJoin4 = nullptr, evJoin2 = nullptr, evJoinN = nullptr;
  DevBuf<uint32_t> surfRnd;
  DevBuf<float4> pixBuf;
  int aoOverlap = 0;
  hipEvent_t evPre = nullptr, evPre2 = nullptr, evAo = nullptr, evAo2 = nullptr;
  DevBuf<AoRecord> aoRecs;
  DevBuf<uint32_t> aoCount;
  DevBuf<uint32_t> aoKeys, aoOrder, aoHist;
  DevBuf<uint8_t> aoHit;
  uint32_t aoBins = 0;
  int aoDefer = 1;
  DevBuf<uint32_t> color;
  DevBuf<int32_t> tileMap;
  int numBlocks = 0;
  bool layoutDirty = true;

  DevBuf<unsigned long long> statsBuf;
  int walkProbeOn = 0;
  DevBuf<uint32_t> walkProbe;
  DevBuf<int32_t> errorFlag;
  DevBuf<char> probeStage;
  int samplePatch = 3, sampleUniform = 1;
  DevBuf<float> isoVertices, isoGradients;
  DevBuf<int32_t> isoTriangles;
  bool haveIsoMesh = false;
  float isoStageMs[6] = { 0, 0, 0, 0, 0, 0 };
  DevBuf<uint4> histSegs;
  DevBuf<uint32_t> histRuns;
  uint32_t histNumRuns = 0;
  bool histPlanBuilt = false, histVolumeFits = true;
  DevBuf<unsigned long long> histResult;
  float histKernelMs = 0.f;
  DevBuf<float> streamVertices, streamVelocities;
  DevBuf<unsigned long long> streamOffsets;
  DevBuf<uint32_t> streamSeedVertex;
  DevBuf<int32_t> streamReasons;
  uint64_t streamSeeds = 0, streamNumVertices = 0;
  bool haveStreamlines = false;
  float streamKernelMs = 0.f;
  hipEvent_t ev0 = nullptr, ev1 = nullptr, ev2 = nullptr;
  ExaHipStats last{};

  bool isoEnabled() const
  {
    for (int i = 0; i < EXA_MAX_ISO_SURFACES; i++) if (fs.iso[i].enabled) return true;
    return false;
  }
  bool contourEnabled() const
// ... 57 lines not shown
```

Baseline: 59.08 frames/s.

## Pack rope-march leaf headers into 16 bytes and unpack on device

Adds a 16-byte packed leaf header format (int16 lowers, 8-bit sizes, level stored as a float exponent for the inverse cell width, begin) built at create time when the scene fits. The shipped single-channel rope march kernel reads these instead of the 32-byte headers, which halves header load traffic per brick visit in exchange for a few unpack ALU ops. It keeps a 32-byte fallback kernel, patches the packed begin on brick reordering, and exposes an option and debug query.

New measurement: 60.51 frames/s, median of 6. 1.02x the previous value.

```diff
diff --git a/include/exa_hip.h b/include/exa_hip.h
--- a/include/exa_hip.h
+++ b/include/exa_hip.h
@@ -220,6 +220,9 @@
 
 const char *exa_hip_last_error(const ExaHipRenderer * );
 
+int exa_hip_march_headers(const ExaHipScene *scene, int32_t *hdr32, uint32_t *hdr16, int32_t *unpacked, uint64_t *firstMisfit);
+int exa_hip_last_march_header_bytes(const ExaHipRenderer *);
+
 #ifdef __cplusplus
 }
 #endif
diff --git a/owlexabrick_amd/binding.py b/owlexabrick_amd/binding.py
--- a/owlexabrick_amd/binding.py
+++ b/owlexabrick_amd/binding.py
@@ -100,7 +100,7 @@
                "exa_hip_advance_tracer", "exa_hip_read_traces", "exa_hip_set_params", "exa_hip_set_shard", "exa_hip_output_pixels",
                "exa_hip_untile", "exa_hip_render", "exa_hip_render_stats", "exa_hip_get_stats",
                "exa_hip_read_accum", "exa_hip_write_accum", "exa_hip_read_activity",
-               "exa_hip_set_option", "exa_hip_last_error", "exa_hip_sample_points", "exa_hip_resample",
+               "exa_hip_set_option", "exa_hip_last_error", "exa_hip_march_headers", "exa_hip_last_march_header_bytes", "exa_hip_sample_points", "exa_hip_resample",
                "exa_hip_isosurface", "exa_hip_isosurface_read", "exa_hip_isosurface_release", "exa_hip_isosurface_stage_ms",
                "exa_hip_histogram", "exa_hip_histogram_ms",
                "exa_hip_streamlines", "exa_hip_streamlines_read", "exa_hip_streamlines_release", "exa_hip_streamlines_ms"]
@@ -165,6 +165,9 @@
         L.exa_hip_write_accum.argtypes = [vp, vp]
         L.exa_hip_read_activity.argtypes = [vp, C.c_int32, vp]
         L.exa_hip_set_option.argtypes = [vp, C.c_char_p, C.c_int32]
+        if hasattr(L, "exa_hip_march_headers"):
+            L.exa_hip_last_march_header_bytes.argtypes = [vp]
+            L.exa_hip_march_headers.argtypes = [C.POINTER(ExaHipScene), vp, vp, vp, C.POINTER(C.c_uint64)]
         L.exa_hip_last_error.restype = C.c_char_p
         L.exa_hip_last_error.argtypes = [vp]
         L.exa_hip_sample_points.argtypes = [vp, vp, C.c_uint64, vp, C.c_int32, C.c_int32, C.c_float, vp, vp, vp,
@@ -239,6 +242,19 @@
                                 nodes.ctypes.data, C.byref(flags)):
             raise RuntimeError(lib().exa_prep_last_error().decode())
         return dict(boxes=boxes, links=links, region=region, nodes=nodes[:nn.value], flags=int(flags.value))
+
+    def march_headers(self):
+        n = int(self.scene.leafListSize)
+        hdr32 = np.zeros((n, 8), dtype=np.int32)
+        hdr16 = np.zeros((n, 4), dtype=np.uint32)
+        unpacked = np.zeros((n, 8), dtype=np.int32)
+        misfit = C.c_uint64(0)
+        rc = lib().exa_hip_march_headers(C.byref(self.scene), hdr32.ctypes.data, hdr16.ctypes.data, unpacked.ctypes.data, C.byref(misfit))
+        if rc not in (0, 1):
+            raise RuntimeError("exa_hip_march_headers: bad arguments")
+        if rc:
+            return dict(packs=False, hdr32=hdr32, misfit=int(misfit.value))
+        return dict(packs=True, hdr32=hdr32, hdr16=hdr16, unpacked=unpacked)
 
     def set_kd_tree(self, nodes, root):
         nodes = np.ascontiguousarray(nodes, dtype=KDNODE_DTYPE)
@@ -379,6 +395,9 @@
 
     def setOption(self, key, value):
         self._check(lib().exa_hip_set_option(self.h, key.encode(), int(value)))
+
+    def lastMarchHeaderBytes(self):
+        return int(lib().exa_hip_last_march_header_bytes(self.h))
 
     def _push_state(self):
         contour = any(self.frameState.contour[i].enabled for i in range(MAX_CONTOUR))
diff --git a/owlexabrick_amd/csrc/exa_create.cpp b/owlexabrick_amd/csrc/exa_create.cpp
--- a/owlexabrick_amd/csrc/exa_create.cpp
+++ b/owlexabrick_amd/csrc/exa_create.cpp
@@ -69,6 +69,20 @@
     o.size[1] = B.size[0]; o.size[2] = B.size[1]; o.level = B.size[2]; o.begin = B.begin;
   }
   return hdr;
+}
+
+bool buildPackedMarchHeaders(const ExaHipScene *scene, std::vector<uint32_t> &out, uint64_t *misfit)
+{
+  out.resize(scene->leafListSize * 4);
+  for (uint64_t i = 0; i < scene->leafListSize; i++) {
+    const ExaBrick &B = scene->bricks[scene->leafList[i]];
+    if (!packMarchHeader(B.lower, B.size, B.level, B.begin, &out[4 * i])) {
+      if (misfit) *misfit = i;
+      out.clear();
+      return false;
+    }
+  }
+  return true;
 }
 
 void chooseAddressForms(ExaHipRenderer *h, const ExaHipScene *scene)
@@ -276,6 +290,11 @@
     h->kdRoot = scene->kdRoot;
     h->haveKd = true;
   }
+  if (h->haveKd && h->mul24 && h->addr32 && h->leafBeginBits) {
+    std::vector<uint32_t> hdr16;
+    if (buildPackedMarchHeaders(scene, hdr16, nullptr) && !hdr16.empty())
+      CREATE_TRY(h->leafHdr16.upload(reinterpret_cast<const int4 *>(hdr16.data()), hdr16.size() / 4));
+  }
   CREATE_TRY(h->volActive.alloc(scene->numRegions));
   CREATE_TRY(h->isoActive.alloc(scene->numRegions));
   CREATE_TRY(h->xf.alloc(size_t(EXA_MAX_CHANNELS) * EXA_NUM_XF_VALUES));
@@ -304,6 +323,29 @@
   h->sc.numInternal = 0;
 #undef CREATE_TRY
   *out = h;
+  return 0;
+}
+
+int exa_hip_march_headers(const ExaHipScene *scene, int32_t *hdr32, uint32_t *hdr16, int32_t *unpacked, uint64_t *firstMisfit)
+{
+  if (!scene || (scene->leafListSize && (!scene->leafList || !scene->bricks))) return 2;
+  for (uint64_t i = 0; i < scene->leafListSize; i++)
+    if (scene->leafList[i] < 0 || uint64_t(scene->leafList[i]) >= scene->numBricks) return 2;
+  if (hdr32) {
+    const std::vector<ExaBrick> hdr = buildMarchHeaders(scene);
+    if (!hdr.empty()) std::memcpy(hdr32, hdr.data(), hdr.size() * sizeof(ExaBrick));
+  }
+  std::vector<uint32_t> packed;
+  if (!buildPackedMarchHeaders(scene, packed, firstMisfit)) return 1;
+  for (uint64_t i = 0; i < scene->leafListSize; i++) {
+    const uint32_t *w = &packed[4 * i];
+    if (hdr16) std::memcpy(hdr16 + 4 * i, w, 16);
+    if (unpacked) {
+      const MarchHeader m = unpackMarchHeader(w[0], w[1], w[2], w[3]);
+      static_assert(sizeof(MarchHeader) == 32, "the unpacked header is the 32-byte header");
+      std::memcpy(unpacked + 8 * i, &m, sizeof(m));
+    }
+  }
   return 0;
 }
 
diff --git a/owlexabrick_amd/csrc/exa_device.h b/owlexabrick_amd/csrc/exa_device.h
--- a/owlexabrick_amd/csrc/exa_device.h
+++ b/owlexabrick_amd/csrc/exa_device.h
@@ -1,5 +1,6 @@
 #pragma once
 #include "../../include/exa_hip.h"
+#include "exa_march_header.h"
 #include <hip/hip_runtime.h>
 
 #include <vector>
@@ -130,6 +131,7 @@
   int32_t            kdMarchRoot;
   uint32_t           leafBeginBits, leafSizeBits;
   const RegionRec   *regionRec;
+  const int4        *leafHdr16;
   const RopeLeaf    *ropeLeaves;
   const KdNodeDev   *ropeNodes;
   int32_t            ropeRoot;
@@ -240,9 +242,9 @@
   hipError_t launchCompositeKd(const RenderArgs &a, int numBlocks, hipStream_t s);                                      \
   hipError_t launchRenderKd(const RenderArgs &a, int numBlocks, bool grad, bool fast, bool surf,                        \
                             int stats , hipStream_t s);                                 \
-                                                                    \
+                                                    \
   hipError_t launchRenderKdRope(const RenderArgs &a, int numBlocks, bool grad, bool fast, bool surf,                    \
-                                int stats, hipStream_t s);                                                              \
+                                int stats, hipStream_t s, int *headerBytes);                                            \
   hipError_t launchRenderKdWide(const RenderArgs &a, int numTiles, int lanesPerRay, bool grad, bool fast, bool surf,    \
                                 hipStream_t s);                                                                         \
                           \
@@ -265,7 +267,7 @@
 hipError_t launchKdRefit(KdNodeDev *nodes, KdNodeDev *marchNodes, const int32_t *nodeIds, int count, const uint8_t *active, int which, hipStream_t s);
 hipError_t launchRopeActivity(RopeLeaf *leaves, uint32_t numRegions, const uint8_t *active, int which, uint32_t *activeCount, hipStream_t s);
 hipError_t launchPermuteBricks(const float *src, float *dst, const uint32_t *srcBegin, const uint32_t *dstBegin, int4 *bricks,
-                               unsigned long long numBricks, int4 *leafHdr, const int32_t *leafList, unsigned long long leafListSize,
+                               unsigned long long numBricks, int4 *leafHdr, int4 *leafHdr16, const int32_t *leafList, unsigned long long leafListSize,
                                unsigned long long totalCells, int numFields, hipStream_t s);
 hipError_t launchInterleave(const DeviceScene &sc, unsigned long long totalCells, int nch, float *out, hipStream_t s);
 hipError_t launchUntile(const uint32_t *gathered, unsigned long long shardStride, int world,
diff --git a/owlexabrick_amd/csrc/exa_frame.cpp b/owlexabrick_amd/csrc/exa_frame.cpp
--- a/owlexabrick_amd/csrc/exa_frame.cpp
+++ b/owlexabrick_amd/csrc/exa_frame.cpp
@@ -28,7 +28,7 @@
   HIP_TRY(this, dFrom.upload(from.data(), from.size()));
   HIP_TRY(this, dTo.upload(to.data(), to.size()));
   HIP_TRY(this, moved.alloc(scalars.n));
-  HIP_TRY(this, launchPermuteBricks(scalars.p, moved.p, dFrom.p, dTo.p, bricks.p, numBricks, leafHdr.p, leafList.p, leafListSize,
+  HIP_TRY(this, launchPermuteBricks(scalars.p, moved.p, dFrom.p, dTo.p, bricks.p, numBricks, leafHdr.p, leafHdr16.p, leafList.p, leafListSize,
                                     totalCells, numFields, s));
   HIP_TRY(this, hipStreamSynchronize(s));
   std::swap(scalars.p, moved.p);
@@ -476,6 +476,7 @@
   a.leafBeginBits = packed ? leafBeginBits : 0;
   a.leafSizeBits = packed ? leafSizeBits : 0;
   a.regionRec = regionRec.p;
+  a.leafHdr16 = packHeaders ? leafHdr16.p : nullptr;
   a.ropeLeaves = (ropeThisFrame && ropeBuilt) ? ropeLeaves.p : nullptr;
   a.ropeNodes = ropeNodes.p;
   a.ropeRoot = ropeRoot;
@@ -523,7 +524,8 @@
 
 hipError_t ExaHipRenderer::march(const RenderArgs &a, int n, bool surfArg, int statsArg, hipStream_t s)
 {
-  return (ropeThisFrame && ropeBuilt) ? EXA_FORM(this, launchRenderKdRope)(a, n, p.gradientShadingDVR != 0, fastMath != 0, surfArg, statsArg, s)
+  lastMarchHeaderBytes = 0;
+  return (ropeThisFrame && ropeBuilt) ? EXA_FORM(this, launchRenderKdRope)(a, n, p.gradientShadingDVR != 0, fastMath != 0, surfArg, statsArg, s, &lastMarchHeaderBytes)
                                       : EXA_FORM(this, launchRenderKd)(a, n, p.gradientShadingDVR != 0, fastMath != 0, surfArg, statsArg, s);
 }
 
diff --git a/owlexabrick_amd/csrc/exa_kernels.hip b/owlexabrick_amd/csrc/exa_kernels.hip
--- a/owlexabrick_amd/csrc/exa_kernels.hip
+++ b/owlexabrick_amd/csrc/exa_kernels.hip
@@ -1923,9 +1923,10 @@
                            : (MULTI ? 5 : ((ROPE && !STATS && SMALL && EXA_BASIS_FORM == 1) ? EXA_ROPE_WAVES : EXA_MARCH_WAVES)));
 }
 
-template <bool GRAD, bool FAST, int MULTI, bool SURF, int STATS, bool SMALL, int NCH = 0, bool ROPE = false>
-__global__ __launch_bounds__(kKdBlock, marchWaves(MULTI, STATS, SMALL, NCH, ROPE)) void renderFrameKdKernel(const RenderArgs a)
-{
+template <bool GRAD, bool FAST, int MULTI, bool SURF, int STATS, bool SMALL, int NCH, bool ROPE, bool HDR16>
+__device__ __forceinline__ void marchFrame(const RenderArgs &a)
+{
+  static_assert(!HDR16 || (ROPE && SMALL && STATS == 0 && MULTI == 0 && NCH == 0), "16-byte headers: the shipped one-channel rope march only");
   constexpr bool LEAN = marchWaves(MULTI, STATS, SMALL, NCH, ROPE) >= 7;
   constexpr int PACKED_CT = !ROPE ? -1 : (STATS == 1 ? 0 : (SMALL ? 1 : -1));
   const bool packedRec = PACKED_CT < 0 ? a.leafBeginBits != 0 : PACKED_CT != 0;
@@ -2036,6 +2037,7 @@
     float t1 = 0.f, t_i = 0.f, t_sample = 0.f, actual_dt = 0.f;
     int child = 0, chan = 0;
     int4 hb0 = make_int4(0, 0, 0, 1), hb1 = make_int4(1, 1, 1, 0);
+    int4 hpA = make_int4(0, 0, 0x010101, 0);
     Basis B;
     B.sumWV = 0.f; B.sumW = 0.f; B.sumD = mk(0.f, 0.f, 0.f); B.sumDC = mk(0.f, 0.f, 0.f);
     float xWV[NCH > 1 ? NCH - 1 : 1];
@@ -2115,7 +2117,16 @@
 
       C.lap(ST_T_BRICK);
       C.phase(ST_W_BRICK);
-      if (listSize > 1 || w.pk.get(PK_NEEDHDR)) {
+      if (HDR16) {
+        if (listSize > 1 || w.pk.get(PK_NEEDHDR)) {
+          const char *hp = reinterpret_cast<const char *>(a.leafHdr16) + ((uint32_t)(listBegin + child) << 4);
+          hpA = *reinterpret_cast<const int4 *>(hp);
+          w.pk.clearField(PK_NEEDHDR);
+        }
+        const MarchHeader h = unpackMarchHeader((uint32_t)hpA.x, (uint32_t)hpA.y, (uint32_t)hpA.z, (uint32_t)hpA.w);
+        hb0 = make_int4(__float_as_int(h.lower[0]), __float_as_int(h.lower[1]), __float_as_int(h.lower[2]), __float_as_int(h.invCellWidth));
+        hb1 = make_int4(h.size[0], h.size[1], h.size[2], h.begin);
+      } else if (listSize > 1 || w.pk.get(PK_NEEDHDR)) {
         if (SMALL) {
           const char *hp = reinterpret_cast<const char *>(a.sc.leafHdr) + ((uint32_t)(listBegin + child) << 5);
           hb0 = *reinterpret_cast<const int4 *>(hp); hb1 = *reinterpret_cast<const int4 *>(hp + 16);
@@ -2246,6 +2257,20 @@
     if (lane == 0) atomicAdd(&a.stats[ST_WAVE_ITERS], (unsigned long long)v);
     if (threadIdx.x == 0) atomicAdd(&a.stats[ST_TILE_ITERS], 4ull * wgMaxIters);
   }
+}
+
+constexpr bool marchHdr16(int MULTI, int STATS, bool SMALL, int NCH, bool ROPE) { return ROPE && SMALL && STATS == 0 && MULTI == 0 && NCH == 0; }
+
+template <bool GRAD, bool FAST, int MULTI, bool SURF, int STATS, bool SMALL, int NCH = 0, bool ROPE = false>
+__global__ __launch_bounds__(kKdBlock, marchWaves(MULTI, STATS, SMALL, NCH, ROPE)) void renderFrameKdKernel(const RenderArgs a)
+{
+  marchFrame<GRAD, FAST, MULTI, SURF, STATS, SMALL, NCH, ROPE, marchHdr16(MULTI, STATS, SMALL, NCH, ROPE)>(a);
+}
+
+template <bool GRAD, bool FAST, bool SURF>
+__global__ __launch_bounds__(kKdBlock, marchWaves(0, 0, true, 0, true)) void renderFrameKdHdr32Kernel(const RenderArgs a)
+{
+  marchFrame<GRAD, FAST, 0, SURF, 0, true, 0, true, false>(a);
 }
 
 __device__ __forceinline__ void kdCollectStep(Ctx<0> &C, KdWalk &w, const float winLo, const float winHi, const RenderArgs &a,
@@ -2660,9 +2685,20 @@
 
 #endif
 
+template <bool ROPE, bool G, bool F, int M, bool I>
+static void launchShippedMarch(bool small, bool hdr32, dim3 grid, dim3 block, size_t lds, hipStream_t s, const RenderArgs &a)
+{
+  if constexpr (ROPE && M == 0) {
+    if (hdr32) { hipLaunchKernelGGL((renderFrameKdHdr32Kernel<G, F, I>), grid, block, lds, s, a); return; }
+  }
+  if (small) hipLaunchKernelGGL((renderFrameKdKernel<G, F, M, I, 0, true, 0, ROPE>), grid, block, lds, s, a);
+  else       hipLaunchKernelGGL((renderFrameKdKernel<G, F, M, I, 0, false, 0, ROPE>), grid, block, lds, s, a);
+}
+
 template <bool ROPE>
-static hipError_t launchRenderKdT(const RenderArgs &a, int numBlocks, bool grad, bool fast, bool surf, int stats, hipStream_t s)
-{
+static hipError_t launchRenderKdT(const RenderArgs &a, int numBlocks, bool grad, bool fast, bool surf, int stats, hipStream_t s, int *headerBytes = nullptr)
+{
+  if (headerBytes) *headerBytes = 0;
   if (numBlocks <= 0) return hipSuccess;
 #ifndef EXA_LDS_PAD
 #define EXA_LDS_PAD 0
@@ -2675,8 +2711,10 @@
   const dim3 grid(numBlocks * (256 / kKdBlock)), block(kKdBlock);
   const bool small = a.mul24 && a.addr32 && (!ROPE || (a.ropeAddr32 && a.leafBeginBits));
 #define EXA_LAUNCH(G, F, M, I, S, A) hipLaunchKernelGGL((renderFrameKdKernel<G, F, M, I, S, A, 0, ROPE>), grid, block, lds, s, a)
+  const bool hdr32 = ROPE && small && mode == 0 && !a.leafHdr16;
+  if (headerBytes && ROPE && small && mode == 0 && !stats) *headerBytes = hdr32 ? 32 : 16;
 #define EXA_PICK2(G, F, M, I) do { if (stats == 1) EXA_LAUNCH(G, F, (M ? 2 : 0), I, 1, false); else if (stats == 2) EXA_LAUNCH(G, F, (M ? 2 : 0), I, 2, false); \
-                                   else if (small) EXA_LAUNCH(G, F, M, I, 0, true); else EXA_LAUNCH(G, F, M, I, 0, false); } while (0)
+                                   else launchShippedMarch<ROPE, G, F, M, I>(small, hdr32, grid, block, lds, s, a); } while (0)
 #define EXA_PICK(G, F, M) do { if (surf) EXA_PICK2(G, F, M, true); else EXA_PICK2(G, F, M, false); } while (0)
 #define EXA_PICKM(G, F) do { if (mode == 0) EXA_PICK(G, F, 0); else if (mode == 1) EXA_PICK(G, F, 1); else EXA_PICK(G, F, 2); } while (0)
 #if !EXA_EMPTY_CELLS
@@ -2704,8 +2742,8 @@
   return hipGetLastError();
 }
 #if EXA_TU_ROPE
-hipError_t launchRenderKdRope(const RenderArgs &a, int numBlocks, bool grad, bool fast, bool surf, int stats, hipStream_t s)
-{ return launchRenderKdT<true>(a, numBlocks, grad, fast, surf, stats, s); }
+hipError_t launchRenderKdRope(const RenderArgs &a, int numBlocks, bool grad, bool fast, bool surf, int stats, hipStream_t s, int *headerBytes)
+{ return launchRenderKdT<true>(a, numBlocks, grad, fast, surf, stats, s, headerBytes); }
 #else
 hipError_t launchRenderKd(const RenderArgs &a, int numBlocks, bool grad, bool fast, bool surf, int stats, hipStream_t s)
 { return launchRenderKdT<false>(a, numBlocks, grad, fast, surf, stats, s); }
@@ -2938,21 +2976,25 @@
   for (int f = 0; f < numFields; f++)
     for (unsigned long long i = threadIdx.x; i < vol; i += 256) dst[f * totalCells + db + i] = src[f * totalCells + sb + i];
 }
-__global__ __launch_bounds__(256) void patchBeginKernel(int4 *bricks, unsigned long long numBricks, int4 *leafHdr, const int32_t *leafList,
-                                                        unsigned long long leafListSize, const uint32_t *dstBegin)
+__global__ __launch_bounds__(256) void patchBeginKernel(int4 *bricks, unsigned long long numBricks, int4 *leafHdr, int4 *leafHdr16,
+                                                        const int32_t *leafList, unsigned long long leafListSize, const uint32_t *dstBegin)
 {
   const unsigned long long i = blockIdx.x * 256ull + threadIdx.x;
   if (i < numBricks) bricks[2 * i + 1].w = (int)dstBegin[i];
-  if (i < leafListSize) leafHdr[2 * i + 1].w = (int)dstBegin[leafList[i]];
+  if (i < leafListSize) {
+    const int begin = (int)dstBegin[leafList[i]];
+    leafHdr[2 * i + 1].w = begin;
+    if (leafHdr16) leafHdr16[i].w = begin;
+  }
 }
 hipError_t launchPermuteBricks(const float *src, float *dst, const uint32_t *srcBegin, const uint32_t *dstBegin, int4 *bricks,
-                               unsigned long long numBricks, int4 *leafHdr, const int32_t *leafList, unsigned long long leafListSize,
+                               unsigned long long numBricks, int4 *leafHdr, int4 *leafHdr16, const int32_t *leafList, unsigned long long leafListSize,
                                unsigned long long totalCells, int numFields, hipStream_t s)
 {
   if (numBricks == 0) return hipSuccess;
   hipLaunchKernelGGL(permuteBricksKernel, dim3((unsigned)numBricks), dim3(256), 0, s, src, dst, srcBegin, dstBegin, bricks, totalCells, numFields);
   const unsigned long long n = numBricks > leafListSize ? numBricks : leafListSize;
-  hipLaunchKernelGGL(patchBeginKernel, dim3((unsigned)((n + 255) / 256)), dim3(256), 0, s, bricks, numBricks, leafHdr, leafList, leafListSize, dstBegin);
+  hipLaunchKernelGGL(patchBeginKernel, dim3((unsigned)((n + 255) / 256)), dim3(256), 0, s, bricks, numBricks, leafHdr, leafHdr16, leafList, leafListSize, dstBegin);
   return hipGetLastError();
 }
 
diff --git a/owlexabrick_amd/csrc/exa_march_header.h b/owlexabrick_amd/csrc/exa_march_header.h
--- /dev/null
+++ b/owlexabrick_amd/csrc/exa_march_header.h
@@ -0,0 +1,53 @@
+#pragma once
+#include <cstdint>
+
+#if defined(__HIPCC__)
+#define EXA_HD __host__ __device__ inline __attribute__((always_inline))
+#else
+#define EXA_HD inline
+#endif
+
+namespace exa {
+
+enum { kHdr16MinLower = -32768, kHdr16MaxLower = 32767, kHdr16MaxSize = 255, kHdr16MaxLevel = 30 };
+
+struct MarchHeader {
+  float   lower[3];
+  float   invCellWidth;
+  int32_t size[3];
+  int32_t begin;
+};
+
+EXA_HD bool marchHeaderPacks(const int32_t lower[3], const int32_t size[3], int32_t level)
+{
+  bool ok = level >= 0 && level <= kHdr16MaxLevel;
+  for (int k = 0; k < 3; k++)
+    ok = ok && lower[k] >= kHdr16MinLower && lower[k] <= kHdr16MaxLower && size[k] >= 1 && size[k] <= kHdr16MaxSize;
+  return ok;
+}
+
+EXA_HD bool packMarchHeader(const int32_t lower[3], const int32_t size[3], int32_t level, uint32_t begin, uint32_t w[4])
+{
+  if (!marchHeaderPacks(lower, size, level)) return false;
+  w[0] = (uint32_t(lower[0]) & 0xffffu) | (uint32_t(lower[1]) << 16);
+  w[1] = (uint32_t(lower[2]) & 0xffffu) | (uint32_t(127 - level) << 23);
+  w[2] = uint32_t(size[0]) | (uint32_t(size[1]) << 8) | (uint32_t(size[2]) << 16);
+  w[3] = begin;
+  return true;
+}
+
+EXA_HD MarchHeader unpackMarchHeader(uint32_t w0, uint32_t w1, uint32_t w2, uint32_t w3)
+{
+  MarchHeader h;
+  h.lower[0] = float(int32_t(int16_t(w0 & 0xffffu)));
+  h.lower[1] = float(int32_t(w0) >> 16);
+  h.lower[2] = float(int32_t(int16_t(w1 & 0xffffu)));
+  h.invCellWidth = __builtin_bit_cast(float, w1 & 0xffff0000u);
+  h.size[0] = int32_t(w2 & 0xffu);
+  h.size[1] = int32_t((w2 >> 8) & 0xffu);
+  h.size[2] = int32_t((w2 >> 16) & 0xffu);
+  h.begin = int32_t(w3);
+  return h;
+}
+
+}
diff --git a/owlexabrick_amd/csrc/exa_module.cpp b/owlexabrick_amd/csrc/exa_module.cpp
--- a/owlexabrick_amd/csrc/exa_module.cpp
+++ b/owlexabrick_amd/csrc/exa_module.cpp
@@ -236,6 +236,7 @@
   if (!std::strcmp(key, "interleave")) { h->interleave = value != 0; return 0; }
   if (!std::strcmp(key, "addr64")) { h->addr64 = value != 0; return 0; }
   if (!std::strcmp(key, "pack_records")) { h->packRecords = value != 0; return 0; }
+  if (!std::strcmp(key, "pack_headers")) { h->packHeaders = value != 0; return 0; }
   if (!std::strcmp(key, "brick_order")) {
     if (value && !h->brickOrderPossible) {
       h->fail("exa_hip_set_option: brick_order 1 needs channel offsets f * totalCells and brick begins that partition [0, totalCells)");
@@ -252,6 +253,12 @@
   return 1;
 }
 
+int exa_hip_last_march_header_bytes(const ExaHipRenderer *h)
+{
+  if (!h) return 0;
+  return isMulti(h) ? exa_hip_last_march_header_bytes(h->children[0]) : h->lastMarchHeaderBytes;
+}
+
 int exa_hip_read_activity(ExaHipRenderer *h, int32_t which, uint8_t *dst)
 {
   if (isMulti(h)) return onChild(h, firstChild(h), [&](ExaHipRenderer *c) { return exa_hip_read_activity(c, which, dst); });
diff --git a/owlexabrick_amd/csrc/exa_renderer.h b/owlexabrick_amd/csrc/exa_renderer.h
--- a/owlexabrick_amd/csrc/exa_renderer.h
+++ b/owlexabrick_amd/csrc/exa_renderer.h
@@ -82,6 +82,9 @@
   DevBuf<int4> bricks;
   DevBuf<int32_t> leafList;
   DevBuf<int4> leafHdr;
+  DevBuf<int4> leafHdr16;
+  int packHeaders = 1;
+  int lastMarchHeaderBytes = 0;
   DevBuf<float> scalars;
   DevBuf<float> cellsIl;
   int ilChannels = 0;
```
